# tanmayb123/OpenAI-Whisper-CoreML

Measured on AMD Instinct MI355X. Metric: audio-sec/s (RTF) + decoder tok/s, Whisper-large-v2 30s chunks, 1->8 GPU, higher is better.
Workload: dtype bf16

## Files before the change

include/whisper_mi355x_debug.h:

```cpp
#ifndef WHISPER_MI355X_DEBUG_H
#define WHISPER_MI355X_DEBUG_H

#include "whisper_mi355x.h"

#ifdef __cplusplus
extern "C" {
#endif

WM_API int wmdbg_mel_filterbank(int n_mels, float *out);
WM_API int wmdbg_mel80(float *out);

WM_API int wmdbg_gemm(wm_ctx *ctx, const float *A, const float *W, const float *bias, float *C, int M, int N,
               int K, int epi);
typedef struct wmdbg_gemm_map {
    int32_t M, N, K, epi;
    int64_t a_off, a_rpb, a_bstride, a_rstride, a_elems;
    int64_t c_off, c_rpb, c_bstride, c_rstride, c_elems;
    int32_t d_model, n_head, seq, seq_pad, batch, reserved;
    int64_t vt_elems;
} wmdbg_gemm_map;
WM_API int wmdbg_gemm_mapped(wm_ctx *ctx, const wmdbg_gemm_map *map, const float *A, const float *W, const float *bias,
                             const float *pos, float *C, float *vt);
WM_API int wmdbg_gemm_map_layout(int32_t *out4);

// ... 75 lines not shown
                               uint32_t *hit_out, uint32_t *ban_out, int32_t *cnt_out, int32_t *id_out, float *total_out,
                               int32_t *woff_out);
WM_API int wmdbg_sb_expand_tables(const int32_t *tokens, const int32_t *seq_offsets, const float *bias, const uint8_t *boost_prefixes,
                                  const int32_t *table_offsets, int n_tables, int32_t eot, int V, int32_t *counts_out,
                                  int32_t *tab_grp_out, int32_t *grp_id_out, int32_t *grp_beg_out, int32_t *ent_len_out,
                                  float *ent_bias_out, int32_t *ent_ctx_out);
WM_API int wmdbg_group_given(const int32_t *lens, const int32_t *tokens, int stride, int rows, int b0, int Cg, int N, int32_t *lens_out,
                             int32_t *tok_out, int tok_cap, int32_t *L_out);
WM_API int wmdbg_group_bias_rows(const int32_t *table_of_row, int B, const int32_t *tab_grp, int n_tables, int b0, int Cg, int N,
                                 int32_t *rng_out);
WM_API int wmdbg_seqbias_rows_state(wm_ctx *ctx, const int32_t *seq, int B, int n_ctx, int pos, int n_prompt, int V,
                                    const int32_t *tokens, const int32_t *seq_offsets, const float *bias,
                                    const uint8_t *boost_prefixes, const int32_t *table_offsets, int n_tables, int32_t eot,
                                    const int32_t *table_of_row, const uint32_t *ban_in, uint32_t *hit_out, uint32_t *ban_out,
                                    int32_t *cnt_out, int32_t *id_out, float *total_out, int32_t *woff_out);
WM_API int wmdbg_constraint_state(wm_ctx *ctx, const int32_t *seq, int B, int n_ctx, int pos, int n_prompt, int V,
                                  const int32_t *edge_beg, const int32_t *edge_tok, const int32_t *edge_next, const int32_t *def_next,
                                  const uint8_t *accept, int n_states, int32_t eot, const int32_t *starts, const uint32_t *ban_in,
                                  uint32_t *ban_out, int32_t *state_out);
WM_API int wmdbg_decode_close_cst(wm_ctx *ctx, wmdbg_step *io, const int32_t *edge_beg, const int32_t *edge_tok,
                                  const int32_t *edge_next, const int32_t *def_next, const uint8_t *accept, int n_states, int32_t eot,
                                  const int32_t *starts);
WM_API int wmdbg_step_layout(int32_t *out4);

WM_API int wmdbg_dec_attention(wm_ctx *ctx, const float *q, const float *k, const float *v, int B, int H, int T,
                        int n_keys, int nsplit, float *out);
WM_API int wmdbg_dec_self_attention_off(wm_ctx *ctx, const float *q, const float *k, const float *v, int B, int H, int T,
                                        int pos, const int32_t *off, float *out);

typedef struct wmdbg_attn {
    int32_t form;
    int32_t B, C, N, H;
    int32_t T;
    int32_t n_keys;
    int32_t nsplit;
    int32_t pos;
    int32_t n_live;
    int32_t short_lived;
    int32_t warm_rows, warm_k;
    int32_t K;
    const int32_t *off;
    const int32_t *live_rows;
    const float *q;
    const float *k, *v;
    const float *x;
    const float *ln_g, *ln_b;
    const float *Wq;
    const float *bias;
    float *out;
    float *mean_out;
    int32_t plan[16];
} wmdbg_attn;
WM_API int wmdbg_dec_attention_form(wm_ctx *ctx, wmdbg_attn *io);
WM_API int wmdbg_attn_layout(int32_t *out4);

WM_API int wmdbg_dec_self_attention_panel(wm_ctx *ctx, const float *q, const float *k, const float *v, int C, int w, int H,
                                          int T, int pos, int out_rows, float *out);
WM_API int wmdbg_dec_qkv_panel(wm_ctx *ctx, const float *x, const float *ln_g, const float *ln_b, const float *W,
                               const float *bias, int C, int w, int N, int K, int n_head, int T, int pos, float *q_out,
                               float *kcache, float *vcache);
WM_API int wmdbg_dec_embed_panel(wm_ctx *ctx, const float *emb, const float *pemb, int V, int d, int n_ctx, const int32_t *seq,
                                 int stride, int c0, int C, int w, int pos, int by_steps, float *x, float *xb, float *stats,
                                 float *mean);
WM_API int wmdbg_dec_self_attention_panel_off(wm_ctx *ctx, const float *q, const float *k, const float *v, int C, int w, int H,
                                              int T, int pos, const int32_t *off, int out_rows, float *out);
WM_API int wmdbg_dec_embed_panel_off(wm_ctx *ctx, const float *emb, const float *pemb, int V, int d, int n_ctx, const int32_t *seq,
                                     int stride, int c0, int C, int w, int pos, const int32_t *off, int by_steps, float *x, float *xb,
                                     float *stats, float *mean);
WM_API int wmdbg_prompt_panel_plan(int G, int width, int P, int sot_pos, int acap_base, int32_t *out);
WM_API int wmdbg_prompt_panel_plan_batch(int n, const int32_t *in, int32_t *out);
WM_API int wmdbg_last_prompt_prefill(wm_ctx *ctx, int32_t *out);
WM_API int wmdbg_given_panel_plan(int G, int width, const int32_t *lens, const int32_t *budgets, int max_new, int P, int n_text_ctx,
                                  uint32_t bits, int32_t *out);
WM_API int wmdbg_given_panel_plan_batch(int n, int g_max, const int32_t *in, int32_t *out);
WM_API int wmdbg_last_given_panel(wm_ctx *ctx, int32_t *out);
WM_API int wmdbg_last_given_panel_lane(wm_ctx *ctx, int lane, int32_t *out);
typedef struct {
    int32_t G, w, V, K, n_ctx, pos, n_prompt, max_new, first, last;
    const float *x;
    const float *ln_g, *ln_b;
    const float *emb;
    const float *bias;
    const int32_t *suppress;
    int32_t n_suppress, fallback_tok;
    int32_t ts_mode, ts_begin, eot;
    int32_t *hist, *rng;
    int32_t *chist, *crng;
    int32_t stop_on, stop_eot, pad_tok;
    int32_t *done;
    const int32_t *budget;
    int32_t *live_rows;
    int32_t n_live;
    const int32_t *glens, *gtok;
    int32_t stride;
    int32_t *seq;
    float *logprob;
    int32_t *wtok;
    float *wlp;
    float *logits;
    int32_t pos_out;
} wmdbg_given_panel;
WM_API int wmdbg_given_panel_round(wm_ctx *ctx, wmdbg_given_panel *io);
WM_API int wmdbg_align_capture_panel(wm_ctx *ctx, const float *dq, int d, int C, int w, int pos, const int32_t *heads,
                                     int n_heads, int slot0, int Tq, int J, int by_steps, float *cap);
WM_API int wmdbg_align_token_prob_panel(wm_ctx *ctx, const float *logits, int C, int w, int V, int ldo, const int32_t *seq,
                                        int n_ctx, int pos, int S, int eot, const int32_t *n_text, int max_text, int by_steps,
                                        float *prob);

WM_API int wmdbg_bench_dec_gemv(wm_ctx *ctx, int B, int N, int K, int ln, int resid, int n_mats, int iters,
                         int nw_override, float *avg_us);
WM_API int wmdbg_bench_dec_attention(wm_ctx *ctx, int B, int H, int T, int n_keys, int nsplit, int n_slices,
                              int iters, float *avg_us);

WM_API int wmdbg_bench_launch_floor(wm_ctx *ctx, int iters, int grid, float *eager_us, float *graph_us);

WM_API int wmdbg_bench_graph_branches(wm_ctx *ctx, int iters, int grid, int us_each, float *one_us, float *two_us);

WM_API int wmdbg_bench_gemm(wm_ctx *ctx, int M, int N, int K, int epi, int iters, int n_w, float *us);

WM_API int wmdbg_set_gemm_tile(int tile);

WM_API int wmdbg_lane_parts(int B, int lanes, int explicit_lanes, int n_text_state);
WM_API int wmdbg_cu_mask(int cu_lo, int cu_hi, uint32_t *mask8);

WM_API int wmdbg_set_precision(wm_ctx *ctx, int precision);

WM_API int wmdbg_set_tuning(const char *key, int value);
WM_API int wmdbg_group_count(int B, int lanes, int explicit_lanes);
WM_API int wmdbg_right_align(const int32_t *prompts, int stride, const int32_t *prompt_len, int b0, int Bg, int32_t *table_out,
                             int32_t *off_out);

WM_API int wmdbg_cand_groups(int B, int N, int lanes, int explicit_lanes, int32_t *b0_out, int32_t *cg_out);
WM_API int wmdbg_dec_attn_plan(const int32_t *in, int n, int32_t *out);
WM_API int wmdbg_dec_gemv_plan(const int32_t *in, int n, int32_t *out);
WM_API int wmdbg_tx_plan(const int32_t *in, int n, int32_t *out, int32_t *cut, int cut_cap);
WM_API int wmdbg_tx_plan_bounded(const int32_t *in, const int32_t *max_group_rows, int n, int32_t *out, int32_t *cut, int cut_cap);
WM_API int wmdbg_group_tables(const int32_t *in, int n, int32_t *out);
WM_API int wmdbg_group_rows_out(const int32_t *in, int n, int32_t *out);
WM_API int wmdbg_spec_groups(int B, int k, int spec_group, int32_t *b0_out, int32_t *cg_out);
WM_API int wmdbg_spec_width(int k, int bound, int last);
WM_API int wmdbg_spec_round(int G, int w, const int32_t *accepted, const int32_t *live, const int32_t *eot_at, const int32_t *left,
                            int32_t *live_out, int32_t *inc_out);
WM_API int wmdbg_spec_round_batch(int n, int G, int w, const int32_t *in, int32_t *out);
WM_API int wmdbg_pending_refusal(unsigned pending, int entry, unsigned flags, int n_cand, char *msg_out, int msg_cap);
WM_API int wmdbg_pending_take(unsigned bits, unsigned again, int32_t *out);
WM_API int wmdbg_spec_script(wm_ctx *ctx, const int32_t *tokens, int B, int max_new);
WM_API int wmdbg_spec_accept(wm_ctx *ctx, int G, int w, int n_tiles, int pos, int n_prompt, int n_ctx, int max_new, int32_t eot,
                             const int32_t *budget, const uint64_t *tilemax, const float *txt, const float *win, int32_t *seq,
                             int32_t *done, float *logprob_out, int32_t *stats_out, int32_t *round_out, int32_t *acc_out,
                             int32_t *draft_seq_out, int32_t *pos_out);
typedef struct wmdbg_spec {
    int32_t which;
    int32_t G, w, cap;
    int32_t n_prompt, n_ctx, max_new, n_vocab;
    int32_t tts_on, dts_on;
    int32_t tts_par[4], dts_par[4];
    int32_t eot, pad_tok;
    const int32_t *script;
    const int32_t *budget;
    int32_t *tseq, *dseq;
    int32_t *pos2;
    int32_t *tts_hist;
    int32_t *tts_rng;
    int32_t *dts_hist, *dts_rng;
    int32_t *chist, *crng, *dchist, *dcrng;
// ... 94 lines not shown
```

openai-whisper-coreml_amd/csrc/call_src.cpp:

```cpp
#include "call_src.h"

#include <string.h>

static size_t pcm_elem(wm_dtype t) { return t == WM_I16 ? 2 : t == WM_F32 ? 4 : 8; }

int wm_check_window(const WmAudioSrc &a, int b, const char *who) {
    WM_REQUIRE(a.mel_base[b] >= 0 && a.mel_len[b] >= 1 && a.seek[b] >= 0 && a.n_frames[b] >= 1 &&
                   a.n_frames[b] <= WM_N_FRAMES && (int64_t)a.seek[b] + a.n_frames[b] <= a.mel_len[b],
               WM_ERR_INVALID, "%srow %d: window (base %lld, T %d, seek %d, n_frames %d) invalid", who, b,
               (long long)a.mel_base[b], a.mel_len[b], a.seek[b], a.n_frames[b]);
    return WM_OK;
}

int wm_check_src_pointers(const WmAudioSrc &a) {
    if (a.windows) {
        WM_REQUIRE(a.set != nullptr, WM_ERR_INVALID, "null window set");
        return WM_OK;
    }
    WM_REQUIRE(a.mel && a.mel_base && a.mel_len && a.seek && a.n_frames, WM_ERR_INVALID, "null mel / window pointer");
    return WM_OK;
}

int wm_check_set_owner(const wm_ctx *ctx, const wm_windows *w) {
    const WmModel *m = ctx->model;
// ... 10 lines not shown
    WM_REQUIRE(a.rows || B == W, WM_ERR_INVALID, "%srows is NULL: B (%d) must be the set's %d windows", who, B, W);
    for (int b = 0; a.rows && b < B; ++b)
        WM_REQUIRE(a.rows[b] >= 0 && a.rows[b] < W, WM_ERR_INVALID, "%srow %d: window %d outside the set's [0, %d)", who, b, a.rows[b], W);
    return WM_OK;
}

int wm_stage_pcm(wm_ctx *c, const WmAudioSrc &a, int b0, int Bg, wm_mem mem, const void **d_pcm) {
    WmModel *m = c->model;
    *d_pcm = nullptr;
    if (a.mel || a.windows) return WM_OK;
    const size_t row = WM_N_SAMPLES * pcm_elem(a.pcm_dtype);
    *d_pcm = (const char *)a.pcm + (size_t)b0 * row;
    if (mem != WM_MEM_HOST) return WM_OK;
    WM_TRY(m->pcm_stage.reserve(c->stream, (size_t)Bg * row));
    WM_HIP(hipMemcpyAsync(m->pcm_stage.p, *d_pcm, (size_t)Bg * row, hipMemcpyHostToDevice, c->stream));
    *d_pcm = m->pcm_stage.p;
    return WM_OK;
}

int wm_stage_mel(wm_ctx *c, const WmAudioSrc &a, int b0, int Bg, wm_mem mem, const void *d_pcm, std::vector<WmMelWin> &win,
              const float **enc_mel, const WmMelWin **enc_win) {
    WmModel *m = c->model;
    const int C = m->dims.n_mels;
    *enc_mel = m->mel_f32;
    *enc_win = nullptr;
    if (!a.mel) return wm_frontend_run(&c->fe, &c->prof, c->stream, d_pcm, a.pcm_dtype, Bg, C, m->mel_f32, WM_F32);
    win.resize(Bg);
    for (int b = 0; b < Bg; ++b) {
        const int r = b0 + b;
        WmMelWin &w = win[b];
        w.T = a.mel_len[r]; w.seek = a.seek[r]; w.n = a.n_frames[r]; w.pad = 0;
        w.base = a.mel_base[r];
        if (mem == WM_MEM_HOST) {
            WM_HIP(hipMemcpy2DAsync(m->mel_f32 + (size_t)b * C * WM_N_FRAMES, WM_N_FRAMES * sizeof(float),
                                    a.mel + w.base + w.seek, (size_t)w.T * sizeof(float), (size_t)w.n * sizeof(float),
                                    C, hipMemcpyHostToDevice, c->stream));
            w.base = (long long)b * C * WM_N_FRAMES; w.T = WM_N_FRAMES; w.seek = 0;
        }
    }
    WM_HIP(hipMemcpyAsync(m->dmel_win, win.data(), (size_t)Bg * sizeof(WmMelWin), hipMemcpyHostToDevice, c->stream));
    if (mem != WM_MEM_HOST) *enc_mel = a.mel;
    *enc_win = m->dmel_win;
    return WM_OK;
}

int wm_stage_cross_kv(wm_ctx *c, const WmAudioSrc &a, int b0, int Bg, wm_mem mem, const void *d_pcm, std::vector<WmMelWin> &win,
                   std::vector<int32_t> &map, hipEvent_t staged) {
    WmModel *m = c->model;
    if (a.windows) {
        const wm_dims &D = m->dims;
        map.resize(Bg);
        for (int b = 0; b < Bg; ++b) map[b] = a.rows ? a.rows[b0 + b] : b0 + b;
        WM_HIP(hipMemcpyAsync(m->dxkv_rows, map.data(), (size_t)Bg * 4, hipMemcpyHostToDevice, c->stream));
        WM_TRY(wm_xkv_rows(c, m->xkv, Bg, a.set->store, m->dxkv_rows, 0, Bg, 2 * D.n_text_layer, (long)D.n_text_head * 1500 * 64,
                           false));
        if (staged) WM_HIP(hipEventRecord(staged, c->stream));
        return WM_OK;
    }
    const float *enc_mel;
    const WmMelWin *enc_win;
    WM_TRY(wm_stage_mel(c, a, b0, Bg, mem, d_pcm, win, &enc_mel, &enc_win));
    if (staged) WM_HIP(hipEventRecord(staged, c->stream));
    WM_TRY(wm_model_encode_win(c, enc_mel, enc_win, Bg, nullptr));
    return wm_model_cross_kv(c, Bg);
}
```

openai-whisper-coreml_amd/csrc/debug_hooks.cpp:

```cpp
#include <math.h>
#include <stddef.h>
#include <stdio.h>
#include <stdlib.h>
#include <string.h>

#include <algorithm>
#include <cmath>
#include <vector>

#include "../../include/whisper_mi355x_debug.h"
#include "beam.h"
#include "model.h"
#include "tx_plan.h"

namespace {
struct DevPool {
    std::vector<void *> v;
    DevPool() = default;
    DevPool(const DevPool &) = delete;
    DevPool &operator=(const DevPool &) = delete;
    ~DevPool() {
        for (void *p : v) (void)hipFree(p);
    }
    template <class T>
    int get(T **d, const void *h, size_t bytes, hipStream_t s, int fill = 0) {
        void *p = nullptr;
        WM_HIP(hipMalloc(&p, bytes + 512));
        v.push_back(p);
        *d = static_cast<T *>(p);
        WM_HIP(hipMemsetAsync(p, fill, bytes + 512, s));
        if (h) WM_HIP(hipMemcpyAsync(p, h, bytes, hipMemcpyHostToDevice, s));
        return WM_OK;
    }
};

bf16_t f2bf(float f) {
    uint32_t u;
    memcpy(&u, &f, 4);
    u += 0x7fffu + ((u >> 16) & 1u);
    return (bf16_t)(u >> 16);
}
void to_bf16(const float *in, std::vector<bf16_t> &out, size_t n) {
    out.resize(n);
    for (size_t i = 0; i < n; ++i) out[i] = f2bf(in[i]);
}
void from_bf16(const std::vector<bf16_t> &in, float *out) {
    for (size_t i = 0; i < in.size(); ++i) {
        uint32_t u = (uint32_t)in[i] << 16;
        memcpy(&out[i], &u, 4);
    }
}
void tile_bf16(const float *m, size_t rows, size_t K, std::vector<bf16_t> &out) {
    const size_t rpad = (rows + 15) / 16 * 16;
    std::vector<float> t(rpad * K, 0.f);
    for (size_t r = 0; r < rows; ++r)
        for (size_t k = 0; k < K; ++k) t[wm_tiled_offset(r, k, K)] = m[r * K + k];
    to_bf16(t.data(), out, t.size());
}
void untile_bf16(const std::vector<bf16_t> &t, size_t rows, size_t K, float *out) {
    std::vector<bf16_t> lin(rows * K);
    for (size_t r = 0; r < rows; ++r)
        for (size_t k = 0; k < K; ++k) lin[r * K + k] = t[wm_tiled_offset(r, k, K)];
    from_bf16(lin, out);
}
void fill_bf16(std::vector<bf16_t> &v, size_t n) { v.assign(n, (bf16_t)WMDBG_SENTINEL_BF16); }
void fill_f32(std::vector<float> &v, size_t n) {
// ... 103 lines not shown
        return WM_OK;
    }
    int replay_us(EventPair &ev, float *us) {
        WM_HIP(hipGraphLaunch(ge, s));
        WM_HIP(hipStreamSynchronize(s));
        WM_TRY(ev.start(s));
        WM_HIP(hipGraphLaunch(ge, s));
        return ev.stop_us(s, us);
    }
};

struct SideBranch {
    hipStream_t s2 = nullptr;
    hipEvent_t ef = nullptr, ej = nullptr;
    SideBranch() = default;
    SideBranch(const SideBranch &) = delete;
    SideBranch &operator=(const SideBranch &) = delete;
    ~SideBranch() {
        if (ef) (void)hipEventDestroy(ef);
        if (ej) (void)hipEventDestroy(ej);
        if (s2) (void)hipStreamDestroy(s2);
    }
    int init() {
        WM_HIP(hipStreamCreateWithFlags(&s2, hipStreamNonBlocking));
        WM_HIP(hipEventCreateWithFlags(&ef, hipEventDisableTiming));
        WM_HIP(hipEventCreateWithFlags(&ej, hipEventDisableTiming));
        return WM_OK;
    }
    int fork(hipStream_t s) {
        WM_HIP(hipEventRecord(ef, s));
        WM_HIP(hipStreamWaitEvent(s2, ef, 0));
        return WM_OK;
    }
    int join(hipStream_t s) {
        WM_HIP(hipEventRecord(ej, s2));
        WM_HIP(hipStreamWaitEvent(s, ej, 0));
        return WM_OK;
    }
};
}

int wm_gemm_set_tile_override(int tile);
extern "C" int wmdbg_set_gemm_tile(int tile) { return wm_gemm_set_tile_override(tile); }

extern "C" int wmdbg_set_tuning(const char *key, int value) {
    WM_REQUIRE(key, WM_ERR_INVALID, "wmdbg_set_tuning: null key");
    struct { const char *name; int *field; } table[] = {
        {"gemv_tn", &g_wm_tuning.gemv_tn}, {"gemv_nblk", &g_wm_tuning.gemv_nblk}, {"gemv_no_ppw2", &g_wm_tuning.gemv_no_ppw2}, {"gemv_ppw2_nblk", &g_wm_tuning.gemv_ppw2_nblk},
        {"prefetch_max_b", &g_wm_tuning.prefetch_max_b}, {"xattn_split_below", &g_wm_tuning.xattn_split_below},
        {"xattn_wgs", &g_wm_tuning.xattn_wgs}, {"xattn_no_flat", &g_wm_tuning.xattn_no_flat},
        {"xattn_lds_pad", &g_wm_tuning.xattn_lds_pad}, {"xattn_splits", &g_wm_tuning.xattn_splits},
        {"gemm_tile", &g_wm_tuning.gemm_tile}, {"gemm128_pipe", &g_wm_tuning.gemm128_pipe}, {"gemm_gm", &g_wm_tuning.gemm_gm}, {"no_early_stop", &g_wm_tuning.no_early_stop},
        {"xattn_no_deep", &g_wm_tuning.xattn_no_deep}, {"xattn_never_short", &g_wm_tuning.xattn_never_short},         {"logits_tn", &g_wm_tuning.logits_tn}, {"enc_attn_mfma_sum", &g_wm_tuning.enc_attn_mfma_sum},
        {"group_chunks", &g_wm_tuning.group_chunks}, {"argmax_rows_per_wg", &g_wm_tuning.argmax_rows_per_wg}, {"xattn_fuse_q", &g_wm_tuning.xattn_fuse_q},
        {"teacher_panel_cut", &g_wm_tuning.teacher_panel_cut}, {"lane_parts", &g_wm_tuning.lane_parts}, {"lane_solo_cus", &g_wm_tuning.lane_solo_cus}, {"spec_group", &g_wm_tuning.spec_group}, {"frontend_per_wave_twiddles", &g_wm_tuning.frontend_per_wave_twiddles},
    };
    if (strcmp(key, "reset") == 0) { g_wm_tuning = WmTuning(); return WM_OK; }
    for (auto &e : table)
        if (strcmp(key, e.name) == 0) { *e.field = value; return WM_OK; }
    wm_set_error("wmdbg_set_tuning: unknown key '%s'", key);
    return WM_ERR_INVALID;
}

extern "C" int wmdbg_group_count(int B, int lanes, int explicit_lanes) { return wm_group_count(B, lanes, explicit_lanes != 0, 0); }
extern "C" int wmdbg_cand_groups(int B, int N, int lanes, int explicit_lanes, int32_t *b0_out, int32_t *cg_out) {
    if (B < 1 || N < 1 || N > WM_MAX_BEST_OF || !b0_out || !cg_out) return -1;
    std::vector<int> b0, cg;
    const int G = wm_cand_groups(B, N, lanes, explicit_lanes != 0, b0, cg);
    for (int g = 0; g < G; ++g) { b0_out[g] = b0[g]; cg_out[g] = cg[g]; }
    return G;
}
extern "C" int wmdbg_dec_attn_plan(const int32_t *in, int n, int32_t *out) {
    if (!in || !out || n < 0) return -1;
    for (int i = 0; i < n; ++i) wm_attn_plan_flat(in + (size_t)i * WM_ATTN_PLAN_IN, g_wm_tuning, out + (size_t)i * WM_ATTN_PLAN_OUT);
    return n;
}
extern "C" int wmdbg_dec_gemv_plan(const int32_t *in, int n, int32_t *out) {
    if (!in || !out || n < 0) return -1;
    for (int i = 0; i < n; ++i) wm_gemv_plan_flat(in + (size_t)i * WM_GEMV_PLAN_IN, g_wm_tuning, out + (size_t)i * WM_GEMV_PLAN_OUT);
    return n;
}
extern "C" int wmdbg_tx_plan(const int32_t *in, int n, int32_t *out, int32_t *cut, int cut_cap) {
    if (!in || !out || !cut || n < 0 || cut_cap < 0) return -1;
    int used = 0;
    for (int i = 0; i < n; ++i) {
        int32_t *o = out + (size_t)i * WM_TX_PLAN_OUT;
        const int k = wm_tx_plan_flat(in + (size_t)i * WM_TX_PLAN_IN, o, cut + used, cut_cap - used);
        if (k < 0) return -1;
        o[5] = used;
        used += k;
    }
    return n;
}
extern "C" int wmdbg_tx_plan_bounded(const int32_t *in, const int32_t *max_group_rows, int n, int32_t *out, int32_t *cut, int cut_cap) {
    if (!in || !max_group_rows || !out || !cut || n < 0 || cut_cap < 0) return -1;
    int used = 0;
    for (int i = 0; i < n; ++i) {
        int32_t *o = out + (size_t)i * WM_TX_PLAN_OUT;
        const int k = wm_tx_plan_flat(in + (size_t)i * WM_TX_PLAN_IN, o, cut + used, cut_cap - used, max_group_rows[i]);
        if (k < 0) return -1;
        o[5] = used;
        used += k;
    }
    return n;
}
extern "C" int wmdbg_group_tables(const int32_t *in, int n, int32_t *out) {
    if (!in || !out || n < 0) return -1;
// ... 449 lines not shown
    WM_TRY(pool.get(&dl, live.data(), live.size() * 4, s));
    WM_TRY(pool.get(&datt, nullptr, ((size_t)B + 15) / 16 * 16 * H * 64 * 2, s));
    DecAttnArgs t = {};
    t.q = dq; t.kc = dk; t.vc = dv; t.att = datt; t.part = dp; t.C = C; t.N = N; t.H = H; t.T_stride = T; t.n_keys = n_keys;
    t.live = live_rows ? dl : nullptr; t.short_lived = short_lived;
    WM_TRY(wm_dec_attention_cand(ctx, t));
    return down_tiled_bf16(datt, (size_t)B, (size_t)H * 64, out, s);
}

extern "C" int wmdbg_dec_attention_cand(wm_ctx *ctx, const float *q, const float *k, const float *v, int C, int N, int H, int T,
                                        int n_keys, const int32_t *live_rows, int n_live, float *out) {
    return dec_attention_cand(ctx, q, k, v, C, N, H, T, n_keys, live_rows, n_live, out, false);
}
extern "C" int wmdbg_dec_attention_cand_shared(wm_ctx *ctx, const float *q, const float *k, const float *v, int C, int N, int H,
                                               int T, int n_keys, const int32_t *live_rows, int n_live, float *out) {
    return dec_attention_cand(ctx, q, k, v, C, N, H, T, n_keys, live_rows, n_live, out, true);
}

extern "C" int wmdbg_dec_self_attention_off(wm_ctx *ctx, const float *q, const float *k, const float *v, int B, int H, int T,
                                            int pos, const int32_t *off, float *out) {
    WM_TRY(wm_ctx_make_current(ctx));
    WM_REQUIRE(q && k && v && off && out, WM_ERR_INVALID, "dec_self_attention_off: null pointer");
    WM_REQUIRE(B >= 1 && B <= WM_DEC_MAXB && T >= 1 && pos >= 0 && pos < T, WM_ERR_INVALID, "dec_self_attention_off: bad geometry");
    for (int b = 0; b < B; ++b)
        WM_REQUIRE(off[b] >= 0 && off[b] < T, WM_ERR_INVALID, "dec_self_attention_off: off[%d] = %d outside [0, %d)", b, off[b], T);
    std::vector<bf16_t> k16, v16;
    to_bf16(k, k16, (size_t)B * H * T * 64);
    to_bf16(v, v16, (size_t)B * H * T * 64);
    DevPool pool;
    hipStream_t s = ctx->stream;
    const float *dq;
    const bf16_t *dk, *dv;
    const int *doff, *dpos;
    bf16_t *datt;
    WM_TRY(pool.get(&dq, q, (size_t)B * H * 64 * 4, s));
    WM_TRY(pool.get(&dk, k16.data(), k16.size() * 2, s));
    WM_TRY(pool.get(&dv, v16.data(), v16.size() * 2, s));
    WM_TRY(pool.get(&doff, off, (size_t)B * 4, s));
    WM_TRY(pool.get(&dpos, &pos, 4, s));
    WM_TRY(pool.get(&datt, nullptr, ((size_t)B + 15) / 16 * 16 * H * 64 * 2, s));
    DecAttnArgs t = {};
    t.q = dq; t.kc = dk; t.vc = dv; t.att = datt; t.B = B; t.H = H; t.T_stride = T; t.pos_ptr = dpos; t.off = doff;
    WM_TRY(wm_dec_self_attention(ctx, t));
    return down_tiled_bf16(datt, (size_t)B, (size_t)H * 64, out, s);
}

extern "C" int wmdbg_attn_layout(int32_t *out4) {
    if (!out4) return WM_ERR_INVALID;
    out4[0] = (int32_t)sizeof(wmdbg_attn); out4[1] = (int32_t)offsetof(wmdbg_attn, off);
    out4[2] = (int32_t)offsetof(wmdbg_attn, out); out4[3] = (int32_t)offsetof(wmdbg_attn, plan);
    return WM_OK;
}

extern "C" int wmdbg_dec_attention_form(wm_ctx *ctx, wmdbg_attn *io) {
    WM_TRY(wm_ctx_make_current(ctx));
    WM_REQUIRE(io && io->out && io->k && io->v, WM_ERR_INVALID, "dec_attention_form: null pointer");
    memset(io->plan, 0, sizeof(io->plan));
    const int form = io->form, H = io->H, T = io->T;
    WM_REQUIRE(form >= 0 && form <= 3, WM_ERR_INVALID, "dec_attention_form: form %d is not 0 .. 3", form);
    const bool cand = form == 1, fq = form == 2, self = form == 3;
    WM_REQUIRE(!cand || (io->C >= 1 && io->N >= 1 && io->N <= WM_MAX_BEST_OF && io->C <= WM_DEC_MAXB), WM_ERR_INVALID,
               "dec_attention_form: %d windows x %d candidates", io->C, io->N);
    const int rows = cand ? io->C * io->N : io->B, entries = cand ? io->C : io->B;
    WM_REQUIRE(rows >= 1 && rows <= WM_DEC_MAXB && H >= 1 && H <= 1024, WM_ERR_INVALID, "dec_attention_form: %d rows x %d heads", rows, H);
    const size_t dd = (size_t)H * 64, rpad = ((size_t)rows + 15) / 16 * 16;
    {
        std::vector<bf16_t> s16;
        fill_bf16(s16, rpad * dd);
        from_bf16(s16, io->out);
        const uint32_t u = WMDBG_SENTINEL_F32;
        for (int b = 0; fq && io->mean_out && b < rows; ++b) memcpy(io->mean_out + b, &u, 4);
    }
    const bool has_pos = io->pos >= 0, has_pf = io->warm_rows > 0 && io->warm_k > 0;
    int32_t pin[WM_ATTN_PLAN_IN] = {0};
    pin[0] = form; pin[1] = cand ? 0 : io->B; pin[2] = cand ? io->C : 0; pin[3] = cand ? io->N : 0; pin[4] = H; pin[5] = T;
    pin[6] = io->n_keys; pin[7] = io->nsplit; pin[8] = fq ? io->K : 0;
    pin[9] = (has_pos ? 1 : 0) | (fq || self ? 0 : 2) | (io->off ? 4 : 0) | (has_pf ? 8 : 0) | (io->short_lived ? 16 : 0) | (io->live_rows ? 32 : 0);
    pin[10] = has_pf ? io->warm_rows : 0; pin[11] = has_pf ? io->warm_k : 0; pin[12] = ctx->n_cus;
    wm_attn_plan_flat(pin, g_wm_tuning, io->plan);
    if (io->plan[0] != WM_OK) return WM_ERR_INVALID;
    WM_REQUIRE(H <= 255 && T >= 1 && T <= WM_ATT_MAXK, WM_ERR_INVALID, "dec_attention_form: H 1 .. 255, T 1 .. %d", WM_ATT_MAXK);
    WM_REQUIRE(!has_pos || form == 0 || self, WM_ERR_INVALID, "dec_attention_form: form %d takes no device position", form);
    const int nk = has_pos ? io->pos + 1 : io->n_keys;
    WM_REQUIRE(nk >= 1 && nk <= T && io->n_keys >= 0 && io->n_keys <= T, WM_ERR_INVALID, "dec_attention_form: %d keys outside 1 .. T = %d", nk, T);
    WM_REQUIRE(self || (io->n_keys >= 1 && (!has_pos || io->n_keys == nk)), WM_ERR_INVALID,
               "dec_attention_form: a cross form needs n_keys >= 1 keys, and n_keys = pos + 1 with a device position");
    WM_REQUIRE(!io->off || self, WM_ERR_INVALID, "dec_attention_form: row offsets belong to the self-attention");
    WM_REQUIRE(!io->off || has_pos, WM_ERR_INVALID, "dec_attention_form: row offsets need the device position");
    for (int b = 0; io->off && b < rows; ++b)
        WM_REQUIRE(io->off[b] >= 0 && io->off[b] < T, WM_ERR_INVALID, "dec_attention_form: off[%d] = %d outside [0, %d)", b, io->off[b], T);
    WM_REQUIRE(!io->short_lived || form <= 1, WM_ERR_INVALID, "dec_attention_form: short_lived is a cross-attention shape");
    WM_REQUIRE(io->warm_rows >= 0 && io->warm_rows <= 8192 && io->warm_k >= 0 && io->warm_k <= 8192 && io->warm_k % 32 == 0 && io->warm_rows % 16 == 0,
               WM_ERR_INVALID, "dec_attention_form: warm-up matrix of %d x %d", io->warm_rows, io->warm_k);
    std::vector<int32_t> live((size_t)WM_DEC_MAXB + 4, 0);
    if (io->live_rows) {
        WM_REQUIRE(io->n_live >= 0 && io->n_live <= rows, WM_ERR_INVALID, "dec_attention_form: n_live %d outside [0, %d]", io->n_live, rows);
        for (int i = 0; i < io->n_live; ++i) {
            WM_REQUIRE(io->live_rows[i] >= 0 && io->live_rows[i] < rows && (i == 0 || io->live_rows[i] > io->live_rows[i - 1]), WM_ERR_INVALID,
                       "dec_attention_form: the live list must be ascending rows of the group");
            live[i] = io->live_rows[i];
        }
        live[WM_DEC_MAXB] = io->n_live;
    }
    if (fq)
        WM_REQUIRE(io->x && io->ln_g && io->ln_b && io->Wq && io->mean_out && io->K == H * 64 && io->K <= 1280, WM_ERR_INVALID,
                   "dec_attention_form: the fused query needs x, ln_g, ln_b, Wq, mean_out and K = H * 64 <= 1280");
    else
        WM_REQUIRE(io->q, WM_ERR_INVALID, "dec_attention_form: null query");
    std::vector<bf16_t> k16, v16, w16, x16, fill;
    std::vector<float> st, mean;
    to_bf16(io->k, k16, (size_t)entries * dd * T);
    to_bf16(io->v, v16, (size_t)entries * dd * T);
    fill_bf16(fill, rpad * dd);
    const std::vector<uint32_t> fill32((size_t)rows, WMDBG_SENTINEL_F32);
    DevPool pool;
    hipStream_t s = ctx->stream;
    const bf16_t *dk, *dv;
    bf16_t *datt;
    WM_TRY(pool.get(&dk, k16.data(), k16.size() * 2, s));
    WM_TRY(pool.get(&dv, v16.data(), v16.size() * 2, s));
    WM_TRY(pool.get(&datt, fill.data(), fill.size() * 2, s));
    DecAttnArgs t = {};
    t.kc = dk; t.vc = dv; t.att = datt; t.H = H; t.T_stride = T; t.n_keys = io->n_keys; t.short_lived = io->short_lived != 0;
    if (cand) { t.C = io->C; t.N = io->N; } else t.B = io->B;
    if (!fq) WM_TRY(pool.get(&t.q, io->q, (size_t)rows * dd * 4, s));
    if (form <= 1) WM_TRY(pool.get(&t.part, nullptr, (size_t)rows * H * WM_MAXSPLIT * 66 * 4, s));
    if (has_pos) WM_TRY(pool.get(&t.pos_ptr, &io->pos, 4, s));
    if (io->off) WM_TRY(pool.get(&t.off, io->off, (size_t)rows * 4, s));
    if (io->live_rows) WM_TRY(pool.get(&t.live, live.data(), live.size() * 4, s));
    if (has_pf) {
        WM_TRY(pool.get(&t.pf.ptr, nullptr, (size_t)io->warm_rows * io->warm_k * 2, s));
        t.pf.rows = io->warm_rows; t.pf.k = io->warm_k;
    }
    float *dmean_out = nullptr;
    switch (form) {
        case 0: t.nsplit = io->nsplit; WM_TRY(wm_dec_attention(ctx, t)); break;
        case 1: WM_TRY(wm_dec_attention_cand(ctx, t)); break;
        case 3: WM_TRY(wm_dec_self_attention(ctx, t)); break;
        default: {
            const int K = io->K, B = io->B;
            tile_bf16(io->Wq, (size_t)K, (size_t)K, w16);
            stage_ln_rows(io->x, B, K, true, x16, st, mean);
            DecGemvArgs a;
            memset(&a, 0, sizeof(a));
            a.epi = DE_Q; a.B = B; a.N = K; a.K = K; a.stats_parts = K / 16; a.ldo = K;
            const bf16_t *dW;
            bf16_t *dWf;
            float *dc1, *dc2;
            const float *dg, *db, *dbias = nullptr;
            WM_TRY(pool.get(&a.a, x16.data(), x16.size() * 2, s));
            WM_TRY(pool.get(&dW, w16.data(), w16.size() * 2, s));
            WM_TRY(pool.get(&dWf, nullptr, w16.size() * 2, s));
            WM_TRY(pool.get(&dc1, nullptr, (size_t)K * 4, s));
            WM_TRY(pool.get(&dc2, nullptr, (size_t)K * 4, s));
            WM_TRY(pool.get(&dg, io->ln_g, (size_t)K * 4, s));
            WM_TRY(pool.get(&db, io->ln_b, (size_t)K * 4, s));
            if (io->bias) WM_TRY(pool.get(&dbias, io->bias, (size_t)K * 4, s));
            WM_TRY(pool.get(&a.stats_in, st.data(), st.size() * 4, s));
            WM_TRY(pool.get(&a.mean_in, mean.data(), (size_t)B * 4, s));
            WM_TRY(pool.get(&a.mean_out, fill32.data(), (size_t)B * 4, s));
            WM_TRY(wm_ln_fold(ctx, dW, dg, db, dbias, K, K, dWf, dc1, dc2));
            a.W = dWf; a.c1 = dc1; a.c2 = dc2;
            dmean_out = a.mean_out;
            WM_TRY(wm_dec_xattn_fq(ctx, a, t));
        }
    }
    if (dmean_out) WM_HIP(hipMemcpyAsync(io->mean_out, dmean_out, (size_t)rows * 4, hipMemcpyDeviceToHost, s));
    return down_tiled_bf16(datt, rpad, dd, io->out, s);
}


extern "C" int wmdbg_bench_dec_gemv(wm_ctx *ctx, int B, int N, int K, int ln, int resid, int n_mats, int iters,
                                    int nw_override, float *avg_us) {
    (void)nw_override;
    WM_TRY(wm_ctx_make_current(ctx));
    WM_REQUIRE(B >= 1 && B <= WM_DEC_MAXB, WM_ERR_INVALID, "wmdbg_bench_dec_gemv: B out of range");
    DevPool pool;
    hipStream_t s = ctx->stream;
    const int Npad = ((N + 15) / 16) * 16;
    const bf16_t *dW;
    const float *dc;
    bf16_t *dout16;
    float *dstat;
    DecGemvArgs a;
    memset(&a, 0, sizeof(a));
    a.B = B; a.N = N; a.K = K; a.ldo = Npad; a.epi = resid ? DE_RESID : DE_Q;
    WM_TRY(pool.get(&dW, nullptr, (size_t)n_mats * Npad * K * 2, s, 0x3c));
    WM_TRY(pool.get(&a.a, nullptr, (size_t)WM_DEC_MAXB * K * 2, s));
    WM_TRY(pool.get(&dc, nullptr, (size_t)Npad * 4, s));
    WM_TRY(pool.get(&a.out_f32, nullptr, (size_t)WM_DEC_MAXB * Npad * 4, s));
    WM_TRY(pool.get(&dout16, nullptr, (size_t)WM_DEC_MAXB * Npad * 2, s));
    WM_TRY(pool.get(&dstat, nullptr, (size_t)(WM_DEC_MAXB / 16) * 2 * (K > N ? K : N) * 4 + 4096, s));
    a.c2 = dc;
    if (resid) { a.stats_out = dstat; a.out_bf16 = dout16; }
    if (ln) { a.c1 = dc; a.stats_in = dstat; a.stats_parts = K / 16; }
    EventPair ev;
    WM_TRY(ev.init());
    GraphRun run(s);
    WM_TRY(run.begin());
    for (int i = 0; i < iters; ++i) {
        a.W = dW + (size_t)(i % n_mats) * Npad * K;
        WM_TRY(wm_dec_gemv(ctx, a));
    }
    WM_TRY(run.end());
    float us = 0.f;
    WM_TRY(run.replay_us(ev, &us));
    *avg_us = us / iters;
    return WM_OK;
}

extern "C" int wmdbg_bench_dec_attention(wm_ctx *ctx, int B, int H, int T, int n_keys, int nsplit, int n_slices,
                                         int iters, float *avg_us) {
    WM_TRY(wm_ctx_make_current(ctx));
    DevPool pool;
    hipStream_t s = ctx->stream;
    const size_t slice = (size_t)B * H * T * 64;
    const bf16_t *dk, *dv;
    const float *dq;
    float *dp;
    bf16_t *datt;
    WM_TRY(pool.get(&dk, nullptr, slice * n_slices * 2, s));
    WM_TRY(pool.get(&dv, nullptr, slice * n_slices * 2, s));
    WM_TRY(pool.get(&dq, nullptr, (size_t)B * H * 64 * 4, s));
    WM_TRY(pool.get(&dp, nullptr, (size_t)B * H * WM_MAXSPLIT * 66 * 4, s));
    WM_TRY(pool.get(&datt, nullptr, ((size_t)B + 15) / 16 * 16 * H * 64 * 2, s));
    EventPair ev;
    WM_TRY(ev.init());
    DecAttnArgs t = {};
    t.q = dq; t.att = datt; t.part = dp; t.B = B; t.H = H; t.T_stride = T; t.n_keys = n_keys; t.nsplit = nsplit;
    for (int pass = 0; pass < 2; ++pass) {
        if (pass == 1) WM_TRY(ev.start(s));
        for (int i = 0; i < iters; ++i) {
            t.kc = dk + (size_t)(i % n_slices) * slice;
            t.vc = dv + (size_t)(i % n_slices) * slice;
            WM_TRY(wm_dec_attention(ctx, t));
        }
    }
    float us = 0.f;
    WM_TRY(ev.stop_us(s, &us));
    *avg_us = us / iters;
    return WM_OK;
}

int wm_launch_trivial(wm_ctx *ctx, int *p, int grid);
extern "C" int wmdbg_bench_launch_floor(wm_ctx *ctx, int iters, int grid, float *eager_us, float *graph_us) {
    WM_TRY(wm_ctx_make_current(ctx));
    DevPool pool;
    hipStream_t s = ctx->stream;
    int *d;
    WM_TRY(pool.get(&d, nullptr, 64, s));
    EventPair ev;
    WM_TRY(ev.init());
    float us = 0.f;
    for (int i = 0; i < 20; ++i) WM_TRY(wm_launch_trivial(ctx, d, grid));
    WM_TRY(ev.start(s));
    for (int i = 0; i < iters; ++i) WM_TRY(wm_launch_trivial(ctx, d, grid));
    WM_TRY(ev.stop_us(s, &us));
    *eager_us = us / iters;
    GraphRun run(s);
    WM_TRY(run.begin());
    for (int i = 0; i < iters; ++i) WM_TRY(wm_launch_trivial(ctx, d, grid));
    WM_TRY(run.end());
    WM_TRY(run.replay_us(ev, &us));
    *graph_us = us / iters;
    return WM_OK;
}

extern "C" int wmdbg_bench_gemm(wm_ctx *ctx, int M, int N, int K, int epi, int iters, int n_w, float *us) {
    WM_TRY(wm_ctx_make_current(ctx));
    WM_REQUIRE(epi == EPI_F32 || epi == EPI_BIAS_BF16 || epi == EPI_GELU_BF16 || epi == EPI_RESID_F32, WM_ERR_INVALID,
               "wmdbg_bench_gemm: epilogue %d not exposed", epi);
    WM_REQUIRE(n_w >= 1 && n_w <= 64, WM_ERR_INVALID, "wmdbg_bench_gemm: n_w out of range");
    std::vector<bf16_t> a16((size_t)M * K), w16((size_t)N * K);
    uint32_t x = 12345u;
    auto gauss = [&]() {
        float acc = 0.f;
        for (int i = 0; i < 4; ++i) { x = x * 1664525u + 1013904223u; acc += (float)(x >> 8) * (1.0f / 16777216.0f); }
        return (acc - 2.0f) * 1.7320508f;
    };
    for (auto &v : a16) v = f2bf(gauss());
    for (auto &v : w16) v = f2bf(0.02f * gauss());
    std::vector<float> bias(N);
    for (auto &v : bias) v = 0.01f * gauss();
    DevPool pool;
    hipStream_t s = ctx->stream;
    std::vector<const bf16_t *> dW(n_w, nullptr);
    GemmArgs g;
    memset(&g, 0, sizeof(g));
    WM_TRY(pool.get(&g.A, a16.data(), a16.size() * 2, s));
    for (int i = 0; i < n_w; ++i) WM_TRY(pool.get(&dW[i], w16.data(), w16.size() * 2, s));
    WM_TRY(pool.get(&g.bias, bias.data(), (size_t)N * 4, s));
    WM_TRY(pool.get(&g.C, nullptr, (size_t)M * N * 4, s));
    g.a_rpb = (long)M + 1; g.a_rstride = K;
    g.c_rpb = (long)M + 1; g.c_rstride = N; g.M = M; g.N = N; g.K = K; g.epi = epi;
// ... 584 lines not shown
    WmTsDev ts;
    memset(&ts, 0, sizeof(ts));
    if (io->ts_on) {
        ts.hist = (int *)dev(io->hist); ts.rng = (int *)dev(io->rng);
        ts.ts_begin = io->ts_par[0]; ts.eot = io->ts_par[1]; ts.n_vocab = io->ts_par[2]; ts.max_initial = io->ts_par[3];
    }
    WmStopDev sp;
    memset(&sp, 0, sizeof(sp));
    if (io->stop_on) {
        sp.done = (int *)dev(io->done); sp.live_rows = (int *)dev(io->live_rows); sp.n_live = (int *)dev(io->n_live);
        sp.eot = io->eot; sp.pad_tok = io->pad;
    }
    WmXDev xd;
    memset(&xd, 0, sizeof(xd));
    WM_TRY(pool.get(&xd.par, &xp, sizeof(xp), s));
    xd.logprob = (float *)dev(io->logprob);
    WM_TRY(wm_beam_select_step(ctx, rows, (int *)dev(io->seq), d_pos, n_prompt, WmEmbedDev{d_emb, d_pemb, d, d_x, d_xb, d_st, d_mean}, ts, sp,
                               xd, d_off, bm));
    for (const Buf &b : bufs)
        if (b.h) WM_HIP(hipMemcpyAsync(b.h, b.d, b.bytes, hipMemcpyDeviceToHost, s));
    WM_HIP(hipMemcpyAsync(&io->pos_out, d_pos, 4, hipMemcpyDeviceToHost, s));
    WM_HIP(hipMemcpyAsync(io->x_next, d_x, nr * d * 4, hipMemcpyDeviceToHost, s));
    WM_HIP(hipMemcpyAsync(io->mean_next, d_mean, nr * 4, hipMemcpyDeviceToHost, s));
    WM_HIP(hipMemcpyAsync(stn.data(), d_st, st_words * 4, hipMemcpyDeviceToHost, s));
    WM_TRY(down_tiled_bf16(d_xb, nr, (size_t)d, io->xb_next, s));
    io->stats_tail_nonzero = 0;
    for (size_t b = 0; b < nr; ++b) {
        stats_sum(stn.data(), d, (int)b, io->stats_next + b * 2);
        for (int part = 1; part < d / 16 && b < (size_t)rows; ++part)
            for (int c = 0; c < 2; ++c) {
                uint32_t u;
                memcpy(&u, &stn[stat_at(d, b, part, c)], 4);
                if (u != 0u) ++io->stats_tail_nonzero;
            }
    }
    return WM_OK;
}

extern "C" int wmdbg_xkv_rows(wm_ctx *ctx, uint16_t *group, int group_rows, uint16_t *store, int64_t store_rows, const int32_t *rows,
                              int n_rows, int L, int H, int to_store) {
    WM_TRY(wm_ctx_make_current(ctx));
    WM_REQUIRE(group && store && rows && L >= 1 && H >= 1 && n_rows >= 1 && n_rows <= group_rows && group_rows <= WM_DEC_MAXB &&
                   store_rows >= 1, WM_ERR_INVALID, "xkv_rows: bad args");
    for (int b = 0; b < n_rows; ++b) {
        WM_REQUIRE(rows[b] >= 0 && rows[b] < store_rows, WM_ERR_INVALID, "xkv_rows: rows[%d] = %d outside [0, %lld)", b, rows[b],
                   (long long)store_rows);
        for (int o = 0; to_store && o < b; ++o)
            WM_REQUIRE(rows[o] != rows[b], WM_ERR_INVALID, "xkv_rows: store row %d named twice", rows[b]);
    }
    DevPool pool;
    hipStream_t s = ctx->stream;
    const int *drows;
    WM_TRY(pool.get(&drows, rows, (size_t)n_rows * 4, s));
    int rc = wm_xkv_rows(ctx, group, group_rows, store, drows, 0, n_rows, 2 * L, (long)H * 1500 * 64, to_store != 0);
    if (hipStreamSynchronize(s) != hipSuccess && rc == WM_OK) {
        wm_set_error("xkv_rows: %s", hipGetErrorString(hipGetLastError()));
        rc = WM_ERR_HIP;
    }
    return rc;
}

static int dec_gemv_ln_run(wm_ctx *ctx, int epi, const float *x, const float *ln_g, const float *ln_b, const float *W,
                           const float *bias, int B, int N, int K, int centre, int n_head, int T, int pos, int panel, float *out_f32,
                           float *out_bf16, float *kcache, float *vcache, float *mean_out, float *Wf, float *c1, float *c2) {
    WM_TRY(wm_ctx_make_current(ctx));
    WM_REQUIRE(panel == 0 || (epi == DE_QKV && panel >= 1 && panel <= WM_MAX_TEACHER_PANEL && pos + panel <= T), WM_ERR_INVALID,
               "wmdbg_dec_qkv_panel: width 1 .. %d, pos + width <= T", WM_MAX_TEACHER_PANEL);
    WM_REQUIRE(epi == DE_QKV || epi == DE_Q || epi == DE_GELU, WM_ERR_INVALID, "wmdbg_dec_gemv_ln: epilogue %d not exposed", epi);
    WM_REQUIRE(x && ln_g && ln_b && W && mean_out && Wf && c1 && c2, WM_ERR_INVALID, "wmdbg_dec_gemv_ln: null pointer");
    WM_REQUIRE(B >= 1 && B <= WM_DEC_MAXB && N >= 1 && K >= 64 && K % 64 == 0 && K <= 1280, WM_ERR_INVALID,
               "wmdbg_dec_gemv_ln: B 1 .. %d, N >= 1, K a multiple of 64 up to 1280", WM_DEC_MAXB);
    const int d = N / 3;
    if (epi == DE_QKV)
        WM_REQUIRE(N % 3 == 0 && n_head >= 1 && d == n_head * 64 && T >= 1 && pos >= 0 && pos < T && out_f32 && kcache && vcache,
                   WM_ERR_INVALID, "wmdbg_dec_gemv_ln: DE_QKV needs N = 3 * n_head * 64, pos in [0, T) and its three outputs");
    if (epi == DE_Q) WM_REQUIRE(out_f32, WM_ERR_INVALID, "wmdbg_dec_gemv_ln: DE_Q needs out_f32");
    if (epi == DE_GELU) WM_REQUIRE(N % 32 == 0 && out_bf16, WM_ERR_INVALID, "wmdbg_dec_gemv_ln: DE_GELU needs N %% 32 == 0 and out_bf16");
    const size_t Npad = ((size_t)N + 15) / 16 * 16, Bpad = ((size_t)B + 15) / 16 * 16;
    std::vector<bf16_t> w16, x16;
    std::vector<float> st, mean;
    tile_bf16(W, (size_t)N, (size_t)K, w16);
    stage_ln_rows(x, B, K, centre != 0, x16, st, mean);
    const size_t n_f32 = epi == DE_QKV ? (size_t)B * d : epi == DE_Q ? (size_t)B * N : 0;
    const size_t n_b16 = epi == DE_GELU ? Bpad * N : 0, n_cache = epi == DE_QKV ? (size_t)(panel ? (B + panel - 1) / panel : B) * n_head * T * 64 : 0;
    const std::vector<bf16_t> fill16(std::max(n_b16, n_cache), (bf16_t)WMDBG_SENTINEL_BF16);
    const std::vector<uint32_t> fill32((size_t)B, WMDBG_SENTINEL_F32);
    std::vector<bf16_t> wf16(w16.size()), ob16(n_b16), k16(n_cache), v16(n_cache);
    DevPool pool;
    hipStream_t s = ctx->stream;
    DecGemvArgs a;
    memset(&a, 0, sizeof(a));
    a.epi = epi; a.B = B; a.N = N; a.K = K; a.stats_parts = K / 16; a.ldo = N;
    const bf16_t *dW;
    bf16_t *dWf;
    float *dc1, *dc2;
    const float *dg, *db, *dbias = nullptr, *dmin;
    const int *dpos;
    WM_TRY(pool.get(&a.a, x16.data(), x16.size() * 2, s));
    WM_TRY(pool.get(&dW, w16.data(), w16.size() * 2, s));
    WM_TRY(pool.get(&dWf, nullptr, w16.size() * 2, s));
    WM_TRY(pool.get(&dc1, nullptr, Npad * 4, s));
    WM_TRY(pool.get(&dc2, nullptr, Npad * 4, s));
    WM_TRY(pool.get(&dg, ln_g, (size_t)K * 4, s));
    WM_TRY(pool.get(&db, ln_b, (size_t)K * 4, s));
    if (bias) WM_TRY(pool.get(&dbias, bias, (size_t)N * 4, s));
    WM_TRY(pool.get(&a.stats_in, st.data(), st.size() * 4, s));
// ... 1364 lines not shown
    WM_HIP(hipMemcpyAsync(m->att, s16.data(), M * d * 2, hipMemcpyHostToDevice, s));
    WM_HIP(hipMemcpyAsync(m->hid, s16.data(), M * 4 * d * 2, hipMemcpyHostToDevice, s));
    WM_HIP(hipMemsetAsync(m->vt, 0, vt_n * 2, s));
    int rc = wm_model_encode_layer_qkv(ctx, layer, B);
    if (rc == WM_OK) rc = wm_model_encode_layer_tail(ctx, layer, B, dmid);
    if (rc == WM_OK) rc = down_bf16(m->att, M * d, att_out, s);
    if (rc == WM_OK) rc = down_bf16(m->xn, M * d, xn2_out, s);
    if (rc == WM_OK) rc = down_bf16(m->hid, M * 4 * d, hid_out, s);
    if (rc == WM_OK) {
        WM_HIP(hipMemcpyAsync(x_mid_out, dmid, M * d * 4, hipMemcpyDeviceToHost, s));
        WM_HIP(hipMemcpyAsync(x_out, m->x, M * d * 4, hipMemcpyDeviceToHost, s));
    }
    WM_HIP(hipMemsetAsync(m->qk + M * 2 * d, 0, (size_t)64 * 2 * d * 2, s));
    WM_HIP(hipStreamSynchronize(s));
    return rc;
}

extern "C" int wmdbg_encode_post(wm_ctx *ctx, const float *x, int B, float *xn_out, float *xa_out) {
    WM_REQUIRE(x && xn_out && xa_out, WM_ERR_INVALID, "wmdbg_encode_post: null pointer");
    WM_TRY(model_ready(ctx, B, "wmdbg_encode_post"));
    WmModel *m = ctx->model;
    const int d = m->dims.n_audio_state;
    const size_t M = (size_t)B * 1500;
    std::vector<bf16_t> s16;
    std::vector<float> s32;
    fill_bf16(s16, M * d);
    fill_f32(s32, M * d);
    hipStream_t s = ctx->stream;
    WM_HIP(hipMemcpyAsync(m->x, x, M * d * 4, hipMemcpyHostToDevice, s));
    WM_HIP(hipMemcpyAsync(m->xn, s16.data(), M * d * 2, hipMemcpyHostToDevice, s));
    WM_HIP(hipMemcpyAsync(m->xa_f32, s32.data(), M * d * 4, hipMemcpyHostToDevice, s));
    int rc = wm_model_encode_post(ctx, B, nullptr);
    if (rc == WM_OK) rc = down_bf16(m->xn, M * d, xn_out, s);
    if (rc == WM_OK) WM_HIP(hipMemcpyAsync(xa_out, m->xa_f32, M * d * 4, hipMemcpyDeviceToHost, s));
    WM_HIP(hipStreamSynchronize(s));
    return rc;
}

extern "C" int wmdbg_cross_kv(wm_ctx *ctx, const float *xa, int B, float *xkv_out) {
    WM_REQUIRE(xa && xkv_out, WM_ERR_INVALID, "wmdbg_cross_kv: null pointer");
    WM_TRY(model_ready(ctx, B, "wmdbg_cross_kv"));
    WmModel *m = ctx->model;
    const wm_dims &D = m->dims;
    WM_REQUIRE(D.n_text_state == D.n_audio_state, WM_ERR_INVALID, "wmdbg_cross_kv: encoder and decoder widths differ");
    const int d = D.n_text_state, H = D.n_text_head;
    const size_t M = (size_t)B * 1500, used = (size_t)D.n_text_layer * 2 * B * H * 1500 * 64,
                 cap = (size_t)D.n_text_layer * 2 * m->cap_b * H * 1500 * 64;
    std::vector<bf16_t> s16, got(cap);
    fill_bf16(s16, cap);
    DevPool pool;
    hipStream_t s = ctx->stream;
    const float *dxa;
    WM_TRY(pool.get(&dxa, xa, M * d * 4, s));
    WM_HIP(hipMemcpyAsync(m->xkv, s16.data(), cap * 2, hipMemcpyHostToDevice, s));
    int rc = wm_model_set_xa(ctx, dxa, B);
    if (rc == WM_OK) rc = wm_model_cross_kv(ctx, B);
    WM_HIP(hipMemcpyAsync(got.data(), m->xkv, cap * 2, hipMemcpyDeviceToHost, s));
    if (cap > used) WM_HIP(hipMemsetAsync(m->xkv + used, 0, (cap - used) * 2, s));
    WM_HIP(hipStreamSynchronize(s));
    WM_TRY(rc);
    size_t disturbed = 0;
    for (size_t i = used; i < cap; ++i) disturbed += got[i] != (bf16_t)WMDBG_SENTINEL_BF16;
    WM_REQUIRE(disturbed == 0, WM_ERR_STATE, "wmdbg_cross_kv: %zu elements behind the %d chunks' cache were written", disturbed, B);
    got.resize(used);
    from_bf16(got, xkv_out);
    return WM_OK;
}
```

openai-whisper-coreml_amd/csrc/dec_kernels.hip:

```cpp
#include <stdlib.h>

#include <atomic>
#include <string.h>

#include "dec_close.h"
#include "model.h"
#include "philox.h"

namespace {

typedef __attribute__((ext_vector_type(8))) __bf16 bf16x8;
typedef __attribute__((ext_vector_type(4))) float f32x4;
typedef __attribute__((ext_vector_type(4))) unsigned u32x4;

typedef __attribute__((ext_vector_type(2))) float f32x2;
typedef __attribute__((ext_vector_type(2))) __bf16 bf16x2;

__device__ __forceinline__ unsigned pack2(float a, float b) {
    const f32x2 v = {a, b};
    return __builtin_bit_cast(unsigned, __builtin_convertvector(v, bf16x2));
}
__device__ __forceinline__ float gelu_erf(float x) {
    return 0.5f * x * (1.0f + erff(x * 0.70710678118654752440f));
}
struct DecGemvDev {
    int B, N, K;
    const bf16_t *W;
    const float *c1;
    const float *c2;
    const bf16_t *a;
    const float *stats_in;
    int stats_parts;
    long stats_stride;
    float *stats_out;
    const float *mean_in;
    float *mean_out;
    float *out_f32;
    bf16_t *out_bf16;
    bf16_t *kcache, *vcache;
    const int *pos_ptr;
    int n_ctx, n_head;
    long ldo;
    unsigned long long *tilemax;
    int n_tiles;
    int n_tg, n_tg_pad;
    int arg_first, arg_last;
    const unsigned *mask;
    int mask_words, mask_first_pos;
    WmTsDev ts;
    WmXDev x;
    const char *pf_ptr;
    long pf_tile_bytes;
    int pf_tiles;
    int pf_head_major;
    int bgroups;
    WmRepDev rep;
    int panel;
    WmSbEpi sb;
};

// ... 1003 lines not shown
        const bf16_t *vb = vc + (long)bh * T_stride * 64 + e8 * 8;
        float qe[8];
        attn_scale_query(q + (long)b * d + h * 64 + e8 * 8, qe);
        float m_run = -1e30f, l_run = 0.f;
        float oa[8] = {0, 0, 0, 0, 0, 0, 0, 0};
        auto load_block = [&](int r0, u32x4 (&kv)[U], u32x4 (&vv)[U]) {
            attn_load_block<NS, U, NT>(kb, vb, r0, stream, rg, n_keys, last, kv, vv);
        };
        auto process_block = [&](int r0, const u32x4 (&kv)[U], const u32x4 (&vv)[U]) {
            attn_block<NS, U, false>(qe, r0, stream, rg, n_keys, kv, vv, m_run, l_run, oa);
        };
        if (DEEP) {
            constexpr int NB = ATT_MAXK / (NS * 8 * U);
            u32x4 kall[NB][U], vall[NB][U];
#pragma unroll
            for (int blk = 0; blk < NB; ++blk) load_block(blk * (NS * 8 * U), kall[blk], vall[blk]);
#pragma unroll
            for (int blk = 0; blk < NB; ++blk)
                if (blk * (NS * 8 * U) < n_keys) process_block(blk * (NS * 8 * U), kall[blk], vall[blk]);
        } else {
            for (int r0 = 0; r0 < n_keys; r0 += NS * 8 * U) {
                u32x4 kv[U], vv[U];
                load_block(r0, kv, vv);
                process_block(r0, kv, vv);
            }
        }
        attn_stream_reduce(l_run, oa);
        if (nsplit > 1) {
            if (rg == 0) {
                float *po = part + ((long)bh * NS + stream) * 66;
#pragma unroll
                for (int i = 0; i < 8; ++i) po[2 + e8 * 8 + i] = oa[i];
                if (e8 == 0) {
                    po[0] = m_run;
                    po[1] = l_run;
                }
            }
            continue;
        }
        if (rg == 0) {
#pragma unroll
            for (int i = 0; i < 8; ++i) wo_[wave][e8 * 8 + i] = oa[i];
            if (e8 == 0) {
                wm_[wave] = m_run;
                wl_[wave] = l_run;
            }
        }
        __syncthreads();
        if (tid < 64)
            att[wm_tiled_offset((size_t)b, (size_t)(h * 64 + tid), (size_t)d)] = f2bf(attn_merge<NS>(wm_, wl_, &wo_[0][0], 64, tid));
    }
}

struct CandLive {
    int r_lo, r_hi;
    unsigned long long head_lo, head_hi;
};
template <int N>
__device__ __forceinline__ void cand_window(const CandLive &L, int wj, int lane, int &c, unsigned &lm) {
    const int rank_lo = (int)__builtin_amdgcn_mbcnt_hi((unsigned)(L.head_lo >> 32), __builtin_amdgcn_mbcnt_lo((unsigned)L.head_lo, 0u));
    const int rank_hi = (int)__builtin_amdgcn_mbcnt_hi((unsigned)(L.head_hi >> 32), __builtin_amdgcn_mbcnt_lo((unsigned)L.head_hi, 0u)) +
                        __popcll(L.head_lo);
    const unsigned long long sel_lo = __ballot(((L.head_lo >> lane) & 1ull) && rank_lo == wj);
    const unsigned long long sel_hi = __ballot(((L.head_hi >> lane) & 1ull) && rank_hi == wj);
    int row;
    if (sel_lo) row = __builtin_amdgcn_readlane(L.r_lo, __builtin_ctzll(sel_lo));
    else row = __builtin_amdgcn_readlane(L.r_hi, sel_hi ? __builtin_ctzll(sel_hi) : 0);
    c = row / N;
    lm = 0u;
#pragma unroll
    for (int s = 0; s < N; ++s) {
        const int r = c * N + s;
        if ((__ballot(L.r_lo == r) | __ballot(L.r_hi == r)) != 0ull) lm |= 1u << s;
    }
}

template <int N, bool NT>
__global__ __launch_bounds__(512) void dec_xcand_attn_kernel(
    const float *__restrict__ q, const bf16_t *__restrict__ kc, const bf16_t *__restrict__ vc,
    const int *__restrict__ live_rows , bf16_t *__restrict__ att,
    float *__restrict__ part, unsigned packA , unsigned packB ,
    unsigned packC , const char *pf_ptr, long pf_tile_bytes) {
    constexpr int NS = 8, U = 4;
    static_assert(N >= 1 && N <= 8, "1 .. 8 candidates per window");
    constexpr int NP = N <= 5 ? N : (N + 1) / 2;
    const int H = (int)(packA & 0xffu), flat_wpw = (int)(packA >> 16);
    const int T_stride = (int)(packB & 0xffffu), n_keys = (int)(packB >> 16);
    const int C = (int)(packC & 0xffffu), n_wg = (int)(packC >> 16);
    const int d = H * 64;
    if (attn_warm_up(n_wg, pf_ptr, pf_tile_bytes, blockDim.x)) return;
    __shared__ float wm_[N][NS], wl_[N][NS];
    __shared__ float wo_[N][NS][64];
    const int tid = threadIdx.x, lane = tid & 63, wave = tid >> 6;
    const int rg = lane >> 3, e8 = lane & 7;
    const int last = n_keys - 1;
    CandLive L;
    {
        int n_live = C * N, p_lo = lane - 1, p_hi = lane + 63;
        L.r_lo = lane;
        L.r_hi = lane + 64;
        if (live_rows) {
            n_live = live_rows[WM_DEC_MAXB];
            L.r_lo = live_rows[lane];
            L.r_hi = live_rows[lane + 64];
            p_lo = live_rows[lane > 0 ? lane - 1 : 0];
            p_hi = live_rows[lane + 63];
// ... 520 lines not shown
        p.pf_ptr = (const char *)a.pf_ptr;
        p.pf_tile_bytes = pl.pf_tile_bytes; p.pf_tiles = pl.pf_tiles; p.pf_head_major = pl.pf_head_major;
    }
    WmProfScope ps(&ctx->prof, e->label_k && a.K > a.N ? e->label_k : e->label, ctx->stream);
    return e->launch(ctx, p, pl);
}

int wm_ln_fold(wm_ctx *ctx, const bf16_t *W, const float *g, const float *beta, const float *bias, int N, int K,
               bf16_t *Wf, float *c1, float *c2) {
    const int npad = (N + 15) / 16 * 16;
    ln_fold_kernel<<<npad, 256, 0, ctx->stream>>>(W, g, beta, bias, N, K, Wf, c1, c2);
    WM_HIP(hipGetLastError());
    return WM_OK;
}

int wm_dec_embed(wm_ctx *ctx, const int *seq, const int *pos_ptr, int B, const WmEmbedDev &e, const int *off) {
    WmProfScope ps(&ctx->prof, "dec_embed", ctx->stream);
    dec_embed_kernel<<<B, 256, 0, ctx->stream>>>(seq, pos_ptr, B, e.emb, e.pemb, e.d, e.x, e.xb, e.stats_out, e.mean_buf, off);
    WM_HIP(hipGetLastError());
    return WM_OK;
}

int wm_dec_embed_panel(wm_ctx *ctx, const int *seq, int seq_stride, const int *pos_ptr, int pos_add, int C, int w, int n_ctx,
                       const WmEmbedDev &e, const int *off) {
    WM_REQUIRE(w >= 1 && w <= WM_MAX_TEACHER_PANEL && C >= 1 && C * w <= WM_DEC_MAXB && seq_stride >= C, WM_ERR_INVALID,
               "dec_embed_panel: %d windows x %d positions (stride %d)", C, w, seq_stride);
    WmProfScope ps(&ctx->prof, "dec_embed_panel", ctx->stream);
    if (off)
        dec_embed_panel_off_kernel<<<C * w, 256, 0, ctx->stream>>>(seq, seq_stride, pos_ptr, pos_add, w, e.emb, e.pemb, e.d, n_ctx, e.x,
                                                                  e.xb, e.stats_out, e.mean_buf, off);
    else
        dec_embed_panel_kernel<<<C * w, 256, 0, ctx->stream>>>(seq, seq_stride, pos_ptr, pos_add, w, e.emb, e.pemb, e.d, n_ctx, e.x, e.xb,
                                                              e.stats_out, e.mean_buf);
    WM_HIP(hipGetLastError());
    return WM_OK;
}

int wm_dec_pos_add(wm_ctx *ctx, int *pos_ptr, int add) {
    dec_pos_add_kernel<<<1, 1, 0, ctx->stream>>>(pos_ptr, add);
    WM_HIP(hipGetLastError());
    return WM_OK;
}

int wm_dec_attn_splits(int B, int H) { return wm_dec_attn_splits(B, H, g_wm_tuning); }
bool wm_dec_xattn_fq_applies(int B, int H, int K, bool short_lived) { return wm_dec_xattn_fq_applies(B, H, K, short_lived, g_wm_tuning); }

namespace {
DecAttnShape attn_shape(const DecAttnArgs &t) {
    DecAttnShape s;
    memset(&s, 0, sizeof(s));
    s.B = t.B; s.C = t.C; s.N = t.N; s.H = t.H; s.T_stride = t.T_stride; s.n_keys = t.n_keys; s.nsplit = t.nsplit;
    s.has_pos = t.pos_ptr != nullptr; s.has_part = t.part != nullptr; s.has_off = t.off != nullptr; s.short_lived = t.short_lived;
    s.has_pf = t.pf.ptr != nullptr; s.pf_rows = t.pf.rows; s.pf_k = t.pf.k;
    return s;
}
int launch_combine(wm_ctx *ctx, const DecAttnArgs &t, const DecAttnPlan &pl);
}

int wm_dec_attention(wm_ctx *ctx, const DecAttnArgs &t) {
    DecAttnPlan pl;
    WM_TRY(wm_plan_attention(attn_shape(t), ctx->n_cus, g_wm_tuning, &pl));
    {
        WmProfScope ps(&ctx->prof, "dec_attn_cross", ctx->stream);
        const dim3 grid(pl.grid_x, pl.grid_y);
        if (pl.variant == DAV_STREAM) {
            const int lds_pad = g_wm_tuning.xattn_lds_pad;
            static std::atomic<int> pad_set[64];
            if (lds_pad > pad_set[ctx->device & 63].load(std::memory_order_acquire)) {
                WM_HIP(hipFuncSetAttribute((const void *)dec_xrows_attn_kernel<8, 4, WM_XATTN_NT>,
                                           hipFuncAttributeMaxDynamicSharedMemorySize, lds_pad));
                pad_set[ctx->device & 63].store(lds_pad, std::memory_order_release);
            }
            const AttnCold cold = {t.att, t.part, (const char *)t.pf.ptr, pl.tile_bytes};
            dec_xrows_attn_kernel<8, 4, WM_XATTN_NT><<<grid, pl.block, pl.lds, ctx->stream>>>(
                t.q, t.kc, t.vc, t.pos_ptr, t.live, pl.w.a, pl.w.b, pl.w.c, cold);
        } else {
            const AttnCold cold = {t.att, t.part, nullptr, 0};
            if (pl.variant == DAV_FLAT)
                dec_xrows_attn_kernel<8, 4, WM_XATTN_NT><<<grid, pl.block, 0, ctx->stream>>>(
                    t.q, t.kc, t.vc, t.pos_ptr, t.live, pl.w.a, pl.w.b, pl.w.c, cold);
            else if (pl.variant == DAV_FLAT_DEEP_C)
                dec_rows_attn_kernel<8, 4, false, true><<<grid, pl.block, 0, ctx->stream>>>(
                    t.q, t.kc, t.vc, t.pos_ptr, t.live, pl.w.a, pl.w.b, pl.w.c, cold);
            else
                dec_rows_attn_kernel<8, 4, WM_XATTN_NT, true><<<grid, pl.block, 0, ctx->stream>>>(
                    t.q, t.kc, t.vc, t.pos_ptr, t.live, pl.w.a, pl.w.b, pl.w.c, cold);
        }
        WM_HIP(hipGetLastError());
    }
    return pl.combine_grid ? launch_combine(ctx, t, pl) : WM_OK;
}

namespace {
int launch_combine(wm_ctx *ctx, const DecAttnArgs &t, const DecAttnPlan &pl) {
    WmProfScope ps(&ctx->prof, "dec_attn_combine", ctx->stream);
    dec_attn_combine_kernel<8><<<pl.combine_grid, 64, 0, ctx->stream>>>(t.part, t.H, t.H * 64, t.att);
    WM_HIP(hipGetLastError());
    return WM_OK;
}
}

int wm_dec_attention_cand(wm_ctx *ctx, const DecAttnArgs &t) {
    DecAttnPlan pl;
    WM_TRY(wm_plan_attention_cand(attn_shape(t), ctx->n_cus, g_wm_tuning, &pl));
    {
        WmProfScope ps(&ctx->prof, "dec_attn_cross_cand", ctx->stream);
        const char *pf = pl.warm_tiles ? (const char *)t.pf.ptr : nullptr;
        switch (t.N) {
#define WM_XCAND_CASE(n)                                                                                              \
    case n:                                                                                                           \
        dec_xcand_attn_kernel<n, WM_XATTN_NT><<<pl.grid_x, pl.block, 0, ctx->stream>>>(                               \
            t.q, t.kc, t.vc, t.live, t.att, t.part, pl.w.a, pl.w.b, pl.w.c, pf, pl.warm_tiles ? pl.tile_bytes : 0);   \
        break
            WM_XCAND_CASE(1); WM_XCAND_CASE(2); WM_XCAND_CASE(3); WM_XCAND_CASE(4);
            WM_XCAND_CASE(5); WM_XCAND_CASE(6); WM_XCAND_CASE(7); WM_XCAND_CASE(8);
#undef WM_XCAND_CASE
        }
        WM_HIP(hipGetLastError());
// ... 188 lines not shown
```

openai-whisper-coreml_amd/csrc/dec_launch.cpp:

```cpp
#include "dec_launch.h"

#include <stddef.h>
#include <string.h>

#include "../../include/whisper_mi355x.h"

void wm_set_error(const char *fmt, ...);

#define PLAN_REQUIRE(cond, ...)           \
    do {                                  \
        if (!(cond)) {                    \
            wm_set_error(__VA_ARGS__);    \
            return WM_ERR_INVALID;        \
        }                                 \
    } while (0)

namespace {
inline bool fits(int v, int bits) { return v >= 0 && (bits >= 31 || v < (1 << bits)); }
}

bool wm_pack_attn_keys(int T_stride, int n_keys, unsigned *b) {
    *b = (unsigned)T_stride | ((unsigned)n_keys << 16);
    return fits(T_stride, 16) && fits(n_keys, 16);
}
// ... 63 lines not shown
    const int bh = B * H;
    const int thr = t.xattn_split_below;
    if (bh >= thr) return 1;
    int ns = 2;
    while (ns < 8 && bh * ns < 192) ns *= 2;
    return ns;
}

int wm_dec_gemv_split(int K, int *spw) {
    const int steps = K / 32;
    for (int nw = steps >= 96 ? 16 : 8; nw >= 1; --nw) {
        if (steps % nw) continue;
        const int s = steps / nw;
        if (s == 2 || s == 4 || s == 5 || s == 6 || s == 8 || s == 10 || s == 12) {
            if (spw) *spw = s;
            return nw;
        }
    }
    return 0;
}

bool wm_dec_xattn_fq_applies(int B, int H, int K, bool short_lived, const WmTuning &t) {
    if (!t.xattn_fuse_q || short_lived) return false;
    const int pairs = B * H;
    if (pairs < t.xattn_split_below || pairs > 256 || K != H * 64) return false;
    int spw = 0;
    const int nw = wm_dec_gemv_split(K, &spw);
    return nw >= 1 && nw <= 8 && (spw == 2 || spw == 4 || spw == 5 || spw == 6);
}

int wm_plan_attention(const DecAttnShape &s, int n_cus, const WmTuning &t, DecAttnPlan *p) {
    const int B = s.B, H = s.H, nsplit = s.nsplit;
    memset(p, 0, sizeof(*p));
    PLAN_REQUIRE(nsplit == 1 || nsplit == 2 || nsplit == 4 || nsplit == 8, "dec_attention: nsplit %d is not 1, 2, 4 or 8", nsplit);
    PLAN_REQUIRE(s.T_stride <= WM_ATT_MAXK && s.n_keys <= WM_ATT_MAXK, "dec_attention: more than %d keys", WM_ATT_MAXK);
    PLAN_REQUIRE(nsplit == 1 || s.has_part, "dec_attention: split launch without a partials buffer");
    PLAN_REQUIRE(H >= 1 && H <= 255 && (long)B * H < 65536, "dec_attention: %d heads x %d rows do not fit the packed arguments", H, B);
    bool ok = wm_pack_attn_keys(s.T_stride, s.n_keys, &p->w.b);
    if (nsplit > 1 && !t.xattn_no_flat) {
        int wpw, g;
        wm_dec_flat_deal(B * H, 4, &wpw, &g);
        PLAN_REQUIRE(g < 65536, "dec_attention: flat grid too large");
        ok = wm_pack_attn_rows(H, 8, wpw, B * H, g, &p->w.a, &p->w.c) && ok;
        if (t.xattn_no_deep) p->variant = DAV_FLAT;
        else if ((size_t)B * H * s.T_stride * 64 * 2 * 2 <= (size_t)3200 * 1024) p->variant = DAV_FLAT_DEEP_C;
        else p->variant = DAV_FLAT_DEEP_NT;
        p->n_wg = p->grid_x = g;
        p->grid_y = 1;
        p->block = wpw * 64;
    } else {
        const int n_wg = wm_dec_persistent_wgs(B * H, n_cus, s.short_lived, t);
        p->warm_tiles = wm_dec_warm_tiles(B, s.has_pf && nsplit == 1, s.pf_rows, s.pf_k, n_wg, t, &p->tile_bytes);
        ok = wm_pack_attn_rows(H, nsplit, 0, B * H, n_wg, &p->w.a, &p->w.c) && ok;
        p->variant = DAV_STREAM;
        p->n_wg = n_wg;
        p->grid_x = n_wg + p->warm_tiles;
        p->grid_y = nsplit;
        p->block = (8 / nsplit) * 64;
        p->lds = nsplit == 1 ? t.xattn_lds_pad : 0;
    }
    PLAN_REQUIRE(ok, "dec_attention: a packed argument does not fit its bits");
    p->combine_grid = nsplit > 1 ? B * H : 0;
    return WM_OK;
}

int wm_plan_attention_cand(const DecAttnShape &s, int n_cus, const WmTuning &t, DecAttnPlan *p) {
    const int C = s.C, N = s.N, H = s.H;
    memset(p, 0, sizeof(*p));
    PLAN_REQUIRE(N >= 1 && N <= WM_MAX_BEST_OF && C >= 1 && (long)C * N <= WM_DEC_MAXB,
                 "dec_attention_cand: %d windows x %d candidates outside 1 .. %d rows of 1 .. %d candidates", C, N, WM_DEC_MAXB,
                 WM_MAX_BEST_OF);
    PLAN_REQUIRE(s.T_stride >= 1 && s.T_stride <= WM_ATT_MAXK && s.n_keys >= 1 && s.n_keys <= s.T_stride,
                 "dec_attention_cand: 1 .. %d keys", WM_ATT_MAXK);
    PLAN_REQUIRE(H >= 1 && H <= 255, "dec_attention_cand: %d heads do not fit the packed arguments", H);
    PLAN_REQUIRE(s.has_part || C * H >= 256 || s.short_lived, "dec_attention_cand: flat launch without a partials buffer");
    const int pairs = C * H;
    const bool flat = pairs < 256 && !s.short_lived;
    bool ok = wm_pack_attn_keys(s.T_stride, s.n_keys, &p->w.b);
    if (flat) {
        int wpw, g;
        wm_dec_flat_deal(pairs, 8, &wpw, &g);
        ok = wm_pack_attn_cand(H, wpw, C, g, &p->w.a, &p->w.c) && ok;
        p->variant = DAV_CAND_FLAT;
        p->n_wg = g;
        p->block = wpw * 64;
        p->combine_grid = C * N * H;
    } else {
        const int n_wg = wm_dec_persistent_wgs(pairs, n_cus, s.short_lived, t);
        PLAN_REQUIRE(n_wg < 65536, "dec_attention_cand: grid too large");
        ok = wm_pack_attn_cand(H, 0, C, n_wg, &p->w.a, &p->w.c) && ok;
        p->variant = DAV_CAND;
        p->n_wg = n_wg;
        p->block = 512;
    }
    PLAN_REQUIRE(ok, "dec_attention_cand: a packed argument does not fit its bits");
    p->warm_tiles = wm_dec_warm_tiles(C * N, s.has_pf, s.pf_rows, s.pf_k, p->n_wg, t, &p->tile_bytes);
    p->grid_x = p->n_wg + p->warm_tiles;
    p->grid_y = 1;
    return WM_OK;
}

int wm_plan_xattn_fq(const DecAttnShape &s, int n_cus, const WmTuning &t, DecAttnPlan *p) {
    (void)n_cus;
    const int B = s.B, H = s.H;
    memset(p, 0, sizeof(*p));
    PLAN_REQUIRE(s.K == (long)H * 64, "xattn_fq: not a LayerNorm-folded d x d query projection");
    PLAN_REQUIRE(H >= 1 && H <= 255 && B >= 1 && B <= WM_DEC_MAXB && s.T_stride <= WM_ATT_MAXK && s.n_keys >= 1 && s.n_keys <= WM_ATT_MAXK,
// ... 108 lines not shown
        const bool two = knob ? knob == 2 : (p->n_tiles * blocks > n_cus && p->n_tiles * ((blocks + 1) / 2) <= n_cus);
        if (two) {
            nblk = 2;
            p->bgroups = (blocks + 1) / 2;
        }
    }
    p->tn = tn;
    p->nblk = nblk;
    p->ppw = ppw;
    p->n_tg = (p->n_tiles + tn - 1) / tn;
    p->n_tg_pad = p->bgroups > 1 ? (p->n_tg + 7) / 8 * 8 : p->n_tg;
    p->grid = p->n_tg_pad * p->bgroups;
    p->pf_tiles = wm_dec_warm_tiles(B, s.has_pf, s.pf_rows, s.pf_k, p->grid, t, &p->pf_tile_bytes);
    if (p->pf_tiles) {
        p->pf_head_major = s.pf_head_major;
        p->grid += s.pf_head_major ? 32 * (s.pf_head_major / B + 2) : p->pf_tiles;
    }
    PLAN_REQUIRE(spw == 2 || spw == 4 || spw == 5 || spw == 6 || spw == 8 || spw == 10 || spw == 12,
                 "dec_gemv: unsupported k-steps per wave %d", spw);
    const bool resid = !ln && epi == DE_RESID;
    if (ppw == 2) {
        const bool two = resid && spw >= 6 && spw <= 10;
        PLAN_REQUIRE(two && tn == 1 && nblk >= 1 && nblk <= 2 && nw % 2 == 0, "dec_gemv: no two-part kernel for this shape");
        const int w2 = nw / 2;
        PLAN_REQUIRE(nblk != 2 || w2 == 8, "dec_gemv: the two-block two-part kernel needs 8 waves");
        p->row_split = nblk == 2 || (w2 >= 4 && B > 1);
        p->block = w2 * 64;
        p->lds = (long)nw * nblk * 1024 + (long)w2 * 32 * 4;
        return WM_OK;
    }
    p->block = nw * 64;
    if (resid && B > 1 && tn == 1 && nblk * 4 <= nw) {
        PLAN_REQUIRE(nblk == 1 || (nblk == 2 && spw <= 8), "dec_gemv: unsupported row-split shape (nblk %d, spw %d)", nblk, spw);
        p->row_split = 1;
        p->lds = (long)nw * nblk * 1024 + (long)nw * 32 * 4;
        return WM_OK;
    }
    const bool logits = de_is_logits(epi);
    const bool wide = ln && (de_is_qkv(epi) || epi == DE_GELU || logits) && spw <= 6;
    const bool have = (tn == 1 && nblk == 1) || (tn == 1 && nblk == 2 && spw <= 8) || ((tn == 2 || tn == 4) && nblk == 1 && wide && logits) ||
                      ((tn == 2 || tn == 4) && nblk == 2 && wide);
    PLAN_REQUIRE(have, "dec_gemv: unsupported launch shape (tn %d, nblk %d, spw %d)", tn, nblk, spw);
    p->lds = (long)nw * tn * nblk * 1024 + (long)nw * 32 * 4;
    return WM_OK;
}

void wm_attn_plan_flat(const int32_t *in, const WmTuning &t, int32_t *out) {
    DecAttnShape s;
    memset(&s, 0, sizeof(s));
    s.B = in[1]; s.C = in[2]; s.N = in[3]; s.H = in[4]; s.T_stride = in[5]; s.n_keys = in[6]; s.nsplit = in[7]; s.K = in[8];
    const int f = in[9];
    s.has_pos = f & 1; s.has_part = f & 2; s.has_off = f & 4; s.has_pf = f & 8; s.short_lived = f & 16;
    s.pf_rows = in[10]; s.pf_k = in[11];
    const int n_cus = in[12];
    DecAttnPlan p;
    memset(&p, 0, sizeof(p));
    int rc = WM_ERR_INVALID;
    switch (in[0]) {
        case 0: rc = wm_plan_attention(s, n_cus, t, &p); break;
        case 1: rc = wm_plan_attention_cand(s, n_cus, t, &p); break;
        case 2: rc = wm_plan_xattn_fq(s, n_cus, t, &p); break;
        case 3: rc = wm_plan_self_attention(s, n_cus, t, &p); break;
        case 4: rc = wm_plan_self_attention_panel(s, n_cus, t, &p); break;
        default: wm_set_error("attention plan: unknown form %d", in[0]);
    }
    memset(out, 0, sizeof(int32_t) * WM_ATTN_PLAN_OUT);
    out[0] = rc;
    const bool sane = s.B >= 0 && s.B <= WM_DEC_MAXB && s.H >= 0 && s.H <= 255;
    if (in[0] == 0 && sane) out[14] = wm_dec_attn_splits(s.B, s.H, t);
    if (in[0] == 2 && sane) out[14] = wm_dec_xattn_fq_applies(s.B, s.H, s.K, s.short_lived, t) ? 1 : 0;
    if (rc != WM_OK) return;
    out[1] = p.variant; out[2] = p.spw; out[3] = p.grid_x; out[4] = p.grid_y; out[5] = p.block; out[6] = p.lds; out[7] = p.n_wg;
    out[8] = p.warm_tiles; out[9] = (int32_t)p.tile_bytes; out[10] = (int32_t)p.w.a; out[11] = (int32_t)p.w.b; out[12] = (int32_t)p.w.c;
    out[13] = p.combine_grid;
}

void wm_gemv_plan_flat(const int32_t *in, const WmTuning &t, int32_t *out) {
    DecGemvShape s;
    memset(&s, 0, sizeof(s));
    s.epi = in[0]; s.ln = in[1] != 0; s.B = in[2]; s.N = in[3]; s.K = in[4];
    s.has_pf = in[5] != 0; s.pf_rows = in[6]; s.pf_k = in[7]; s.pf_head_major = in[8];
    DecGemvPlan p;
    const int rc = wm_plan_gemv(s, in[9], t, &p);
    memset(out, 0, sizeof(int32_t) * WM_GEMV_PLAN_OUT);
    out[0] = rc;
    if (rc != WM_OK) return;
    out[1] = p.nw; out[2] = p.spw; out[3] = p.tn; out[4] = p.nblk; out[5] = p.ppw; out[6] = p.row_split; out[7] = p.bgroups;
    out[8] = p.n_tiles; out[9] = p.n_tg; out[10] = p.n_tg_pad; out[11] = p.grid; out[12] = p.block; out[13] = (int32_t)p.lds;
    out[14] = p.pf_tiles; out[15] = (int32_t)p.pf_tile_bytes; out[16] = p.pf_head_major;
}
```

openai-whisper-coreml_amd/csrc/dec_launch.h:

```cpp
#pragma once
#include <stdint.h>

#include "wm_tuning.h"

constexpr int WM_DEC_MAXB = 128;
constexpr int WM_ATT_MAXK = 1536;

enum DecEpi { DE_QKV = 0, DE_Q = 1, DE_RESID = 2, DE_GELU = 3, DE_LOGITS = 4, DE_LOGITS_X = 5, DE_LOGITS_XR = 6, DE_QKV_P = 7, DE_LOGITS_XB = 8 };
constexpr bool de_is_x(int epi) { return epi == DE_LOGITS_X || epi == DE_LOGITS_XR || epi == DE_LOGITS_XB; }
constexpr bool de_has_rep(int epi) { return epi == DE_LOGITS_XR || epi == DE_LOGITS_XB; }
constexpr bool de_is_logits(int epi) { return epi == DE_LOGITS || de_is_x(epi); }
constexpr bool de_is_qkv(int epi) { return epi == DE_QKV || epi == DE_QKV_P; }

struct DecAttnWords { unsigned a, b, c; };
bool wm_pack_attn_keys(int T_stride, int n_keys, unsigned *b);
void wm_unpack_attn_keys(unsigned b, int *T_stride, int *n_keys);
bool wm_pack_attn_rows(int H, int nsplit, int flat_wpw, int n_bh, int n_wg, unsigned *a, unsigned *c);
void wm_unpack_attn_rows(unsigned a, unsigned c, int *H, int *nsplit, int *flat_wpw, int *n_bh, int *n_wg);
bool wm_pack_attn_cand(int H, int flat_wpw, int C, int n_wg, unsigned *a, unsigned *c);
void wm_unpack_attn_cand(unsigned a, unsigned c, int *H, int *flat_wpw, int *C, int *n_wg);
bool wm_pack_attn_fq(int H, int B, unsigned *a);
void wm_unpack_attn_fq(unsigned a, int *H, int *B);

int wm_dec_warm_tiles(int rows, bool has_pf, int pf_rows, int pf_k, int compute_grid, const WmTuning &t, long *tile_bytes);
int wm_dec_persistent_wgs(int pairs, int n_cus, bool short_lived, const WmTuning &t);
void wm_dec_flat_deal(int pairs, int wave_cap, int *wpw, int *g);
int wm_dec_attn_splits(int B, int H, const WmTuning &t);
int wm_dec_gemv_split(int K, int *spw);
bool wm_dec_xattn_fq_applies(int B, int H, int K, bool short_lived, const WmTuning &t);

enum DecAttnVariant {
    DAV_STREAM = 0,
    DAV_FLAT = 1,
    DAV_FLAT_DEEP_C = 2,
    DAV_FLAT_DEEP_NT = 3,
    DAV_SELF = 4,
    DAV_SELF_OFF = 5,
    DAV_SELF_PANEL = 6,
    DAV_CAND = 7,
    DAV_CAND_FLAT = 8,
    DAV_FQ = 9,
    DAV_SELF_OFF_PANEL = 10,
};
struct DecAttnShape {
    int B;
    int C, N;
    int H, T_stride, n_keys;
    int nsplit;
    int K;
    bool has_pos, has_part, has_off, has_pf, short_lived;
    int pf_rows, pf_k;
};
struct DecAttnPlan {
    int variant;
    int spw;
    int grid_x, grid_y, block;
    int lds;
    int n_wg;
    int warm_tiles;
    long tile_bytes;
    DecAttnWords w;
    int combine_grid;
};
int wm_plan_attention(const DecAttnShape &s, int n_cus, const WmTuning &t, DecAttnPlan *p);
int wm_plan_attention_cand(const DecAttnShape &s, int n_cus, const WmTuning &t, DecAttnPlan *p);
int wm_plan_xattn_fq(const DecAttnShape &s, int n_cus, const WmTuning &t, DecAttnPlan *p);
int wm_plan_self_attention(const DecAttnShape &s, int n_cus, const WmTuning &t, DecAttnPlan *p);
int wm_plan_self_attention_panel(const DecAttnShape &s, int n_cus, const WmTuning &t, DecAttnPlan *p);

struct DecGemvShape {
    int epi;
    bool ln;
    int B, N, K;
    bool has_pf;
    int pf_rows, pf_k, pf_head_major;
};
struct DecGemvPlan {
    int nw, spw;
    int tn, nblk;
    int ppw;
    int row_split;
    int bgroups, n_tiles, n_tg, n_tg_pad;
    int grid, block;
    long lds;
    int pf_tiles;
    long pf_tile_bytes;
    int pf_head_major;
};
int wm_plan_gemv(const DecGemvShape &s, int n_cus, const WmTuning &t, DecGemvPlan *p);

constexpr int WM_ATTN_PLAN_IN = 16, WM_ATTN_PLAN_OUT = 16, WM_GEMV_PLAN_IN = 12, WM_GEMV_PLAN_OUT = 20;
void wm_attn_plan_flat(const int32_t *in, const WmTuning &t, int32_t *out);
void wm_gemv_plan_flat(const int32_t *in, const WmTuning &t, int32_t *out);
```

openai-whisper-coreml_amd/csrc/model.cpp:

```cpp
#include "model.h"
#include "tx_plan.h"

#include <math.h>
#include <cmath>
#include <string.h>

static inline bf16_t host_f2bf(float f) {
    uint32_t u;
    memcpy(&u, &f, 4);
    u += 0x7fffu + ((u >> 16) & 1u);
    return (bf16_t)(u >> 16);
}
static inline float host_bf2f(bf16_t h) {
    uint32_t u = (uint32_t)h << 16;
    float f;
    memcpy(&f, &u, 4);
    return f;
}

static int dalloc(WmModel *m, void **p, size_t bytes, hipStream_t s) {
    bytes = (bytes + 255) & ~(size_t)255;
    WM_HIP(hipMalloc(p, bytes + 256));
    WM_HIP(hipMemsetAsync(*p, 0, bytes + 256, s));
    m->allocs.push_back(*p);
    return WM_OK;
}
template <typename T>
static int dalloc_t(WmModel *m, T **p, size_t n, hipStream_t s) {
    return dalloc(m, (void **)p, n * sizeof(T), s);
}

static void reg(WmModel *m, const std::string &name, void *ptr, bool is_bf16, size_t n, int kind,
                int layout = WL_PLAIN, int conv_c = 0, int kpad = 0) {
    WmTensor t;
    t.name = name; t.ptr = ptr; t.is_bf16 = is_bf16; t.n_elems = n; t.kind = kind;
    t.layout = layout; t.conv_c = conv_c; t.conv_kpad = kpad;
    m->index[name] = (int)m->tensors.size();
    m->tensors.push_back(t);
}

static int alloc_decode_buffers(WmModel *m, hipStream_t s) {
    const wm_dims &D = m->dims;
    const int d = D.n_text_state;
    WM_TRY(dalloc_t(m, &m->dx, (size_t)WM_DEC_MAXB * d, s));
    WM_TRY(dalloc_t(m, &m->dxb, (size_t)WM_DEC_MAXB * d, s));
    WM_TRY(dalloc_t(m, &m->dmean, (size_t)2 * WM_DEC_MAXB, s));
    WM_TRY(dalloc_t(m, &m->dq, (size_t)WM_DEC_MAXB * d, s));
    WM_TRY(dalloc_t(m, &m->dpart, (size_t)WM_DEC_MAXB * D.n_text_head * WM_MAXSPLIT * 66, s));
    WM_TRY(dalloc_t(m, &m->datt, (size_t)WM_DEC_MAXB * d, s));
    WM_TRY(dalloc_t(m, &m->dstats, (size_t)(WM_DEC_MAXB / 16) * (d / 16) * 16 * 2, s));
    WM_TRY(dalloc_t(m, &m->dhid, (size_t)WM_DEC_MAXB * 4 * d, s));
    WM_TRY(dalloc_t(m, &m->dlogits, (size_t)WM_DEC_MAXB * m->vpad, s));
    WM_TRY(dalloc_t(m, &m->dargmax, (size_t)WM_DEC_MAXB * (m->vpad / 16), s));
// ... 585 lines not shown
    const WmModel *pm = parent->model;
    WM_REQUIRE(pm && pm->finalized, WM_ERR_STATE, "clone: the parent's weights must be finalised");
    WmModel *m = new WmModel();
    child->model = m;
    m->dims = pm->dims; m->finalized = true; m->k1pad = pm->k1pad; m->vpad = pm->vpad;
    m->conv1_w = pm->conv1_w; m->conv2_w = pm->conv2_w; m->conv1_b = pm->conv1_b; m->conv2_b = pm->conv2_b;
    m->enc_pos = pm->enc_pos; m->enc = pm->enc; m->ln_post_g = pm->ln_post_g; m->ln_post_b = pm->ln_post_b;
    m->tok_emb = pm->tok_emb; m->dec_pos = pm->dec_pos; m->dec = pm->dec; m->ln_g = pm->ln_g; m->ln_b = pm->ln_b;
    m->emb_f = pm->emb_f; m->logit_c1 = pm->logit_c1; m->logit_c2 = pm->logit_c2;
    m->tensors = pm->tensors; m->index = pm->index;
    m->shares_weights = true;
    WM_TRY(alloc_decode_buffers(m, child->stream));
    WM_HIP(hipMemcpyAsync(m->dmask, pm->dmask, (size_t)2 * (m->vpad / 32) * 4, hipMemcpyDeviceToDevice, child->stream));
    m->mask_on = pm->mask_on; m->mask_host = pm->mask_host;
    m->ts_on = pm->ts_on; m->ts_begin = pm->ts_begin; m->ts_eot = pm->ts_eot; m->ts_max_initial = pm->ts_max_initial;
    m->align_l = pm->align_l; m->align_h = pm->align_h;
    m->teacher_panel = pm->teacher_panel;
    m->prompt_panel = pm->prompt_panel;
    m->given_panel = pm->given_panel;
    m->rep_on = pm->rep_on; m->rep_p = pm->rep_p; m->rep_n = pm->rep_n; m->rep_eot = pm->rep_eot;
    m->samp_k = pm->samp_k; m->samp_p = pm->samp_p; m->samp_minp = pm->samp_minp;
    if (m->rep_on || pm->sb_on || pm->sbt_on || pm->cst_on) WM_TRY(alloc_repetition_state(m, child->stream));
    if (pm->cst_on) {
        WM_TRY(alloc_constraint_state(m, child->stream));
        WM_TRY(upload_constraint(m, pm->dcst, pm->cst_states, pm->cst_edges, hipMemcpyDeviceToDevice, child->stream));
        m->cst_on = true; m->cst_states = pm->cst_states; m->cst_edges = pm->cst_edges; m->cst_eot = pm->cst_eot;
    }
    if (pm->sb_on) {
        WM_TRY(alloc_seqbias_state(m, child->stream));
        const size_t ng = (size_t)pm->sb_groups, ne = (size_t)pm->sb_entries;
        WM_HIP(hipMemcpyAsync((void *)m->dsb.grp_id, pm->dsb.grp_id, ng * 4, hipMemcpyDeviceToDevice, child->stream));
        WM_HIP(hipMemcpyAsync((void *)m->dsb.grp_beg, pm->dsb.grp_beg, (ng + 1) * 4, hipMemcpyDeviceToDevice, child->stream));
        WM_HIP(hipMemcpyAsync((void *)m->dsb.ent_len, pm->dsb.ent_len, ne * 4, hipMemcpyDeviceToDevice, child->stream));
        WM_HIP(hipMemcpyAsync((void *)m->dsb.ent_bias, pm->dsb.ent_bias, ne * 4, hipMemcpyDeviceToDevice, child->stream));
        WM_HIP(hipMemcpyAsync((void *)m->dsb.ent_ctx, pm->dsb.ent_ctx, ne * WM_SB_CTX * 4, hipMemcpyDeviceToDevice, child->stream));
        m->sb_on = true; m->sb_groups = pm->sb_groups; m->sb_entries = pm->sb_entries;
    }
    if (pm->sbt_on) {
        WM_TRY(alloc_seqbias_state(m, child->stream));
        WM_TRY(alloc_seqbias_pool(m, child->stream));
        WM_TRY(upload_seqbias_pool(m, pm->dsbt, pm->sbt_groups, pm->sbt_entries, hipMemcpyDeviceToDevice, child->stream));
        m->sbt_on = true; m->sbt_groups = pm->sbt_groups; m->sbt_entries = pm->sbt_entries; m->sbt_tab_grp = pm->sbt_tab_grp;
    }
    WM_HIP(hipStreamSynchronize(child->stream));
    return WM_OK;
}

void wm_model_destroy(wm_ctx *ctx) {
    WmModel *m = ctx->model;
    if (!m) return;
    wm_model_drop_graphs(m);
    if (m->h_nlive) (void)hipHostFree(m->h_nlive);
    if (m->h_spec) (void)hipHostFree(m->h_spec);
    m->spec_ws.release();
    for (void *p : m->allocs) (void)hipFree(p);
    for (WmDevBuf *b : {&m->pcm_stage, &m->io_stage, &m->align_ws, &m->acap_ws, &m->beam_ws, &m->beam_trace, &m->alt_ws, &m->given_ws})
        b->release();
    delete m;
    ctx->model = nullptr;
}

int wm_model_set_tensor(wm_ctx *ctx, const char *name, const float *data, size_t n) {
    WmModel *m = ctx->model;
    WM_REQUIRE(m, WM_ERR_STATE, "context has no model");
    WM_REQUIRE(!m->shares_weights, WM_ERR_STATE, "a cloned context shares its parent's weights: set them on the parent");
    WM_REQUIRE(name && data, WM_ERR_INVALID, "null name / data");
    auto it = m->index.find(name);
    WM_REQUIRE(it != m->index.end(), WM_ERR_INVALID, "unknown tensor '%s'", name);
    WmTensor &t = m->tensors[it->second];
    WM_REQUIRE(n == t.n_elems, WM_ERR_INVALID, "tensor '%s': %zu elements given, %zu expected", name, n, t.n_elems);
    if (!t.is_bf16) {
        WM_HIP(hipMemcpy(t.ptr, data, n * sizeof(float), hipMemcpyHostToDevice));
    } else if (t.layout == WL_PLAIN) {
        std::vector<bf16_t> tmp(n);
        for (size_t i = 0; i < n; ++i) tmp[i] = host_f2bf(data[i]);
        WM_HIP(hipMemcpy(t.ptr, tmp.data(), n * sizeof(bf16_t), hipMemcpyHostToDevice));
    } else if (t.layout == WL_TILED) {
        const size_t K = (size_t)t.conv_kpad, N = n / K;
        const size_t Np = (N + 15) / 16 * 16;
        std::vector<bf16_t> tmp(Np * K, 0);
        for (size_t r = 0; r < N; ++r)
            for (size_t k = 0; k < K; ++k) tmp[wm_tiled_offset(r, k, K)] = host_f2bf(data[r * K + k]);
        WM_HIP(hipMemcpy(t.ptr, tmp.data(), tmp.size() * sizeof(bf16_t), hipMemcpyHostToDevice));
    } else {
        const size_t per = (size_t)t.conv_c * 3, O = n / per;
        std::vector<bf16_t> tmp(O * t.conv_kpad, 0);
        for (size_t o = 0; o < O; ++o)
            for (int c = 0; c < t.conv_c; ++c)
                for (int tap = 0; tap < 3; ++tap)
                    tmp[o * t.conv_kpad + (size_t)tap * t.conv_c + c] = host_f2bf(data[o * per + (size_t)c * 3 + tap]);
        WM_HIP(hipMemcpy(t.ptr, tmp.data(), tmp.size() * sizeof(bf16_t), hipMemcpyHostToDevice));
    }
    t.set = true;
    m->finalized = false;
    return WM_OK;
}

int wm_model_get_tensor(wm_ctx *ctx, const char *name, float *data, size_t n) {
    WmModel *m = ctx->model;
    WM_REQUIRE(m, WM_ERR_STATE, "context has no model");
    WM_REQUIRE(name && data, WM_ERR_INVALID, "null name / data");
    auto it = m->index.find(name);
    WM_REQUIRE(it != m->index.end(), WM_ERR_INVALID, "unknown tensor '%s'", name);
    const WmTensor &t = m->tensors[it->second];
    WM_REQUIRE(n == t.n_elems, WM_ERR_INVALID, "tensor '%s': %zu elements asked, %zu stored", name, n, t.n_elems);
    WM_HIP(hipStreamSynchronize(ctx->stream));
// ... 33 lines not shown
            const int L = m->dims.n_audio_ctx, half = d / 2;
            std::vector<float> pe((size_t)L * d);
            const double inc = log(10000.0) / (half - 1);
            for (int p = 0; p < L; ++p)
                for (int j = 0; j < half; ++j) {
                    const double a = (double)p * exp(-inc * j);
                    pe[(size_t)p * d + j] = (float)sin(a);
                    pe[(size_t)p * d + half + j] = (float)cos(a);
                }
            WM_HIP(hipMemcpy(t.ptr, pe.data(), pe.size() * sizeof(float), hipMemcpyHostToDevice));
        } else {
            const bool scaled = t.kind == 0 && t.name.find("positional") == std::string::npos;
            WM_TRY(wm_fill_synthetic(ctx, t, (uint32_t)(seed & 0xffffffffu), (int)i, scaled ? matrix_gain : 1.0f));
        }
        t.set = true;
    }
    WM_HIP(hipStreamSynchronize(ctx->stream));
    m->finalized = false;
    return WM_OK;
}

int wm_model_finalize(wm_ctx *ctx) {
    WmModel *m = ctx->model;
    WM_REQUIRE(m, WM_ERR_STATE, "context has no model");
    for (const WmTensor &t : m->tensors)
        WM_REQUIRE(t.set, WM_ERR_STATE, "tensor '%s' was never set", t.name.c_str());
    const int d = m->dims.n_text_state;
    for (DecLayerW &L : m->dec) {
        WM_TRY(wm_ln_fold(ctx, L.wqkv, L.ln1_g, L.ln1_b, L.bqkv, 3 * d, d, L.wqkv_f, L.qkv_c1, L.qkv_c2));
        WM_TRY(wm_ln_fold(ctx, L.wxq, L.lnx_g, L.lnx_b, L.bxq, d, d, L.wxq_f, L.xq_c1, L.xq_c2));
        WM_TRY(wm_ln_fold(ctx, L.w1, L.ln2_g, L.ln2_b, L.b1, 4 * d, d, L.w1_f, L.fc1_c1, L.fc1_c2));
    }
    WM_TRY(wm_ln_fold(ctx, m->tok_emb, m->ln_g, m->ln_b, nullptr, m->dims.n_vocab, d, m->emb_f, m->logit_c1, m->logit_c2));
    WM_HIP(hipStreamSynchronize(ctx->stream));
    m->finalized = true;
    return WM_OK;
}

int WmDevBuf::reserve(hipStream_t stream, size_t need) {
    if (bytes >= need) return WM_OK;
    WM_HIP(hipStreamSynchronize(stream));
    if (p) WM_HIP(hipFree(p));
    p = nullptr; bytes = 0;
    WM_HIP(hipMalloc(&p, need));
    bytes = need;
    return WM_OK;
}

int wm_model_reserve(wm_ctx *ctx, int B) {
    WmModel *m = ctx->model;
    WM_REQUIRE(m, WM_ERR_STATE, "context has no model");
    if (B <= m->cap_b) return WM_OK;
    WM_HIP(hipStreamSynchronize(ctx->stream));
    void *olds[] = {m->mel_t, m->h1p, m->x, m->xn, m->qk, m->vt, m->att, m->hid, m->xa_f32, m->mel_f32, m->xkv, m->skv};
    for (void *p : olds)
        if (p) {
            (void)hipFree(p);
            for (auto &a : m->allocs)
                if (a == p) a = nullptr;
        }
    const wm_dims &D = m->dims;
    const int d = D.n_audio_state, H = D.n_audio_head;
    const size_t M = (size_t)B * 1500;
    hipStream_t s = ctx->stream;
    WM_TRY(dalloc_t(m, &m->mel_t, (size_t)B * 3002 * D.n_mels, s));
    WM_TRY(dalloc_t(m, &m->h1p, (size_t)B * 3001 * d, s));
    WM_TRY(dalloc_t(m, &m->x, M * d, s));
    WM_TRY(dalloc_t(m, &m->xn, M * d, s));
    WM_TRY(dalloc_t(m, &m->qk, (M + 64) * 2 * d, s));
    WM_TRY(dalloc_t(m, &m->vt, (size_t)B * H * 64 * 1536, s));
    WM_TRY(dalloc_t(m, &m->att, M * d, s));
    WM_TRY(dalloc_t(m, &m->hid, M * 4 * d, s));
    WM_TRY(dalloc_t(m, &m->xa_f32, M * d, s));
    WM_TRY(dalloc_t(m, &m->mel_f32, (size_t)B * D.n_mels * WM_N_FRAMES, s));
    WM_TRY(dalloc_t(m, &m->xkv, (size_t)D.n_text_layer * 2 * B * H * 1500 * 64, s));
    const int Bd = std::max(B < WM_DEC_MAXB ? B : WM_DEC_MAXB, m->cap_rows);
    WM_TRY(dalloc_t(m, &m->skv, (size_t)D.n_text_layer * 2 * Bd * H * D.n_text_ctx * 64, s));
    m->cap_b = B;
    m->cap_rows = Bd;
    WM_HIP(hipStreamSynchronize(s));
    return WM_OK;
}

int wm_model_reserve_rows(wm_ctx *ctx, int rows) {
    WmModel *m = ctx->model;
    WM_REQUIRE(m && rows >= 1 && rows <= WM_DEC_MAXB, WM_ERR_INVALID, "decode rows must be 1..%d", WM_DEC_MAXB);
    if (rows <= m->cap_rows) return WM_OK;
    WM_HIP(hipStreamSynchronize(ctx->stream));
    wm_model_drop_graphs(m);
    if (m->skv) {
        (void)hipFree(m->skv);
        for (auto &a : m->allocs)
            if (a == m->skv) a = nullptr;
        m->skv = nullptr;
    }
    const wm_dims &D = m->dims;
    m->cap_rows = 0;
    WM_TRY(dalloc_t(m, &m->skv, (size_t)D.n_text_layer * 2 * rows * D.n_audio_head * D.n_text_ctx * 64, ctx->stream));
    m->cap_rows = rows;
    WM_HIP(hipStreamSynchronize(ctx->stream));
    return WM_OK;
}

static GemmArgs plain_gemm(const bf16_t *A, int lda, const bf16_t *W, const float *bias, void *C, int ldc,
                           int M, int N, int K, int epi) {
    GemmArgs g;
// ... 40 lines not shown
}

int wm_model_encode_layer_qkv(wm_ctx *ctx, int layer, int B) {
    WmModel *m = ctx->model;
    const wm_dims &D = m->dims;
    const int d = D.n_audio_state, H = D.n_audio_head, S = 1500, M = B * S;
    const EncLayerW &L = m->enc[layer];
    WM_TRY(wm_layernorm(ctx, m->x, L.ln1_g, L.ln1_b, M, d, m->xn, nullptr));
    GemmArgs g = plain_gemm(m->xn, d, L.wqkv, L.bqkv, m->qk, 2 * d, M, 3 * d, d, EPI_QKV_ENC);
    g.vt = m->vt; g.d_model = d; g.n_head = H; g.seq = S; g.seq_pad = 1536; g.batch = B;
    return wm_gemm(ctx, g);
}

int wm_model_encode_layer_tail(wm_ctx *ctx, int layer, int B, float *d_x_mid) {
    WmModel *m = ctx->model;
    const wm_dims &D = m->dims;
    const int d = D.n_audio_state, H = D.n_audio_head, S = 1500, M = B * S;
    const EncLayerW &L = m->enc[layer];
    WM_TRY(wm_enc_attention(ctx, m->qk, m->vt, m->att, B, H, S, 1536, d));
    WM_TRY(wm_gemm(ctx, plain_gemm(m->att, d, L.wo, L.bo, m->x, d, M, d, d, EPI_RESID_F32)));
    if (d_x_mid) WM_HIP(hipMemcpyAsync(d_x_mid, m->x, (size_t)M * d * 4, hipMemcpyDeviceToDevice, ctx->stream));
    WM_TRY(wm_layernorm(ctx, m->x, L.ln2_g, L.ln2_b, M, d, m->xn, nullptr));
    WM_TRY(wm_gemm(ctx, plain_gemm(m->xn, d, L.w1, L.b1, m->hid, 4 * d, M, 4 * d, d, EPI_GELU_BF16)));
    return wm_gemm(ctx, plain_gemm(m->hid, 4 * d, L.w2, L.b2, m->x, d, M, d, 4 * d, EPI_RESID_F32));
}

int wm_model_encode_post(wm_ctx *ctx, int B, float *d_xa_out) {
    WmModel *m = ctx->model;
    const int d = m->dims.n_audio_state, M = B * 1500;
    return wm_layernorm(ctx, m->x, m->ln_post_g, m->ln_post_b, M, d, m->xn, d_xa_out ? d_xa_out : m->xa_f32);
}

int wm_model_encode_win(wm_ctx *ctx, const float *d_mel, const WmMelWin *d_win, int B, float *d_xa_out) {
    WM_TRY(wm_model_encode_stem(ctx, d_mel, d_win, B));
    const int n_layer = ctx->model->dims.n_audio_layer;
    for (int i = 0; i < n_layer; ++i) {
        WM_TRY(wm_model_encode_layer_qkv(ctx, i, B));
        WM_TRY(wm_model_encode_layer_tail(ctx, i, B, nullptr));
    }
    return wm_model_encode_post(ctx, B, d_xa_out);
}

int wm_model_set_xa(wm_ctx *ctx, const float *d_xa, int B) {
    WmModel *m = ctx->model;
    WM_REQUIRE(m && m->finalized, WM_ERR_STATE, "model weights not finalised (wm_finalize)");
    WM_TRY(wm_model_reserve(ctx, B));
    return wm_f32_to_bf16(ctx, d_xa, m->xn, (size_t)B * 1500 * m->dims.n_audio_state);
}

int wm_model_cross_kv(wm_ctx *ctx, int B) {
    WmModel *m = ctx->model;
    const wm_dims &D = m->dims;
    const int d = D.n_text_state, H = D.n_text_head, S = 1500, M = B * S;
    for (int l = 0; l < D.n_text_layer; ++l) {
        const DecLayerW &L = m->dec[l];
        GemmArgs g = plain_gemm(m->xn, d, L.wxkv, L.bxkv, m->xkv + (size_t)l * 2 * B * H * S * 64, 0, M, 2 * d, d,
                                EPI_XKV);
        g.d_model = d; g.n_head = H; g.seq = S; g.batch = B;
        WM_TRY(wm_gemm(ctx, g));
    }
    return WM_OK;
}

int wm_model_decode_begin(wm_ctx *ctx, int B) {
    WmModel *m = ctx->model;
    WM_REQUIRE(m && m->finalized, WM_ERR_STATE, "model weights not finalised (wm_finalize)");
    WM_REQUIRE(B >= 1 && B <= WM_DEC_MAXB, WM_ERR_INVALID, "decode batch must be 1..%d", WM_DEC_MAXB);
    WM_HIP(hipMemsetAsync(m->darrive, 0, sizeof(int), ctx->stream));
    return WM_OK;
}

int wm_model_set_pos(wm_ctx *ctx, int pos) {
    WmModel *m = ctx->model;
    if (pos == 0) {
        WM_HIP(hipMemsetAsync(m->dpos, 0, sizeof(int), ctx->stream));
        return WM_OK;
    }
    WM_HIP(hipMemcpyAsync(m->dpos, &pos, sizeof(int), hipMemcpyHostToDevice, ctx->stream));
    WM_HIP(hipStreamSynchronize(ctx->stream));
    return WM_OK;
}

static int decode_step_impl(wm_ctx *ctx, int B, bool want_logits, int arg_first, int arg_last, const WmAlignCap *cap,
                            const WmDecodeMode &mode, int n_prompt, int grp, int c0, bool cache_only = false) {
    WmModel *m = ctx->model;
    const wm_dims &D = m->dims;
    const int d = D.n_text_state, H = D.n_text_head, T = D.n_text_ctx, S = 1500;
    const int PW = mode.panel > 1 ? mode.panel : 1;
    const int NC = mode.n_cand > 1 ? mode.n_cand : 1;
    WM_REQUIRE(PW == 1 || (NC == 1 && !mode.stop && (!mode.off || cache_only) && !(mode.x && mode.rep) && B % PW == 0), WM_ERR_STATE,
               "decode step: a panel is a plain teacher-forced step of windows x width rows");
    const int Bx = B / (NC * PW);
    const int Gx = grp > 0 ? grp : Bx;
    const int Gs = grp > 0 ? grp : (PW > 1 ? Bx : B);
    const int ns = wm_dec_attn_splits(B, H);
    const int xns = g_wm_tuning.xattn_splits > 0 ? g_wm_tuning.xattn_splits : ns;
    const bool xshort = mode.xattn_shared && !g_wm_tuning.xattn_never_short;
    int cur = 0;
    auto mean_buf = [&](int i) { return m->dmean + (size_t)i * WM_DEC_MAXB; };
    for (int l = 0; l < D.n_text_layer; ++l) {
        const DecLayerW &L = m->dec[l];
        bf16_t *kc = m->skv + ((size_t)(l * 2 + 0) * Gs + c0) * H * T * 64;
        bf16_t *vc = m->skv + ((size_t)(l * 2 + 1) * Gs + c0) * H * T * 64;
        const bf16_t *xk = m->xkv + ((size_t)(l * 2 + 0) * Gx + c0) * H * S * 64;
        const bf16_t *xv = m->xkv + ((size_t)(l * 2 + 1) * Gx + c0) * H * S * 64;
        DecAttnArgs t = {};
        t.q = m->dq; t.att = m->datt; t.H = H; t.live = mode.stop ? m->dlive : nullptr;
        t.B = B; t.C = Bx; t.N = NC * PW;
        DecGemvArgs a;
        memset(&a, 0, sizeof(a));
        a.epi = DE_QKV; a.B = B; a.N = 3 * d; a.K = d; a.W = L.wqkv_f; a.c1 = L.qkv_c1; a.c2 = L.qkv_c2;
        a.a = m->dxb; a.out_f32 = m->dq; a.kcache = kc; a.vcache = vc;
        a.stats_in = m->dstats;
        a.mean_in = mean_buf(cur); a.mean_out = mean_buf(cur ^ 1); cur ^= 1;
        a.pos_ptr = m->dpos; a.n_ctx = T; a.n_head = H;
        if (PW > 1) { a.epi = DE_QKV_P; a.panel = PW; }
        WM_TRY(wm_dec_gemv(ctx, a));
        t.kc = kc; t.vc = vc; t.T_stride = T; t.n_keys = 0; t.pos_ptr = m->dpos; t.off = mode.off ? m->doff + c0 : nullptr;
        t.pf = {L.wo, d, d};
        WM_TRY(PW > 1 ? wm_dec_self_attention_panel(ctx, t) : wm_dec_self_attention(ctx, t));
        memset(&a, 0, sizeof(a));
        a.epi = DE_RESID; a.B = B; a.N = d; a.K = d; a.W = L.wo; a.c2 = L.bo;
        a.a = m->datt; a.out_f32 = m->dx; a.out_bf16 = m->dxb; a.ldo = d; a.stats_out = m->dstats;
        a.mean_in = mean_buf(cur);
        a.pf_ptr = L.wxq_f; a.pf_rows = d; a.pf_k = d;
        const bool cap_l = cap && cap->layer[l].n > 0;
        const bool fuse_q = NC == 1 && PW == 1 && !cap_l && xns == 1 && wm_dec_xattn_fq_applies(B, H, d, xshort);
        a.pf_head_major = fuse_q ? (H * B + 7) / 8 : 0;
        WM_TRY(wm_dec_gemv(ctx, a));
        memset(&a, 0, sizeof(a));
        a.epi = DE_Q; a.B = B; a.N = d; a.K = d; a.W = L.wxq_f; a.c1 = L.xq_c1; a.c2 = L.xq_c2;
        a.a = m->dxb; a.out_f32 = m->dq; a.ldo = d;
        a.stats_in = m->dstats;
        a.mean_in = mean_buf(cur); a.mean_out = mean_buf(cur ^ 1); cur ^= 1;
        t.kc = xk; t.vc = xv; t.T_stride = S; t.n_keys = S; t.pos_ptr = nullptr; t.off = nullptr;
        t.part = m->dpart; t.nsplit = xns; t.short_lived = xshort; t.pf = {L.wxo, d, d};
        if (fuse_q) {
            WM_TRY(wm_dec_xattn_fq(ctx, a, t));
        } else {
            WM_TRY(wm_dec_gemv(ctx, a));
            if (cap_l) WM_TRY(wm_align_capture_q(ctx, m->dq, d, B, cap->layer[l], cap->q, cap->Tq, cap->J, m->dpos, PW, cap->base));
            WM_TRY(NC > 1 || PW > 1 ? wm_dec_attention_cand(ctx, t) : wm_dec_attention(ctx, t));
        }
        memset(&a, 0, sizeof(a));
        a.epi = DE_RESID; a.B = B; a.N = d; a.K = d; a.W = L.wxo; a.c2 = L.bxo;
        a.a = m->datt; a.out_f32 = m->dx; a.out_bf16 = m->dxb; a.ldo = d; a.stats_out = m->dstats;
        a.mean_in = mean_buf(cur);
        a.pf_ptr = L.w1_f; a.pf_rows = 4 * d; a.pf_k = d;
        WM_TRY(wm_dec_gemv(ctx, a));
        memset(&a, 0, sizeof(a));
        a.epi = DE_GELU; a.B = B; a.N = 4 * d; a.K = d; a.W = L.w1_f; a.c1 = L.fc1_c1; a.c2 = L.fc1_c2;
        a.a = m->dxb; a.out_bf16 = m->dhid; a.ldo = 4 * d;
        a.stats_in = m->dstats;
        a.mean_in = mean_buf(cur); a.mean_out = mean_buf(cur ^ 1); cur ^= 1;
        a.pf_ptr = L.w2; a.pf_rows = d; a.pf_k = 4 * d;
        WM_TRY(wm_dec_gemv(ctx, a));
        memset(&a, 0, sizeof(a));
        a.epi = DE_RESID; a.B = B; a.N = d; a.K = 4 * d; a.W = L.w2; a.c2 = L.b2;
        a.a = m->dhid; a.out_f32 = m->dx; a.out_bf16 = m->dxb; a.ldo = d; a.stats_out = m->dstats;
        a.mean_in = mean_buf(cur);
        if (l + 1 < D.n_text_layer) { a.pf_ptr = m->dec[l + 1].wqkv_f; a.pf_rows = 3 * d; a.pf_k = d; }
        WM_TRY(wm_dec_gemv(ctx, a));
    }
    if (cache_only) return WM_OK;
    {
        DecGemvArgs a;
        memset(&a, 0, sizeof(a));
        a.epi = DE_LOGITS; a.B = B; a.N = D.n_vocab; a.K = d; a.W = m->emb_f; a.c1 = m->logit_c1; a.c2 = m->logit_c2;
        a.a = m->dxb; a.stats_in = m->dstats;
        a.mean_in = mean_buf(cur); a.mean_out = mean_buf(cur ^ 1);
        a.out_f32 = want_logits ? m->dlogits : nullptr; a.ldo = m->vpad;
        a.argmax = m->dargmax; a.arg_first = arg_first; a.arg_last = arg_last;
        if (mode.mask) {
            a.mask = m->dmask; a.mask_words = m->vpad / 32; a.mask_first_pos = n_prompt - 1; a.pos_ptr = m->dpos;
        }
        if (mode.ts) a.ts = wm_model_ts_dev(m);
        if (mode.x) {
            a.epi = DE_LOGITS_X; a.x = wm_model_x_dev(m, mode); a.pos_ptr = m->dpos;
        }
        if (mode.rep) {
            WM_REQUIRE(mode.x, WM_ERR_STATE, "decode step: the repetition rules need the extended decode");
            a.epi = DE_LOGITS_XR; a.rep = wm_model_rep_dev(m, mode);
            WM_TRY(wm_repeat_state(ctx, m->dseq, m->dpos, B, n_prompt, D.n_text_ctx, D.n_vocab, a.rep));
        }
        if (mode.sb) {
            WM_REQUIRE(mode.rep, WM_ERR_STATE, "decode step: the sequence bias needs the repetition-rule state");
            const WmSbDev sb = wm_model_sb_dev(m, mode);
            a.epi = DE_LOGITS_XB; a.sb = sb.e;
            if (mode.sbt)
// ... 176 lines not shown
```

openai-whisper-coreml_amd/csrc/model.h:

```cpp
#pragma once
#include "wm_internal.h"
#include "dec_launch.h"
#include "tx_pending.h"

struct EncLayerW {
    float *ln1_g, *ln1_b;
    bf16_t *wqkv;
    float *bqkv;
    bf16_t *wo;
    float *bo;
    float *ln2_g, *ln2_b;
    bf16_t *w1;
    float *b1;
    bf16_t *w2;
    float *b2;
};
struct DecLayerW {
    float *ln1_g, *ln1_b;
    bf16_t *wqkv;
    float *bqkv;
    bf16_t *wo;
    float *bo;
    float *lnx_g, *lnx_b;
    bf16_t *wxq;
// ... 197 lines not shown
    int N, n_ctx;
    const int *budget;
    float *sum;
    int *src;
    int *list_n;
    int *list_tok;
    float *list_lp;
    int *wdone;
    int *wsteps;
    int *fin_n;
    int *fin_len;
    float *fin_sum;
    int *fin_tok;
    float *fin_lp;
    float *trace;
    int *anc;
    int *fin_src;
};

struct WmAlignLayer {
    int n = 0, slot0 = 0;
    int head[32] = {};
};
struct WmAlignCap {
    const WmAlignLayer *layer;
    float *q;
    int Tq, J;
    int base = -1;
};
struct WmAlignDev {
    const float *q;
    const bf16_t *xkv;
    const int *hl, *hh;
    const int *n_text;
    const int *n_frames;
    float *rowst;
    float *colst;
    float *x;
    int B, H, Tq, J, S, n_ld;
    float sc;
    int half;
    int tail = 1, n_min = 1;
};

struct WmDecodeMode {
    bool mask = false;
    bool ts = false;
    bool x = false;
    bool off = false;
    bool stop = false;
    bool budget = false;
    int stop_eot = -1;
    bool xattn_shared = false;
    int n_cand = 1;
    int beam = 0;
    bool rep = false;
    bool sb = false;
    bool sbt = false;
    bool cst = false;
    bool trunc = false;
    bool alt = false;
    bool given = false;
    bool srows = false;
    int panel = 1;
    bool acap = false;
    int acap_base = 0, acap_Tq = 0, acap_J = 0;
    float *acap_q = nullptr;
    bool operator==(const WmDecodeMode &o) const {
        return acap == o.acap && acap_base == o.acap_base && acap_Tq == o.acap_Tq && acap_J == o.acap_J && acap_q == o.acap_q && panel == o.panel && trunc == o.trunc && alt == o.alt && given == o.given && srows == o.srows && rep == o.rep && sb == o.sb && sbt == o.sbt && cst == o.cst && n_cand == o.n_cand && beam == o.beam && mask == o.mask && ts == o.ts && x == o.x && off == o.off && stop == o.stop && budget == o.budget &&
               stop_eot == o.stop_eot && xattn_shared == o.xattn_shared;
    }
};

struct WmDevBuf {
    void *p = nullptr;
    size_t bytes = 0;
    int reserve(hipStream_t stream, size_t need);
    void release() {
        if (p) (void)hipFree(p);
        p = nullptr; bytes = 0;
    }
};

struct WmGraph {
    hipGraph_t g = nullptr;
    hipGraphExec_t e = nullptr;
    void destroy() {
        if (e) (void)hipGraphExecDestroy(e);
        if (g) (void)hipGraphDestroy(g);
        e = nullptr; g = nullptr;
    }
};

struct WmModel {
    wm_dims dims;
    bool finalized = false;
    bool shares_weights = false;
    int k1pad = 0;
    int vpad = 0;
    bf16_t *conv1_w = nullptr, *conv2_w = nullptr;
    float *conv1_b = nullptr, *conv2_b = nullptr, *enc_pos = nullptr;
    std::vector<EncLayerW> enc;
    float *ln_post_g = nullptr, *ln_post_b = nullptr;
    bf16_t *tok_emb = nullptr;
    float *dec_pos = nullptr;
    std::vector<DecLayerW> dec;
    float *ln_g = nullptr, *ln_b = nullptr;
    bf16_t *emb_f = nullptr;
    float *logit_c1 = nullptr, *logit_c2 = nullptr;
    std::vector<void *> allocs;
    std::vector<WmTensor> tensors;
    std::map<std::string, int> index;
    int cap_b = 0;
    int cap_rows = 0;
    bf16_t *mel_t = nullptr;
    bf16_t *h1p = nullptr;
    float *x = nullptr;
    bf16_t *xn = nullptr;
    bf16_t *qk = nullptr;
    bf16_t *vt = nullptr;
    bf16_t *att = nullptr;
    bf16_t *hid = nullptr;
    float *xa_f32 = nullptr;
    float *mel_f32 = nullptr;
    bf16_t *xkv = nullptr;
    bf16_t *skv = nullptr;
    float *dx = nullptr;
    bf16_t *dxb = nullptr;
    float *dmean = nullptr;
    float *dq = nullptr;
    float *dpart = nullptr;
    float *dstats = nullptr;
    bf16_t *datt = nullptr;
    bf16_t *dhid = nullptr;
    float *dlogits = nullptr;
    unsigned long long *dargmax = nullptr;
    int *dresult = nullptr;
    int *dseq = nullptr;
    int *dpos = nullptr;
    int *doff = nullptr;
    int *darrive = nullptr;
    int *ddone = nullptr, *dbudget = nullptr, *dlive = nullptr, *dnlive = nullptr;
    int *h_nlive = nullptr;
    WmPending pending;
    struct GraphSet {
        int B = 0, n_prompt = 0, cap_b = 0;
        WmDecodeMode mode;
        int burst[2] = {0, 0};
        WmGraph g1[2], gk[2];
        int bburst[2] = {0, 0};
        WmGraph b1[2], bk[2];
        void destroy() {
            for (int i = 0; i < 2; ++i) { g1[i].destroy(); gk[i].destroy(); b1[i].destroy(); bk[i].destroy(); }
        }
        unsigned long stamp = 0;
    };
    struct LidGraph {
        int B = 0, cap_b = 0, first = 0, last = 0, logits = 0;
        WmGraph graph;
        void destroy() { graph.destroy(); B = 0; }
    } lid_graph;
    std::vector<int32_t> lid_host;
    static constexpr int kMaxGraphSets = 4;
    std::vector<GraphSet> graph_sets;
    unsigned long graph_clock = 0;
    unsigned *dmask = nullptr;
    bool mask_on = false;
    std::vector<unsigned> mask_host;
    bool ts_on = false;
    int ts_begin = 0, ts_eot = 0, ts_max_initial = -1;
    int *dts_rng = nullptr, *dts_hist = nullptr;
    unsigned long long *dts_key = nullptr;
    float *dts_lse = nullptr;
    float *dx_txt = nullptr, *dx_win = nullptr, *dx_all = nullptr, *dx_nsv = nullptr;
    float *dx_logprob = nullptr;
    float *dx_nospeech = nullptr;
    WmXPar *dx_par = nullptr;
    bool rep_on = false;
    float rep_p = 1.f;
    int rep_n = 0, rep_eot = 0;
    unsigned *drep_seen = nullptr, *drep_ban = nullptr;
    WmRepPar *drep_par = nullptr;
    int samp_k = 0;
    float samp_p = 1.f, samp_minp = 0.f;
    bool samp_on() const { return samp_k > 0 || samp_p < 1.f || samp_minp > 0.f; }
    WmSampPar *dsamp_par = nullptr;
    WmAltPar *dalt_par = nullptr;
    WmDevBuf alt_ws;
    WmGivenPar *dgiven_par = nullptr;
    WmDevBuf given_ws;
    int *dgiven_side = nullptr;
    bool sb_on = false;
    int sb_groups = 0, sb_entries = 0;
    WmSbDev dsb = {};
    bool sbt_on = false;
    int sbt_groups = 0, sbt_entries = 0;
    std::vector<int32_t> sbt_tab_grp;
    WmSbDev dsbt = {};
    int *dsb_rng = nullptr;
    bool cst_on = false;
    int cst_states = 0, cst_edges = 0, cst_eot = 0;
    WmCstDev dcst = {};
    unsigned *dx_ids = nullptr;
    WmMelWin *dmel_win = nullptr;
    int *dxkv_rows = nullptr;
    std::vector<int32_t> align_l, align_h;
    WmDevBuf align_ws;
    WmDevBuf acap_ws;
    int teacher_panel = 1;
    int prompt_panel = 1;
    int last_prefill[3] = {0, 0, 0};
    int given_panel = 1;
    int last_given_panel[4] = {0, 0, 0, 0};
    WmDevBuf beam_ws;
    WmDevBuf beam_trace;
    bool beam_trace_on = false;
    WmDevBuf spec_ws;
    int *h_spec = nullptr;
    WmDevBuf pcm_stage;
    WmDevBuf io_stage;
};

struct wm_windows {
    int device = 0;
    wm_dims dims = {};
    const void *weights = nullptr;
    int W = 0;
    std::vector<int32_t> n_frames;
    bf16_t *store = nullptr;
    size_t bytes = 0;
};

int wm_model_create(wm_ctx *ctx, const wm_dims *dims);
void wm_model_destroy(wm_ctx *ctx);
int wm_model_clone(wm_ctx *child, const wm_ctx *parent);
int wm_model_reserve(wm_ctx *ctx, int B);
int wm_model_reserve_rows(wm_ctx *ctx, int rows);
int wm_model_set_tensor(wm_ctx *ctx, const char *name, const float *data, size_t n);
int wm_model_get_tensor(wm_ctx *ctx, const char *name, float *data, size_t n);
int wm_model_init_synthetic(wm_ctx *ctx, uint64_t seed, float matrix_gain);
int wm_model_finalize(wm_ctx *ctx);
int wm_model_encode_dev(wm_ctx *ctx, const float *d_mel, int B, float *d_xa_out );
int wm_model_encode_win(wm_ctx *ctx, const float *d_mel, const WmMelWin *d_win, int B, float *d_xa_out );
int wm_model_encode_stem(wm_ctx *ctx, const float *d_mel, const WmMelWin *d_win, int B);
int wm_model_encode_layer_qkv(wm_ctx *ctx, int layer, int B);
int wm_model_encode_layer_tail(wm_ctx *ctx, int layer, int B, float *d_x_mid );
int wm_model_encode_post(wm_ctx *ctx, int B, float *d_xa_out );
int wm_model_cross_kv(wm_ctx *ctx, int B);
int wm_model_set_xa(wm_ctx *ctx, const float *d_xa, int B);
int wm_model_decode_begin(wm_ctx *ctx, int B);
int wm_model_decode_step(wm_ctx *ctx, int B, bool want_logits, int arg_first, int arg_last, const WmAlignCap *cap = nullptr,
                         const WmDecodeMode &mode = WmDecodeMode(), int n_prompt = 0);
WmXDev wm_model_x_dev(const WmModel *m, const WmDecodeMode &mode);
WmTsDev wm_model_ts_dev(const WmModel *m);
WmRepDev wm_model_rep_dev(const WmModel *m, const WmDecodeMode &mode);
int wm_model_set_repetition_rules(wm_ctx *ctx, float penalty, int ngram, int32_t eot);
int wm_model_set_sampling_rules(wm_ctx *ctx, int top_k, float top_p, float min_p);
int wm_model_sample_truncate(wm_ctx *ctx, int B, int n_prompt, const WmDecodeMode &mode);
int wm_model_alt_begin(wm_ctx *ctx, int rows, int max_new, int n, WmAltPar *host_par);
int wm_model_alternatives(wm_ctx *ctx, int B, int n_prompt, const WmDecodeMode &mode);
int wm_model_given_begin(wm_ctx *ctx, int rows, int stride, const int32_t *lens, const int32_t *tok, WmGivenPar *host_par);
int wm_model_given_tokens(wm_ctx *ctx, int B, int n_prompt, const WmDecodeMode &mode);
WmSbDev wm_model_sb_dev(const WmModel *m, const WmDecodeMode &mode);
int wm_model_set_sequence_bias(wm_ctx *ctx, const WmSbTable &t);
int wm_model_set_sequence_bias_tables(wm_ctx *ctx, const WmSbPool &p);
int wm_model_set_constraint(wm_ctx *ctx, const WmCstTable &t);
int wm_model_set_timestamp_rules(wm_ctx *ctx, int enable, int32_t ts_begin, int32_t eot, int32_t max_initial);
int wm_model_set_suppress(wm_ctx *ctx, const int32_t *ids, int n, const int32_t *first_ids, int n_first);
struct WmSpecDev {
    int *tseq, *dseq;
    int *tpos, *dpos;
    WmTsDev tts, dts;
    int *chist, *crng;
    int *dchist, *dcrng;
    int *wtok;
    float *wlp;
    int *acc;
    int *stats;
    int *round;
    const int *script;
    int max_new, n_vocab;
};
int wm_model_spec_panel_step(wm_ctx *ctx, int G, int w, const WmDecodeMode &mode, int n_prompt);
int wm_model_spec_dev(wm_ctx *ctx, wm_ctx *draft, int max_new, WmSpecDev *out, int **script_area);
int wm_spec_adopt(wm_ctx *draft, const WmSpecDev &sp, int G, int n_prompt);
int wm_spec_stage(wm_ctx *ctx, const WmSpecDev &sp, int G, int w, int n_prompt, int n_ctx);
int wm_spec_accept(wm_ctx *ctx, const unsigned long long *tilemax, int n_tiles, const WmSpecDev &sp, const WmXDev &xd,
                   const WmStopDev &stop, int G, int w, int n_prompt, int n_ctx, int fallback_tok);
int wm_spec_commit(wm_ctx *ctx, const WmSpecDev &sp, const WmXDev &xd, const WmStopDev &stop, int G, int w, int n_prompt, int n_ctx);
int wm_model_prompt_prefill(wm_ctx *ctx, int G, int P0, const WmDecodeMode &mode);
struct WmGivenPanelDev;
int wm_model_given_panel_phase(wm_ctx *ctx, int G, int w, int Lp, int n_prompt, int max_new, const WmDecodeMode &mode);
int wm_model_given_panel_dev(wm_ctx *ctx, int max_new, WmGivenPanelDev *out);
int wm_model_embed_first(wm_ctx *ctx, int B, const WmDecodeMode &mode = WmDecodeMode());
int wm_model_close_step(wm_ctx *ctx, int B, int n_prompt, bool write_seq, int *result, int arg_first,
                        const WmDecodeMode &mode = WmDecodeMode());
WmStopDev wm_model_stop_dev(const WmModel *m, const WmDecodeMode &mode);
WmEmbedDev wm_model_embed_dev(const WmModel *m);
int wm_model_beam_dev(wm_ctx *ctx, const WmDecodeMode &mode, WmBeamDev *out);
int wm_model_beam_begin(wm_ctx *ctx, const WmDecodeMode &mode, int rows, int windows, const WmBeamPar *par, const int32_t *budgets);
int wm_model_beam_close(wm_ctx *ctx, int B, int n_prompt, const WmDecodeMode &mode);
// ... 56 lines not shown
    int stats_parts;
    float *stats_out;
    const float *mean_in;
    float *mean_out;
    float *out_f32;
    bf16_t *out_bf16;
    bf16_t *kcache, *vcache;
    const int *pos_ptr;
    int n_ctx, n_head;
    long ldo;
    unsigned long long *argmax;
    int arg_first, arg_last;
    const unsigned *mask;
    int mask_words, mask_first_pos;
    WmTsDev ts;
    WmXDev x;
    const bf16_t *pf_ptr;
    int pf_rows, pf_k;
    int pf_head_major;
    WmRepDev rep;
    WmSbEpi sb;
    int panel;
};
int wm_dec_gemv(wm_ctx *ctx, const DecGemvArgs &a);
bool wm_dec_xattn_fq_applies(int B, int H, int K, bool short_lived);
struct DecAttnArgs;
int wm_dec_xattn_fq(wm_ctx *ctx, const DecGemvArgs &qa, const DecAttnArgs &t);
int wm_ln_fold(wm_ctx *ctx, const bf16_t *W, const float *g, const float *beta, const float *bias , int N,
               int K, bf16_t *Wf, float *c1, float *c2);
int wm_dec_embed(wm_ctx *ctx, const int *seq, const int *pos_ptr, int B, const WmEmbedDev &e, const int *off);
int wm_dec_embed_panel(wm_ctx *ctx, const int *seq, int seq_stride, const int *pos_ptr, int pos_add, int C, int w, int n_ctx,
                       const WmEmbedDev &e, const int *off = nullptr);
int wm_dec_pos_add(wm_ctx *ctx, int *pos_ptr, int add);
struct DecWarm {
    const bf16_t *ptr;
    int rows, k;
};
struct DecAttnArgs {
    const float *q;
    const bf16_t *kc, *vc;
    bf16_t *att;
    float *part;
    int B;
    int C, N;
    int H;
    int T_stride;
    int n_keys;
    const int *pos_ptr;
    int nsplit;
    const int *live;
    const int *off;
    DecWarm pf;
    bool short_lived;
};
int wm_dec_attn_splits(int B, int H);
int wm_dec_attention(wm_ctx *ctx, const DecAttnArgs &t);
int wm_dec_attention_cand(wm_ctx *ctx, const DecAttnArgs &t);
int wm_dec_self_attention(wm_ctx *ctx, const DecAttnArgs &t);
int wm_dec_self_attention_panel(wm_ctx *ctx, const DecAttnArgs &t);
int wm_argmax_embed(wm_ctx *ctx, const unsigned long long *tilemax, int n_tiles, int B, int *seq, int *pos_ptr,
                    int n_prompt, int *result, int arg_first, int n_ctx, const WmEmbedDev &e, const WmTsDev &ts, int *arrive,
                    int fallback_tok, const WmStopDev &stop, const WmXDev &xd, const int *off);
int wm_sample_noise(wm_ctx *ctx, uint64_t seed, int chunk, int gi, int n0, int count, float *out);
int wm_stop_init(wm_ctx *ctx, const WmStopDev &stop, int B);
int wm_ts_init(wm_ctx *ctx, const WmTsDev &ts, int B);
int wm_range_softmax(wm_ctx *ctx, const float *logits, long ldo, int B, int first, int n, float *probs);
int wm_fill_synthetic(wm_ctx *ctx, const WmTensor &t, uint32_t seed, int tensor_id, float gain);

struct WmStoredRows {
    const float *logits;
    long ldo;
    int n_vocab;
    unsigned long long *tilemax;
    int rows;
    WmTsDev ts;
    WmXDev xd;
    const unsigned *mask;
    int mask_words, n_prompt;
    const int *pos_ptr;
    WmStopDev stop;
    const unsigned *ban;
    int ban_words;
};
inline int wm_stored_rows_check(const WmStoredRows &r, const char *who, bool needs_win) {
    WM_REQUIRE(r.rows >= 1 && r.rows <= WM_DEC_MAXB && r.logits && r.tilemax && r.xd.par && r.xd.txt && (!needs_win || r.xd.win) && r.pos_ptr,
               WM_ERR_INVALID, "%s: bad group", who);
    WM_REQUIRE(r.n_vocab >= 1 && r.ldo >= r.n_vocab, WM_ERR_INVALID, "%s: %d ids in rows of %ld", who, r.n_vocab, r.ldo);
    WM_REQUIRE(!r.mask || (long)r.mask_words * 32 >= r.n_vocab, WM_ERR_INVALID, "%s: %d mask words do not cover %d ids", who, r.mask_words,
               r.n_vocab);
    WM_REQUIRE(!r.ban || (long)r.ban_words * 32 >= r.n_vocab, WM_ERR_INVALID, "%s: %d ban words do not cover %d ids", who, r.ban_words,
               r.n_vocab);
    WM_REQUIRE(!r.ts.rng || (r.ts.key_ts && r.ts.lse && r.ts.ts_begin >= 0), WM_ERR_INVALID, "%s: incomplete timestamp-rule state", who);
    return WM_OK;
}
inline int wm_panel_shape_check(int G, int w, const char *what) {
    WM_REQUIRE(G >= 1 && w >= 1 && w <= WM_MAX_TEACHER_PANEL && G * w <= WM_DEC_MAXB, WM_ERR_INVALID, "%s: %d windows x %d rows", what, G, w);
    return WM_OK;
}

int wm_beam_topk(wm_ctx *ctx, const WmStoredRows &rows, const WmBeamDev &bm);
int wm_beam_select_step(wm_ctx *ctx, int rows, int *seq, int *pos_ptr, int n_prompt, const WmEmbedDev &e, const WmTsDev &ts,
                        const WmStopDev &stop, const WmXDev &xd, const int *off, const WmBeamDev &bm);
int wm_beam_reorder(wm_ctx *ctx, bf16_t *skv, int L2, int rows, int H, int T, const int *pos_ptr, int n_prompt, int *seq,
                    float *logprob, const WmBeamDev &bm);

int wm_sample_truncate(wm_ctx *ctx, const WmStoredRows &rows, const WmSampPar *par, int *dbg);

int wm_alternatives(wm_ctx *ctx, const WmStoredRows &rows, const WmAltPar *par);

int wm_given_tokens(wm_ctx *ctx, const WmStoredRows &rows, const WmGivenPar *par);

struct WmGivenPanelDev {
    int *seq;
    int *pos;
    WmTsDev ts;
    int *chist, *crng;
    int *wtok;
    float *wlp;
    const WmGivenPar *par;
    int max_new, n_vocab;
};
int wm_given_panel_stage(wm_ctx *ctx, const WmGivenPanelDev &gp, const WmStopDev &stop, int G, int w, int n_prompt, int n_ctx, bool first);
int wm_given_panel_close(wm_ctx *ctx, const WmStoredRows &rows, const WmGivenPanelDev &gp, int G, int w, int fallback_tok, bool last);
int wm_given_panel_commit(wm_ctx *ctx, const WmGivenPanelDev &gp, const WmXDev &xd, const WmStopDev &stop, int G, int w, int n_prompt,
                          bool last);

int wm_repeat_state(wm_ctx *ctx, const int *seq, const int *pos_ptr, int B, int n_prompt, int n_ctx, int V, const WmRepDev &rep);

int wm_seqbias_state(wm_ctx *ctx, const int *seq, const int *pos_ptr, int B, int n_prompt, int n_ctx, int V, const WmSbDev &sb,
                     unsigned *ban, int ban_words);
int wm_constraint_state(wm_ctx *ctx, const int *seq, const int *pos_ptr, int B, int n_prompt, int n_ctx, int V, const WmCstDev &cst,
                        unsigned *ban, int ban_words, int *state_out);
int wm_seqbias_rows_state(wm_ctx *ctx, const int *seq, const int *pos_ptr, int B, int n_prompt, int n_ctx, int V, const WmSbDev &pool,
                          const int *rng, unsigned *ban, int ban_words);

int wm_xkv_rows(wm_ctx *ctx, bf16_t *group, long group_rows, bf16_t *store, const int *d_rows, int row0, int n_rows, int L2,
                long slab, bool to_store);

int wm_align_capture_q(wm_ctx *ctx, const float *dq, int d, int B, const WmAlignLayer &L, float *cap, int Tq, int J,
                       const int *pos_ptr, int panel = 1, int base = -1);
int wm_align_token_prob(wm_ctx *ctx, const float *logits, long ldo, const int *seq, const int *pos_ptr, int B, int S, int eot,
                        const int *n_text, float *prob, int max_text, int panel = 1, int seq_stride = 0);
constexpr size_t WM_ALIGN_CAPTURE_BUDGET = (size_t)2 << 30;
inline size_t wm_align_chunk_bytes(size_t T, size_t J, size_t n_ld) { return T * J * (64 * 4 + 8) + J * 1500 * 8 + n_ld * 1500 * 4; }
inline int wm_align_group_rows(size_t T, size_t J, size_t n_ld) {
    const size_t g = WM_ALIGN_CAPTURE_BUDGET / wm_align_chunk_bytes(T, J, n_ld);
    return (int)(g < 1 ? 1 : (g > (size_t)WM_DEC_MAXB ? (size_t)WM_DEC_MAXB : g));
}
inline size_t wm_align_window_bytes(size_t T, size_t J, size_t n_ld, size_t N) {
    return wm_align_chunk_bytes(T, J, n_ld) + (N > 1 ? (N * T * J * 64 + T) * 4 : 0);
}
inline int wm_align_group_windows(size_t T, size_t J, size_t n_ld, size_t N) {
    const size_t g = WM_ALIGN_CAPTURE_BUDGET / wm_align_window_bytes(T, J, n_ld, N), c_max = (size_t)WM_DEC_MAXB / N;
    return (int)(g < 1 ? 1 : (g > c_max ? c_max : g));
}
int wm_align_gather(wm_ctx *ctx, const float *cap, float *q_sel, const int *slot, const int *n_rows, int C, int N, int Tq, int J);
void wm_align_heads(const WmModel *m, std::vector<int32_t> *hl, std::vector<int32_t> *hh);
int wm_align_matrix(wm_ctx *ctx, const WmAlignDev &a, int max_n, int max_m);
size_t wm_dtw_trace_words(int max_rows);
int wm_dtw(wm_ctx *ctx, const float *x, long x_bstride, int ld, const int *N, const int *M, int B, int max_rows, int max_m,
           unsigned *trace, int *start, int n_out);
```

openai-whisper-coreml_amd/csrc/transcribe.cpp:

```cpp
#include <math.h>
#include <stdio.h>
#include <stdlib.h>
#include <string.h>
#include <unistd.h>

#include <algorithm>
#include <cmath>
#include <vector>

#include "beam.h"
#include "call_src.h"
#include "model.h"
#include "tx_plan.h"


namespace {
int lane_limit() {
    static const int n = [] {
        const char *e = getenv("WM_LANES");
        const int v = e ? atoi(e) : 3;
        return v < 1 ? 1 : (v > 8 ? 8 : v);
    }();
    return n;
}
// ... 195 lines not shown
            WM_HIP(hipMemcpyAsync((void *)wm_x_rows(m->dx_ids), j.samp.data(), j.samp.size() * sizeof(WmXRow), hipMemcpyHostToDevice, c->stream));
        }
        WM_HIP(hipMemcpyAsync(m->dx_par, &j.xpar, sizeof(WmXPar), hipMemcpyHostToDevice, c->stream));
    }

    if (j.mode.rep) {
        WM_REQUIRE(xc.on, WM_ERR_STATE, "the repetition rules need the extended decode");
        j.rpar.p = m->rep_p; j.rpar.inv_p = (float)(1.0 / (double)m->rep_p); j.rpar.n = m->rep_n; j.rpar.eot = m->rep_eot;
        if (!m->rep_on) { j.rpar.p = 1.f; j.rpar.inv_p = 1.f; j.rpar.n = 0; j.rpar.eot = 0; }
        WM_HIP(hipMemcpyAsync(m->drep_par, &j.rpar, sizeof(WmRepPar), hipMemcpyHostToDevice, c->stream));
    }
    if (j.mode.trunc) {
        j.spar.top_k = m->samp_k; j.spar.top_p = m->samp_p; j.spar.min_p = m->samp_minp;
        WM_HIP(hipMemcpyAsync(m->dsamp_par, &j.spar, sizeof(WmSampPar), hipMemcpyHostToDevice, c->stream));
    }
    if (j.mode.alt) {
        WM_REQUIRE(xc.on, WM_ERR_STATE, "alternatives need the extended decode");
        WM_TRY(wm_model_alt_begin(c, Bg, call.max_new, pend.alt.n, &j.apar));
    }
    if (j.mode.given) {
        WM_REQUIRE(xc.on, WM_ERR_STATE, "given tokens need the extended decode");
        WM_TRY(wm_model_given_begin(c, Bg, given_L, j.tab.glen.data(), j.tab.gtok.data(), &j.gpar));
    }
    if (j.mode.sbt) {
        WM_REQUIRE(!pend.bias_rows.empty(), WM_ERR_STATE, "sequence-bias tables are in force and the call has no row map (wm_set_bias_rows)");
        wm_group_bias_rows(pend.bias_rows.data(), m->sbt_tab_grp.data(), (int)m->sbt_tab_grp.size() - 1, j.b0, Cg, N, &j.tab.sbr);
        WM_HIP(hipMemcpyAsync(m->dsb_rng, j.tab.sbr.data(), j.tab.sbr.size() * 4, hipMemcpyHostToDevice, c->stream));
    } else if (j.mode.sb) {
        j.sbpar.n_groups = m->sb_groups; j.sbpar.n_entries = m->sb_entries;
        WM_HIP(hipMemcpyAsync((void *)m->dsb.par, &j.sbpar, sizeof(WmSbPar), hipMemcpyHostToDevice, c->stream));
    }
    if (j.mode.cst) {
        j.cpar.n_states = m->cst_states; j.cpar.n_edges = m->cst_edges; j.cpar.eot = m->cst_eot;
        j.cstart.resize(Bg);
        for (int r = 0; r < Bg; ++r) j.cstart[r] = pend.cst_rows.empty() ? 0 : pend.cst_rows[j.b0 + r / N];
        WM_HIP(hipMemcpyAsync((void *)m->dcst.par, &j.cpar, sizeof(WmCstPar), hipMemcpyHostToDevice, c->stream));
        WM_HIP(hipMemcpyAsync((void *)m->dcst.start, j.cstart.data(), (size_t)Bg * 4, hipMemcpyHostToDevice, c->stream));
    }
    WM_TRY(wm_model_reserve(c, Cg));
    if (N > 1) WM_TRY(wm_model_reserve_rows(c, Bg));
    if (call.beam) {
        j.bbud.resize(Cg);
        for (int w = 0; w < Cg; ++w) j.bbud[w] = stop_budget(stop, j.b0 + w, j.bpar.max_new);
        m->beam_trace_on = call.dbg.beam_trace != nullptr;
        if (call.dbg.beam_trace) {
            const size_t bytes = (size_t)j.bpar.max_new * Bg * WM_BEAM_TRACE * 4;
            WM_TRY(m->beam_trace.reserve(c->stream, bytes));
            WM_HIP(hipMemsetAsync(m->beam_trace.p, 0, bytes, c->stream));
        }
        WM_TRY(wm_model_beam_begin(c, j.mode, Bg, Cg, &j.bpar, j.bbud.data()));
    }
    WM_HIP(hipEventRecord(j.ev[0], c->stream));
    WM_TRY(wm_stage_cross_kv(c, call.src, j.b0, Cg, call.mem, d_pcm, j.win, j.xrows, j.ev[1]));

    WM_HIP(hipEventRecord(j.ev[2], c->stream));
    WM_TRY(wm_model_embed_first(c, Bg, j.mode));
    if (j.mode.ts) WM_TRY(wm_ts_init(c, wm_model_ts_dev(m), Bg));
    return WM_OK;
}

int lane_prompt_panels(LaneJob &j, const TxCall &call, const wm_ctx *caller) {
    WmModel *m = j.c->model;
    if (m->prompt_panel <= 1 || call.n_cand != 1 || call.beam || caller->dbg_hooks) return WM_OK;
    WmPromptPanelPlan pl;
    wm_prompt_panel_plan(j.Bg, m->prompt_panel, j.P, j.mode.x ? j.xpar.sot_pos : -1, j.mode.acap ? j.mode.acap_base : -1,
                         g_wm_tuning.teacher_panel_cut, &pl);
    if (pl.w < 1) return WM_OK;
    WM_TRY(wm_model_prompt_prefill(j.c, j.Bg, pl.P0, j.mode));
    j.t = pl.P0;
    return WM_OK;
}

void lane_given_plan(LaneJob &j, const TxCall &call, const wm_ctx *caller) {
    const WmModel *m = j.c->model;
    const WmDecodeMode &md = j.mode;
    unsigned bits = 0;
    if (md.given) bits |= WM_GPB_GIVEN;
    if (call.n_cand != 1 || call.beam) bits |= WM_GPB_CAND;
    if (md.off) bits |= WM_GPB_OFF;
    if (md.x) bits |= WM_GPB_X;
    if (md.srows) bits |= WM_GPB_SROWS;
    if (md.trunc) bits |= WM_GPB_TRUNC;
    if (md.x && j.xpar.sample) bits |= WM_GPB_SAMPLE;
    if (md.alt) bits |= WM_GPB_ALT;
    if (md.sbt) bits |= WM_GPB_SBT;
    if (md.sb) bits |= WM_GPB_SB;
    if (md.cst) bits |= WM_GPB_CST;
    if (md.rep) bits |= WM_GPB_REP;
    if (md.acap) bits |= WM_GPB_ACAP;
    if (call.f32_path || caller->dbg_hooks) bits |= WM_GPB_F32;
    wm_given_panel_plan(j.Bg, m->given_panel, md.given ? j.tab.glen.data() : nullptr, md.budget ? j.tab.bud.data() : nullptr, call.max_new,
                        j.P, m->dims.n_text_ctx, bits, &j.gplan);
}

int lane_given_panels(LaneJob &j, int max_new, const WmDecodeMode &mode) {
    const WmGivenPanelPlan pl = j.gplan;
    j.gplan = WmGivenPanelPlan();
    WM_TRY(wm_model_given_panel_phase(j.c, j.Bg, pl.w, pl.Lp, j.P, max_new, mode));
    j.t = j.P + pl.Lp - 1;
    return WM_OK;
}

int lane_position(LaneJob &j, const WmDecodeMode &mode, int n_prompt, bool gen) {
    WmAlignCap cap = {j.alayers.data(), mode.acap_q, mode.acap_Tq, mode.acap_J, mode.acap_base};
    WM_TRY(wm_model_decode_step(j.c, j.Bg, gen || mode.trunc || mode.alt || mode.given, 0, j.c->model->dims.n_vocab - 1, mode.acap ? &cap : nullptr, mode, n_prompt));
    if (gen) return wm_model_beam_close(j.c, j.Bg, n_prompt, mode);
// ... 71 lines not shown
    WmBeamDev bm;
    (void)wm_model_beam_dev(j.c, j.mode, &bm);
    const char *dev0 = (const char *)j.c->model->beam_ws.p;
    auto host = [&](const void *dev) { return j.bstate.data() + ((const char *)dev - dev0); };
    const float *sum = (const float *)host(bm.sum), *fin_sum = (const float *)host(bm.fin_sum);
    const int *fin_n = (const int *)host(bm.fin_n), *fin_len = (const int *)host(bm.fin_len), *wsteps = (const int *)host(bm.wsteps);
    for (int w = 0; w < j.Cg; ++w) {
        const int W = j.b0 + w;
        int n_hyp = 0;
        auto put = [&](const int32_t *tok, size_t tok_stride, const float *lp, size_t lp_stride, int len, float s) {
            const size_t o = (size_t)W * S + n_hyp++;
            for (int i = 0; i < max_new; ++i) {
                tokens_out[o * max_new + i] = i < len ? tok[(size_t)i * tok_stride] : eot;
                if (logprobs_out) logprobs_out[o * max_new + i] = i < len ? lp[(size_t)i * lp_stride] : 0.f;
            }
            lens_out[o] = len;
            call.sums[o] = s;
        };
        for (int f = 0; f < fin_n[w]; ++f) {
            const size_t base = ((size_t)w * WM_MAX_BEAM_HYPS + f) * n_ctx;
            put(j.bfin_tok.data() + base, 1, j.bfin_lp.data() + base, 1, fin_len[w * WM_MAX_BEAM_HYPS + f], fin_sum[w * WM_MAX_BEAM_HYPS + f]);
        }
        if (n_hyp < N) {
            int order[WM_MAX_BEAM];
            const int n_live = wm_beam_fill_order(N, sum + (size_t)w * N, order);
            for (int k = 0; k < n_live && n_hyp < N; ++k) {
                const int b = w * N + order[k];
                put(j.gen.data() + b, j.Bg, j.lp.data() + b, j.Bg, wsteps[w], sum[b]);
            }
        }
        call.n_hyp[W] = n_hyp;
        for (int h = n_hyp; h < S; ++h) {
            const size_t o = (size_t)W * S + h;
            for (int i = 0; i < max_new; ++i) {
                tokens_out[o * max_new + i] = eot;
                if (logprobs_out) logprobs_out[o * max_new + i] = 0.f;
            }
            lens_out[o] = 0;
            call.sums[o] = -INFINITY;
        }
        if (no_speech_out) no_speech_out[W] = j.ns[(size_t)w * N];
        if (call.dbg.beam_trace)
            for (int gi = 0; gi < max_new; ++gi)
                memcpy(call.dbg.beam_trace + (((size_t)W * max_new + gi) * N) * WM_BEAM_TRACE,
                       j.btrace.data() + ((size_t)gi * j.Bg + (size_t)w * N) * WM_BEAM_TRACE, (size_t)N * WM_BEAM_TRACE * 4);
    }
}

int lane_burst(LaneJob &j, int n_prompt, int n_steps, bool use_graph, bool shared) {
    wm_ctx *c = j.c;
    WmModel *m = c->model;
    const int K = burst_len();
    const bool gen = j.mode.beam && j.t >= n_prompt - 1;
    const int sh = shared ? 1 : 0;
    WmDecodeMode mode = j.mode;
    mode.xattn_shared = shared;
    const bool phase = j.gplan.reason == WM_GP_SERVED;
    if (phase && j.t == n_prompt) {
        WM_TRY(lane_given_panels(j, n_steps - n_prompt + 1, mode));
    } else {
        const int left = (j.mode.beam && !gen ? n_prompt - 1 : (phase ? n_prompt : n_steps)) - j.t;
        const int k = left < K ? left : K;
        WmModel::GraphSet *g = use_graph ? &m->graph_sets[j.gset] : nullptr;
        WmGraph *g1 = g ? (gen ? g->b1 : g->g1) : nullptr, *gk = g ? (gen ? g->bk : g->gk) : nullptr;
        int *burst = g ? (gen ? g->bburst : g->burst) : nullptr;
        if (use_graph && k == K && K > 1) {
            if (!gk[sh].e || burst[sh] != K) {
                WM_TRY(capture_positions(j, mode, n_prompt, K, gen, &gk[sh]));
                burst[sh] = K;
            }
            WM_HIP(hipGraphLaunch(gk[sh].e, c->stream));
        } else {
            if (use_graph && !g1[sh].e) WM_TRY(capture_positions(j, mode, n_prompt, 1, gen, &g1[sh]));
            for (int i = 0; i < k; ++i) {
                if (use_graph) {
                    WM_HIP(hipGraphLaunch(g1[sh].e, c->stream));
                } else {
                    WM_TRY(lane_position(j, mode, n_prompt, gen));
                }
            }
        }
        j.t += k;
    }
    if (j.mode.stop) {
        const int slot = j.bursts % WM_NLIVE_RING;
        WM_HIP(hipMemcpyAsync(m->h_nlive + slot, m->dnlive, sizeof(int), hipMemcpyDeviceToHost, c->stream));
        WM_HIP(hipEventRecord(j.burst_ev[slot], c->stream));
    }
    ++j.bursts;
    return WM_OK;
}
int entry_checks(const TxCall &call) {
    const TxPrompts &p = call.prompts;
    switch (call.entry) {
    case TxCall::PLAIN:
        break;
    case TxCall::MEL:
    case TxCall::RAGGED:
        WM_REQUIRE(call.src.mel && call.src.mel_base && call.src.mel_len && call.src.seek && call.src.n_frames, WM_ERR_INVALID,
                   "null mel / window pointer");
        if (call.entry == TxCall::MEL) break;
        WM_REQUIRE(p.len, WM_ERR_INVALID, "null prompt_len");
        WM_REQUIRE(p.stride >= 1, WM_ERR_INVALID, "prompt_stride %d < 1", p.stride);
        break;
    case TxCall::BEST_OF:
    case TxCall::BEAM:
        WM_TRY(wm_check_src_pointers(call.src));
        if (call.beam) WM_REQUIRE(call.n_hyp && call.sums, WM_ERR_INVALID, "null n_hyp_out / sum_logprobs_out");
        WM_REQUIRE(p.stride >= 1, WM_ERR_INVALID, "prompt_stride %d < 1", p.stride);
        if (call.beam) {
            WM_REQUIRE(call.n_cand >= 1 && call.n_cand <= WM_MAX_BEAM, WM_ERR_INVALID, "beam_size %d outside [1, %d]", call.n_cand,
// ... 919 lines not shown
```

openai-whisper-coreml_amd/csrc/wm_tuning.h:

```cpp
#pragma once
struct WmTuning {
    int gemv_tn = 0;
    int gemv_nblk = 0;
    int gemv_ppw2_nblk = 0;
    int gemv_no_ppw2 = 0;
    int prefetch_max_b = 16;
    int xattn_split_below = 96;
    int xattn_wgs = 256;
    int xattn_no_flat = 0;
    int xattn_lds_pad = 84 * 1024;
    int xattn_splits = 0;
    int gemm_tile = 0;
    int gemm_gm = 4;
    int gemm128_pipe = 0;
    int no_early_stop = 0;
    int logits_tn = 0;
    int enc_attn_mfma_sum = 0;
    int xattn_never_short = 0;
    int xattn_no_deep = 0;
    int xattn_fuse_q = 1;
    int argmax_rows_per_wg = 0;
    int group_chunks = 0;
    int frontend_per_wave_twiddles = 0;
    int lane_parts = 0;
    int teacher_panel_cut = 0;
    int spec_group = 0;
    int lane_solo_cus = 0;
};
```

Before: 2183.

## Pack cross-attention KV cache into 12-bit rows with per-row exponent base

Adds a lossless packing of bf16 cross-attention K/V rows into 96-byte rows (12-bit codes relative to a per-row exponent base, with an escape for rows whose exponent range is too wide), plus a packed decoder cross-attention kernel that unpacks on the fly. The aim is to cut HBM traffic for the bandwidth-bound cross-attention during decode. It adds a pack pass per window set, graph variants keyed on the packed mode, state tracking for invalidation when xkv is rewritten, and debug and bench hooks. Packing is gated by a new tuning knob, xkv_pack, whose default is 0.

```diff
diff --git a/include/whisper_mi355x_debug.h b/include/whisper_mi355x_debug.h
--- a/include/whisper_mi355x_debug.h
+++ b/include/whisper_mi355x_debug.h
@@ -151,6 +151,11 @@
     int32_t plan[16];
 } wmdbg_attn;
 WM_API int wmdbg_dec_attention_form(wm_ctx *ctx, wmdbg_attn *io);
+WM_API int wmdbg_dec_attention_form_packed(wm_ctx *ctx, wmdbg_attn *io, int planes, int32_t *escaped);
+WM_API int wmdbg_xkv_pack_rows(const uint16_t *rows, int n, uint8_t *packed, uint8_t *bases);
+WM_API int wmdbg_xkv_unpack_rows(const uint8_t *packed, const uint8_t *bases, int n, uint16_t *rows);
+WM_API int wmdbg_xkv_base_slot(int i);
+WM_API int wmdbg_xkv_state(wm_ctx *ctx, int32_t *out6);
 WM_API int wmdbg_attn_layout(int32_t *out4);
 
 WM_API int wmdbg_dec_self_attention_panel(wm_ctx *ctx, const float *q, const float *k, const float *v, int C, int w, int H,
@@ -210,6 +215,8 @@
                          int nw_override, float *avg_us);
 WM_API int wmdbg_bench_dec_attention(wm_ctx *ctx, int B, int H, int T, int n_keys, int nsplit, int n_slices,
                               int iters, float *avg_us);
+WM_API int wmdbg_bench_dec_attention_packed(wm_ctx *ctx, int B, int H, int T, int n_keys, int n_slices, int iters, int planes,
+                                            int short_lived, float *avg_us, float *pack_us);
 
 WM_API int wmdbg_bench_launch_floor(wm_ctx *ctx, int iters, int grid, float *eager_us, float *graph_us);
 
diff --git a/openai-whisper-coreml_amd/csrc/call_src.cpp b/openai-whisper-coreml_amd/csrc/call_src.cpp
--- a/openai-whisper-coreml_amd/csrc/call_src.cpp
+++ b/openai-whisper-coreml_amd/csrc/call_src.cpp
@@ -86,6 +86,7 @@
         map.resize(Bg);
         for (int b = 0; b < Bg; ++b) map[b] = a.rows ? a.rows[b0 + b] : b0 + b;
         WM_HIP(hipMemcpyAsync(m->dxkv_rows, map.data(), (size_t)Bg * 4, hipMemcpyHostToDevice, c->stream));
+        wm_model_xkv_written(m);
         WM_TRY(wm_xkv_rows(c, m->xkv, Bg, a.set->store, m->dxkv_rows, 0, Bg, 2 * D.n_text_layer, (long)D.n_text_head * 1500 * 64,
                            false));
         if (staged) WM_HIP(hipEventRecord(staged, c->stream));
diff --git a/openai-whisper-coreml_amd/csrc/debug_hooks.cpp b/openai-whisper-coreml_amd/csrc/debug_hooks.cpp
--- a/openai-whisper-coreml_amd/csrc/debug_hooks.cpp
+++ b/openai-whisper-coreml_amd/csrc/debug_hooks.cpp
@@ -12,6 +12,7 @@
 #include "beam.h"
 #include "model.h"
 #include "tx_plan.h"
+#include "xkv_pack.h"
 
 namespace {
 struct DevPool {
@@ -221,7 +222,7 @@
         {"xattn_lds_pad", &g_wm_tuning.xattn_lds_pad}, {"xattn_splits", &g_wm_tuning.xattn_splits},
         {"gemm_tile", &g_wm_tuning.gemm_tile}, {"gemm128_pipe", &g_wm_tuning.gemm128_pipe}, {"gemm_gm", &g_wm_tuning.gemm_gm}, {"no_early_stop", &g_wm_tuning.no_early_stop},
         {"xattn_no_deep", &g_wm_tuning.xattn_no_deep}, {"xattn_never_short", &g_wm_tuning.xattn_never_short},         {"logits_tn", &g_wm_tuning.logits_tn}, {"enc_attn_mfma_sum", &g_wm_tuning.enc_attn_mfma_sum},
-        {"group_chunks", &g_wm_tuning.group_chunks}, {"argmax_rows_per_wg", &g_wm_tuning.argmax_rows_per_wg}, {"xattn_fuse_q", &g_wm_tuning.xattn_fuse_q},
+        {"group_chunks", &g_wm_tuning.group_chunks}, {"argmax_rows_per_wg", &g_wm_tuning.argmax_rows_per_wg}, {"xattn_fuse_q", &g_wm_tuning.xattn_fuse_q}, {"xkv_pack", &g_wm_tuning.xkv_pack},
         {"teacher_panel_cut", &g_wm_tuning.teacher_panel_cut}, {"lane_parts", &g_wm_tuning.lane_parts}, {"lane_solo_cus", &g_wm_tuning.lane_solo_cus}, {"spec_group", &g_wm_tuning.spec_group}, {"frontend_per_wave_twiddles", &g_wm_tuning.frontend_per_wave_twiddles},
     };
     if (strcmp(key, "reset") == 0) { g_wm_tuning = WmTuning(); return WM_OK; }
@@ -777,9 +778,12 @@
     return WM_OK;
 }
 
-extern "C" int wmdbg_dec_attention_form(wm_ctx *ctx, wmdbg_attn *io) {
+static int dec_attention_form(wm_ctx *ctx, wmdbg_attn *io, int planes, int32_t *escaped) {
     WM_TRY(wm_ctx_make_current(ctx));
     WM_REQUIRE(io && io->out && io->k && io->v, WM_ERR_INVALID, "dec_attention_form: null pointer");
+    WM_REQUIRE(planes >= 0 && planes <= 3 && (planes == 0 || (io->form == 0 && escaped)), WM_ERR_INVALID,
+               "dec_attention_form: packed planes %d (form %d)", planes, io->form);
+    if (escaped) escaped[0] = escaped[1] = -1;
     memset(io->plan, 0, sizeof(io->plan));
     const int form = io->form, H = io->H, T = io->T;
     WM_REQUIRE(form >= 0 && form <= 3, WM_ERR_INVALID, "dec_attention_form: form %d is not 0 .. 3", form);
@@ -801,7 +805,7 @@
     pin[0] = form; pin[1] = cand ? 0 : io->B; pin[2] = cand ? io->C : 0; pin[3] = cand ? io->N : 0; pin[4] = H; pin[5] = T;
     pin[6] = io->n_keys; pin[7] = io->nsplit; pin[8] = fq ? io->K : 0;
     pin[9] = (has_pos ? 1 : 0) | (fq || self ? 0 : 2) | (io->off ? 4 : 0) | (has_pf ? 8 : 0) | (io->short_lived ? 16 : 0) | (io->live_rows ? 32 : 0);
-    pin[10] = has_pf ? io->warm_rows : 0; pin[11] = has_pf ? io->warm_k : 0; pin[12] = ctx->n_cus;
+    pin[10] = has_pf ? io->warm_rows : 0; pin[11] = has_pf ? io->warm_k : 0; pin[12] = ctx->n_cus; pin[13] = planes;
     wm_attn_plan_flat(pin, g_wm_tuning, io->plan);
     if (io->plan[0] != WM_OK) return WM_ERR_INVALID;
     WM_REQUIRE(H <= 255 && T >= 1 && T <= WM_ATT_MAXK, WM_ERR_INVALID, "dec_attention_form: H 1 .. 255, T 1 .. %d", WM_ATT_MAXK);
@@ -856,6 +860,19 @@
     if (has_pf) {
         WM_TRY(pool.get(&t.pf.ptr, nullptr, (size_t)io->warm_rows * io->warm_k * 2, s));
         t.pf.rows = io->warm_rows; t.pf.k = io->warm_k;
+    }
+    int *desc = nullptr;
+    if (planes) {
+        const long pairs = (long)entries * H;
+        unsigned char *pk[2] = {nullptr, nullptr}, *bs[2] = {nullptr, nullptr};
+        WM_TRY(pool.get(&desc, nullptr, 2 * sizeof(int), s));
+        for (int pl = 0; pl < 2; ++pl) {
+            if (!((planes >> pl) & 1)) continue;
+            WM_TRY(pool.get(&pk[pl], nullptr, (size_t)pairs * T * XKV_ROW_BYTES, s, 0xff));
+            WM_TRY(pool.get(&bs[pl], nullptr, (size_t)pairs * XKV_SLOTS, s, 0xff));
+            WM_TRY(wm_xkv_pack(ctx, pl ? dv : dk, pairs, T, pairs, pk[pl], bs[pl], desc + pl));
+        }
+        t.packed = planes; t.kpk = pk[0]; t.kbs = bs[0]; t.vpk = pk[1]; t.vbs = bs[1];
     }
     float *dmean_out = nullptr;
     switch (form) {
@@ -891,8 +908,43 @@
         }
     }
     if (dmean_out) WM_HIP(hipMemcpyAsync(io->mean_out, dmean_out, (size_t)rows * 4, hipMemcpyDeviceToHost, s));
+    if (desc) {
+        int32_t n[2] = {0, 0};
+        WM_HIP(hipMemcpyAsync(n, desc, sizeof(n), hipMemcpyDeviceToHost, s));
+        WM_HIP(hipStreamSynchronize(s));
+        for (int pl = 0; pl < 2; ++pl)
+            if ((planes >> pl) & 1) escaped[pl] = n[pl];
+    }
     return down_tiled_bf16(datt, rpad, dd, io->out, s);
 }
+
+extern "C" int wmdbg_dec_attention_form(wm_ctx *ctx, wmdbg_attn *io) { return dec_attention_form(ctx, io, 0, nullptr); }
+extern "C" int wmdbg_dec_attention_form_packed(wm_ctx *ctx, wmdbg_attn *io, int planes, int32_t *escaped) {
+    WM_REQUIRE(planes >= 1 && planes <= 3, WM_ERR_INVALID, "dec_attention_form_packed: planes %d is not 1 (K), 2 (V) or 3 (both)", planes);
+    return dec_attention_form(ctx, io, planes, escaped);
+}
+
+extern "C" int wmdbg_xkv_pack_rows(const uint16_t *rows, int n, uint8_t *packed, uint8_t *bases) {
+    if (!rows || !packed || !bases || n < 0) return WM_ERR_INVALID;
+    for (int i = 0; i < n; ++i) bases[i] = (uint8_t)xkv_pack_row(rows + (size_t)i * XKV_ROW_VALUES, packed + (size_t)i * XKV_ROW_BYTES);
+    return WM_OK;
+}
+extern "C" int wmdbg_xkv_unpack_rows(const uint8_t *packed, const uint8_t *bases, int n, uint16_t *rows) {
+    if (!rows || !packed || !bases || n < 0) return WM_ERR_INVALID;
+    for (int i = 0; i < n; ++i) {
+        if (!bases[i]) return WM_ERR_INVALID;
+        xkv_unpack_row(packed + (size_t)i * XKV_ROW_BYTES, bases[i], rows + (size_t)i * XKV_ROW_VALUES);
+    }
+    return WM_OK;
+}
+extern "C" int wmdbg_xkv_state(wm_ctx *ctx, int32_t *out6) {
+    WM_REQUIRE(ctx && ctx->model && out6, WM_ERR_INVALID, "xkv_state: null pointer / no model");
+    const WmModel *m = ctx->model;
+    out6[0] = m->xpk_valid; out6[1] = m->xpk_planes; out6[2] = m->h_xpk_esc ? m->h_xpk_esc[0] : -1; out6[3] = m->h_xpk_esc ? m->h_xpk_esc[1] : -1;
+    out6[4] = m->xpk_b; out6[5] = (int32_t)m->xpk_bursts;
+    return WM_OK;
+}
+extern "C" int wmdbg_xkv_base_slot(int i) { return i >= 0 && i < XKV_SLOTS ? xkv_base_slot(i) : -1; }
 
 
 extern "C" int wmdbg_bench_dec_gemv(wm_ctx *ctx, int B, int N, int K, int ln, int resid, int n_mats, int iters,
@@ -934,9 +986,11 @@
     return WM_OK;
 }
 
-extern "C" int wmdbg_bench_dec_attention(wm_ctx *ctx, int B, int H, int T, int n_keys, int nsplit, int n_slices,
-                                         int iters, float *avg_us) {
-    WM_TRY(wm_ctx_make_current(ctx));
+static int bench_dec_attention(wm_ctx *ctx, int B, int H, int T, int n_keys, int nsplit, int n_slices, int iters, int planes,
+                               bool short_lived, float *avg_us, float *pack_us) {
+    WM_TRY(wm_ctx_make_current(ctx));
+    WM_REQUIRE(B >= 1 && B <= WM_DEC_MAXB && H >= 1 && T >= 1 && T <= WM_ATT_MAXK && n_slices >= 1 && iters >= 1 && avg_us, WM_ERR_INVALID,
+               "bench_dec_attention: bad arguments");
     DevPool pool;
     hipStream_t s = ctx->stream;
     const size_t slice = (size_t)B * H * T * 64;
@@ -944,20 +998,46 @@
     const float *dq;
     float *dp;
     bf16_t *datt;
-    WM_TRY(pool.get(&dk, nullptr, slice * n_slices * 2, s));
-    WM_TRY(pool.get(&dv, nullptr, slice * n_slices * 2, s));
+    WM_TRY(pool.get(&dk, nullptr, slice * n_slices * 2, s, planes ? 0x3c : 0));
+    WM_TRY(pool.get(&dv, nullptr, slice * n_slices * 2, s, planes ? 0x3c : 0));
+    unsigned char *pk[2] = {nullptr, nullptr}, *bs[2] = {nullptr, nullptr};
+    int *desc = nullptr;
+    const long pairs = (long)B * H;
+    const size_t pslice = (size_t)pairs * T * XKV_ROW_BYTES, bslice = (size_t)pairs * XKV_SLOTS;
+    if (planes) {
+        WM_TRY(pool.get(&desc, nullptr, 2 * sizeof(int), s));
+        EventPair pev;
+        WM_TRY(pev.init());
+        for (int pl = 0; pl < 2; ++pl) {
+            if (!((planes >> pl) & 1)) continue;
+            WM_TRY(pool.get(&pk[pl], nullptr, pslice * n_slices, s));
+            WM_TRY(pool.get(&bs[pl], nullptr, bslice * n_slices, s));
+            for (int i = 0; i < n_slices; ++i) {
+                const bool timed = i == n_slices - 1 && pack_us;
+                if (timed) WM_TRY(pev.start(s));
+                WM_TRY(wm_xkv_pack(ctx, (pl ? dv : dk) + (size_t)i * slice, pairs, T, pairs, pk[pl] + (size_t)i * pslice,
+                                   bs[pl] + (size_t)i * bslice, desc + pl));
+                if (timed) WM_TRY(pev.stop_us(s, pack_us));
+            }
+        }
+    }
     WM_TRY(pool.get(&dq, nullptr, (size_t)B * H * 64 * 4, s));
     WM_TRY(pool.get(&dp, nullptr, (size_t)B * H * WM_MAXSPLIT * 66 * 4, s));
     WM_TRY(pool.get(&datt, nullptr, ((size_t)B + 15) / 16 * 16 * H * 64 * 2, s));
     EventPair ev;
     WM_TRY(ev.init());
     DecAttnArgs t = {};
-    t.q = dq; t.att = datt; t.part = dp; t.B = B; t.H = H; t.T_stride = T; t.n_keys = n_keys; t.nsplit = nsplit;
+    t.q = dq; t.att = datt; t.part = dp; t.B = B; t.H = H; t.T_stride = T; t.n_keys = n_keys; t.nsplit = nsplit; t.short_lived = short_lived;
     for (int pass = 0; pass < 2; ++pass) {
         if (pass == 1) WM_TRY(ev.start(s));
         for (int i = 0; i < iters; ++i) {
             t.kc = dk + (size_t)(i % n_slices) * slice;
             t.vc = dv + (size_t)(i % n_slices) * slice;
+            if (planes) {
+                t.packed = planes;
+                t.kpk = pk[0] ? pk[0] + (size_t)(i % n_slices) * pslice : nullptr; t.kbs = bs[0] ? bs[0] + (size_t)(i % n_slices) * bslice : nullptr;
+                t.vpk = pk[1] ? pk[1] + (size_t)(i % n_slices) * pslice : nullptr; t.vbs = bs[1] ? bs[1] + (size_t)(i % n_slices) * bslice : nullptr;
+            }
             WM_TRY(wm_dec_attention(ctx, t));
         }
     }
@@ -965,6 +1045,16 @@
     WM_TRY(ev.stop_us(s, &us));
     *avg_us = us / iters;
     return WM_OK;
+}
+
+extern "C" int wmdbg_bench_dec_attention(wm_ctx *ctx, int B, int H, int T, int n_keys, int nsplit, int n_slices,
+                                         int iters, float *avg_us) {
+    return bench_dec_attention(ctx, B, H, T, n_keys, nsplit, n_slices, iters, 0, false, avg_us, nullptr);
+}
+extern "C" int wmdbg_bench_dec_attention_packed(wm_ctx *ctx, int B, int H, int T, int n_keys, int n_slices, int iters, int planes,
+                                                int short_lived, float *avg_us, float *pack_us) {
+    WM_REQUIRE(planes >= 0 && planes <= 3, WM_ERR_INVALID, "bench_dec_attention_packed: planes %d", planes);
+    return bench_dec_attention(ctx, B, H, T, n_keys, 1, n_slices, iters, planes, short_lived != 0, avg_us, pack_us);
 }
 
 int wm_launch_trivial(wm_ctx *ctx, int *p, int grid);
@@ -1655,6 +1745,7 @@
     hipStream_t s = ctx->stream;
     const int *drows;
     WM_TRY(pool.get(&drows, rows, (size_t)n_rows * 4, s));
+    if (!to_store && ctx->model) wm_model_xkv_written(ctx->model);
     int rc = wm_xkv_rows(ctx, group, group_rows, store, drows, 0, n_rows, 2 * L, (long)H * 1500 * 64, to_store != 0);
     if (hipStreamSynchronize(s) != hipSuccess && rc == WM_OK) {
         wm_set_error("xkv_rows: %s", hipGetErrorString(hipGetLastError()));
@@ -3125,6 +3216,7 @@
     hipStream_t s = ctx->stream;
     const float *dxa;
     WM_TRY(pool.get(&dxa, xa, M * d * 4, s));
+    wm_model_xkv_written(m);
     WM_HIP(hipMemcpyAsync(m->xkv, s16.data(), cap * 2, hipMemcpyHostToDevice, s));
     int rc = wm_model_set_xa(ctx, dxa, B);
     if (rc == WM_OK) rc = wm_model_cross_kv(ctx, B);
diff --git a/openai-whisper-coreml_amd/csrc/dec_kernels.hip b/openai-whisper-coreml_amd/csrc/dec_kernels.hip
--- a/openai-whisper-coreml_amd/csrc/dec_kernels.hip
+++ b/openai-whisper-coreml_amd/csrc/dec_kernels.hip
@@ -6,6 +6,7 @@
 #include "dec_close.h"
 #include "model.h"
 #include "philox.h"
+#include "xkv_pack.h"
 
 namespace {
 
@@ -1115,6 +1116,135 @@
     }
 }
 
+struct AttnColdPk {
+    const unsigned char *kpk, *vpk;
+    const unsigned char *kbs, *vbs;
+    bf16_t *att;
+    const char *pf_ptr;
+    long pf_tile_bytes;
+};
+typedef __attribute__((ext_vector_type(3))) unsigned u32x3;
+typedef u32x3 u32x3_a4 __attribute__((aligned(4)));
+
+template <bool NT>
+__device__ __forceinline__ void attn_load_row_pk(const bf16_t *pb, const unsigned char *pp, int i, unsigned base, u32x4 &x) {
+    if (base) {
+        const u32x3_a4 *p = (const u32x3_a4 *)(pp + (long)i * XKV_ROW_BYTES);
+        const u32x3 t = NT ? __builtin_nontemporal_load(p) : *p;
+        x = u32x4{t.x, t.y, t.z, 0u};
+    } else {
+        x = NT ? __builtin_nontemporal_load((const u32x4 *)(pb + (long)i * 64)) : *(const u32x4 *)(pb + (long)i * 64);
+    }
+}
+__device__ __forceinline__ void attn_unpack_row_pk(unsigned base, u32x4 &x) {
+    uint32_t v[4];
+    xkv_unpack_lane(x[0], x[1], x[2], (int)base, v);
+    x = u32x4{v[0], v[1], v[2], v[3]};
+}
+
+template <int NS, int U, bool NT, bool KP, bool VP>
+__global__ __launch_bounds__(NS * 64) void dec_xrows_attn_pk_kernel(
+    const float *__restrict__ q, const bf16_t *__restrict__ kc, const bf16_t *__restrict__ vc,
+    const int *__restrict__ live_rows , unsigned packA ,
+    unsigned packB , unsigned packC , AttnColdPk cold) {
+    static_assert(U == 4 && NS == 8, "a block's base bytes are one dword: 4 loads, 64 lane groups");
+    const int H = (int)(packA & 0xffu);
+    const int T_stride = (int)(packB & 0xffffu), n_keys = (int)(packB >> 16);
+    int n_bh = (int)(packC & 0xffffu);
+    const int n_wg = (int)(packC >> 16);
+    const int d = H * 64;
+    if ((int)blockIdx.x >= n_wg) {
+        l2_warm_tile(cold.pf_ptr, cold.pf_tile_bytes, (int)blockIdx.x - n_wg, blockDim.x);
+        return;
+    }
+    if (live_rows) n_bh = live_rows[WM_DEC_MAXB] * H;
+    __shared__ float wm_[NS], wl_[NS];
+    __shared__ float wo_[NS][64];
+    const int tid = threadIdx.x, lane = tid & 63, wave = tid >> 6;
+    const int rg = lane >> 3, e8 = lane & 7;
+    const int last = n_keys - 1;
+    const int stream = wave;
+    for (int pi = blockIdx.x; pi < n_bh; pi += n_wg) {
+        if (pi != (int)blockIdx.x) __syncthreads();
+        const int h = pi % H;
+        const int b = live_rows ? live_rows[pi / H] : pi / H;
+        const int bh = b * H + h;
+        const bf16_t *kb = kc + (long)bh * T_stride * 64 + e8 * 8;
+        const bf16_t *vb = vc + (long)bh * T_stride * 64 + e8 * 8;
+        const unsigned char *kp = cold.kpk + (long)bh * T_stride * XKV_ROW_BYTES + e8 * XKV_LANE_BYTES;
+        const unsigned char *vp = cold.vpk + (long)bh * T_stride * XKV_ROW_BYTES + e8 * XKV_LANE_BYTES;
+        const unsigned *kbw = (const unsigned *)(cold.kbs + (long)bh * XKV_SLOTS) + stream * 8 + rg;
+        const unsigned *vbw = (const unsigned *)(cold.vbs + (long)bh * XKV_SLOTS) + stream * 8 + rg;
+        float qe[8];
+        attn_scale_query(q + (long)b * d + h * 64 + e8 * 8, qe);
+        float m_run = -1e30f, l_run = 0.f;
+        float oa[8] = {0, 0, 0, 0, 0, 0, 0, 0};
+        unsigned kb_next = KP ? kbw[0] : 0u, vb_next = VP ? vbw[0] : 0u;
+        for (int r0 = 0; r0 < n_keys; r0 += NS * 8 * U) {
+            const unsigned kb4 = kb_next, vb4 = vb_next;
+            unsigned kbase[U], vbase[U];
+            int row[U];
+            u32x4 kv[U], vv[U];
+            bool esc = false;
+#pragma unroll
+            for (int u = 0; u < U; ++u) {
+                const int i = r0 + u * (NS * 8) + stream * 8 + rg;
+                const bool in = i < n_keys;
+                row[u] = in ? i : last;
+                kbase[u] = KP ? (in ? (kb4 >> (8 * u)) & 0xffu : 1u) : 0u;
+                vbase[u] = VP ? (in ? (vb4 >> (8 * u)) & 0xffu : 1u) : 0u;
+                esc = esc || (KP && kbase[u] == 0u) || (VP && vbase[u] == 0u);
+            }
+            const bool next = r0 + NS * 8 * U < n_keys;
+            const int nb = (r0 >> 8) + 1;
+            if (__builtin_amdgcn_ballot_w64(esc) == 0) {
+#pragma unroll
+                for (int u = 0; u < U; ++u) {
+                    attn_load_row_pk<NT>(kb, kp, row[u], KP ? 1u : 0u, kv[u]);
+                    attn_load_row_pk<NT>(vb, vp, row[u], VP ? 1u : 0u, vv[u]);
+                }
+                if (next) {
+                    if (KP) kb_next = kbw[nb * 64];
+                    if (VP) vb_next = vbw[nb * 64];
+                }
+#pragma unroll
+                for (int u = 0; u < U; ++u) {
+                    if (KP) attn_unpack_row_pk(kbase[u], kv[u]);
+                    if (VP) attn_unpack_row_pk(vbase[u], vv[u]);
+                }
+            } else {
+#pragma unroll
+                for (int u = 0; u < U; ++u) {
+                    attn_load_row_pk<NT>(kb, kp, row[u], kbase[u], kv[u]);
+                    attn_load_row_pk<NT>(vb, vp, row[u], vbase[u], vv[u]);
+                }
+                if (next) {
+                    if (KP) kb_next = kbw[nb * 64];
+                    if (VP) vb_next = vbw[nb * 64];
+                }
+#pragma unroll
+                for (int u = 0; u < U; ++u) {
+                    if (kbase[u]) attn_unpack_row_pk(kbase[u], kv[u]);
+                    if (vbase[u]) attn_unpack_row_pk(vbase[u], vv[u]);
+                }
+            }
+            attn_block<NS, U, false>(qe, r0, stream, rg, n_keys, kv, vv, m_run, l_run, oa);
+        }
+        attn_stream_reduce(l_run, oa);
+        if (rg == 0) {
+#pragma unroll
+            for (int i = 0; i < 8; ++i) wo_[wave][e8 * 8 + i] = oa[i];
+            if (e8 == 0) {
+                wm_[wave] = m_run;
+                wl_[wave] = l_run;
+            }
+        }
+        __syncthreads();
+        if (tid < 64)
+            cold.att[wm_tiled_offset((size_t)b, (size_t)(h * 64 + tid), (size_t)d)] = f2bf(attn_merge<NS>(wm_, wl_, &wo_[0][0], 64, tid));
+    }
+}
+
 struct CandLive {
     int r_lo, r_hi;
     unsigned long long head_lo, head_hi;
@@ -1741,6 +1871,7 @@
     s.B = t.B; s.C = t.C; s.N = t.N; s.H = t.H; s.T_stride = t.T_stride; s.n_keys = t.n_keys; s.nsplit = t.nsplit;
     s.has_pos = t.pos_ptr != nullptr; s.has_part = t.part != nullptr; s.has_off = t.off != nullptr; s.short_lived = t.short_lived;
     s.has_pf = t.pf.ptr != nullptr; s.pf_rows = t.pf.rows; s.pf_k = t.pf.k;
+    s.packed = t.packed;
     return s;
 }
 int launch_combine(wm_ctx *ctx, const DecAttnArgs &t, const DecAttnPlan &pl);
@@ -1752,7 +1883,31 @@
     {
         WmProfScope ps(&ctx->prof, "dec_attn_cross", ctx->stream);
         const dim3 grid(pl.grid_x, pl.grid_y);
-        if (pl.variant == DAV_STREAM) {
+        if (pl.variant == DAV_STREAM_PK) {
+            WM_REQUIRE(t.kc && t.vc && (!(t.packed & 1) || (t.kpk && t.kbs)) && (!(t.packed & 2) || (t.vpk && t.vbs)), WM_ERR_INVALID,
+                       "dec_attention: packed planes missing");
+            const AttnColdPk cold = {t.kpk, t.vpk, t.kbs, t.vbs, t.att, (const char *)t.pf.ptr, pl.tile_bytes};
+            const int lds_pad = g_wm_tuning.xattn_lds_pad;
+            static std::atomic<int> pk_pad_set[64];
+#define WM_XPK_LAUNCH(KP, VP)                                                                                                   \
+    do {                                                                                                                        \
+        if (lds_pad > pk_pad_set[ctx->device & 63].load(std::memory_order_acquire)) {                                           \
+            WM_HIP(hipFuncSetAttribute((const void *)dec_xrows_attn_pk_kernel<8, 4, WM_XATTN_NT, true, false>,                   \
+                                       hipFuncAttributeMaxDynamicSharedMemorySize, lds_pad));                                   \
+            WM_HIP(hipFuncSetAttribute((const void *)dec_xrows_attn_pk_kernel<8, 4, WM_XATTN_NT, false, true>,                   \
+                                       hipFuncAttributeMaxDynamicSharedMemorySize, lds_pad));                                   \
+            WM_HIP(hipFuncSetAttribute((const void *)dec_xrows_attn_pk_kernel<8, 4, WM_XATTN_NT, true, true>,                    \
+                                       hipFuncAttributeMaxDynamicSharedMemorySize, lds_pad));                                   \
+            pk_pad_set[ctx->device & 63].store(lds_pad, std::memory_order_release);                                             \
+        }                                                                                                                       \
+        dec_xrows_attn_pk_kernel<8, 4, WM_XATTN_NT, KP, VP><<<grid, pl.block, pl.lds, ctx->stream>>>(                            \
+            t.q, t.kc, t.vc, t.live, pl.w.a, pl.w.b, pl.w.c, cold);                                                             \
+    } while (0)
+            if ((t.packed & 3) == 1) WM_XPK_LAUNCH(true, false);
+            else if ((t.packed & 3) == 2) WM_XPK_LAUNCH(false, true);
+            else WM_XPK_LAUNCH(true, true);
+#undef WM_XPK_LAUNCH
+        } else if (pl.variant == DAV_STREAM) {
             const int lds_pad = g_wm_tuning.xattn_lds_pad;
             static std::atomic<int> pad_set[64];
             if (lds_pad > pad_set[ctx->device & 63].load(std::memory_order_acquire)) {
diff --git a/openai-whisper-coreml_amd/csrc/dec_launch.cpp b/openai-whisper-coreml_amd/csrc/dec_launch.cpp
--- a/openai-whisper-coreml_amd/csrc/dec_launch.cpp
+++ b/openai-whisper-coreml_amd/csrc/dec_launch.cpp
@@ -139,7 +139,7 @@
         const int n_wg = wm_dec_persistent_wgs(B * H, n_cus, s.short_lived, t);
         p->warm_tiles = wm_dec_warm_tiles(B, s.has_pf && nsplit == 1, s.pf_rows, s.pf_k, n_wg, t, &p->tile_bytes);
         ok = wm_pack_attn_rows(H, nsplit, 0, B * H, n_wg, &p->w.a, &p->w.c) && ok;
-        p->variant = DAV_STREAM;
+        p->variant = (s.packed & 3) && nsplit == 1 ? DAV_STREAM_PK : DAV_STREAM;
         p->n_wg = n_wg;
         p->grid_x = n_wg + p->warm_tiles;
         p->grid_y = nsplit;
@@ -354,6 +354,7 @@
     const int f = in[9];
     s.has_pos = f & 1; s.has_part = f & 2; s.has_off = f & 4; s.has_pf = f & 8; s.short_lived = f & 16;
     s.pf_rows = in[10]; s.pf_k = in[11];
+    s.packed = in[13];
     const int n_cus = in[12];
     DecAttnPlan p;
     memset(&p, 0, sizeof(p));
diff --git a/openai-whisper-coreml_amd/csrc/dec_launch.h b/openai-whisper-coreml_amd/csrc/dec_launch.h
--- a/openai-whisper-coreml_amd/csrc/dec_launch.h
+++ b/openai-whisper-coreml_amd/csrc/dec_launch.h
@@ -41,6 +41,7 @@
     DAV_CAND_FLAT = 8,
     DAV_FQ = 9,
     DAV_SELF_OFF_PANEL = 10,
+    DAV_STREAM_PK = 11,
 };
 struct DecAttnShape {
     int B;
@@ -50,6 +51,7 @@
     int K;
     bool has_pos, has_part, has_off, has_pf, short_lived;
     int pf_rows, pf_k;
+    int packed;
 };
 struct DecAttnPlan {
     int variant;
diff --git a/openai-whisper-coreml_amd/csrc/model.cpp b/openai-whisper-coreml_amd/csrc/model.cpp
--- a/openai-whisper-coreml_amd/csrc/model.cpp
+++ b/openai-whisper-coreml_amd/csrc/model.cpp
@@ -1,4 +1,5 @@
 #include "model.h"
+#include "xkv_pack.h"
 #include "tx_plan.h"
 
 #include <math.h>
@@ -690,6 +691,10 @@
     wm_model_drop_graphs(m);
     if (m->h_nlive) (void)hipHostFree(m->h_nlive);
     if (m->h_spec) (void)hipHostFree(m->h_spec);
+    if (m->h_xpk_esc) (void)hipHostFree(m->h_xpk_esc);
+    if (m->xpk_ev) (void)hipEventDestroy(m->xpk_ev);
+    m->xpk.release();
+    m->xbs.release();
     m->spec_ws.release();
     for (void *p : m->allocs) (void)hipFree(p);
     for (WmDevBuf *b : {&m->pcm_stage, &m->io_stage, &m->align_ws, &m->acap_ws, &m->beam_ws, &m->beam_trace, &m->alt_ws, &m->given_ws})
@@ -829,6 +834,7 @@
     WM_REQUIRE(m, WM_ERR_STATE, "context has no model");
     if (B <= m->cap_b) return WM_OK;
     WM_HIP(hipStreamSynchronize(ctx->stream));
+    wm_model_xkv_written(m);
     void *olds[] = {m->mel_t, m->h1p, m->x, m->xn, m->qk, m->vt, m->att, m->hid, m->xa_f32, m->mel_f32, m->xkv, m->skv};
     for (void *p : olds)
         if (p) {
@@ -975,6 +981,7 @@
     WmModel *m = ctx->model;
     const wm_dims &D = m->dims;
     const int d = D.n_text_state, H = D.n_text_head, S = 1500, M = B * S;
+    wm_model_xkv_written(m);
     for (int l = 0; l < D.n_text_layer; ++l) {
         const DecLayerW &L = m->dec[l];
         GemmArgs g = plain_gemm(m->xn, d, L.wxkv, L.bxkv, m->xkv + (size_t)l * 2 * B * H * S * 64, 0, M, 2 * d, d,
@@ -983,6 +990,65 @@
         WM_TRY(wm_gemm(ctx, g));
     }
     return WM_OK;
+}
+
+void wm_model_xkv_written(WmModel *m) {
+    m->xpk_valid = false;
+    m->xpk_planes = 0;
+}
+
+int wm_model_xkv_pack(wm_ctx *ctx, int B) {
+    WmModel *m = ctx->model;
+    const wm_dims &D = m->dims;
+    const int H = D.n_text_head, S = 1500, planes = g_wm_tuning.xkv_pack & 3;
+    wm_model_xkv_written(m);
+    const int xns = g_wm_tuning.xattn_splits > 0 ? g_wm_tuning.xattn_splits : wm_dec_attn_splits(B, H);
+    if (!planes || xns != 1 || B > WM_DEC_MAXB) return WM_OK;
+    const size_t pairs = (size_t)D.n_text_layer * 2 * B * H;
+    const size_t need_pk = pairs * S * XKV_ROW_BYTES, need_bs = pairs * XKV_SLOTS;
+    if (m->xpk.bytes < need_pk || m->xbs.bytes < need_bs) {
+        size_t free_b = 0, total_b = 0;
+        WM_HIP(hipMemGetInfo(&free_b, &total_b));
+        if (free_b + m->xpk.bytes + m->xbs.bytes < 2 * (need_pk + need_bs)) return WM_OK;
+        wm_model_drop_graphs(m);
+        m->xpk_b = 0;
+        WM_TRY(m->xpk.reserve(ctx->stream, need_pk));
+        WM_TRY(m->xbs.reserve(ctx->stream, need_bs));
+    }
+    if (!m->dxpk_esc) WM_TRY(dalloc_t(m, &m->dxpk_esc, 2, ctx->stream));
+    if (!m->h_xpk_esc) WM_HIP(hipHostMalloc((void **)&m->h_xpk_esc, 2 * sizeof(int), hipHostMallocDefault));
+    if (!m->xpk_ev) WM_HIP(hipEventCreateWithFlags(&m->xpk_ev, hipEventDisableTiming));
+    WM_HIP(hipMemsetAsync(m->dxpk_esc, 0, 2 * sizeof(int), ctx->stream));
+    if (planes == 3) {
+        WM_TRY(wm_xkv_pack(ctx, m->xkv, (long)pairs, S, (long)B * H, (unsigned char *)m->xpk.p, (unsigned char *)m->xbs.p, m->dxpk_esc));
+    } else {
+        const int pl = planes == 2 ? 1 : 0;
+        for (int l = 0; l < D.n_text_layer; ++l) {
+            const size_t p0 = (size_t)(l * 2 + pl) * B * H;
+            WM_TRY(wm_xkv_pack(ctx, m->xkv + p0 * S * 64, (long)B * H, S, (long)B * H, (unsigned char *)m->xpk.p + p0 * S * XKV_ROW_BYTES,
+                               (unsigned char *)m->xbs.p + p0 * XKV_SLOTS, m->dxpk_esc + pl));
+        }
+    }
+    WM_HIP(hipMemcpyAsync(m->h_xpk_esc, m->dxpk_esc, 2 * sizeof(int), hipMemcpyDeviceToHost, ctx->stream));
+    WM_HIP(hipEventRecord(m->xpk_ev, ctx->stream));
+    m->xpk_b = B;
+    m->xpk_valid = true;
+    m->xpk_planes = -1;
+    return WM_OK;
+}
+
+int wm_model_xkv_planes(wm_ctx *ctx, int B) {
+    WmModel *m = ctx->model;
+    if (!m->xpk_valid || m->xpk_b != B) return 0;
+    if (m->xpk_planes < 0) {
+        if (g_wm_tuning.xkv_pack & 4) (void)hipEventSynchronize(m->xpk_ev);
+        const hipError_t q = hipEventQuery(m->xpk_ev);
+        if (q != hipSuccess) { (void)hipGetLastError(); return 0; }
+        const long rows = (long)m->dims.n_text_layer * B * m->dims.n_text_head * 1500;
+        const int want = g_wm_tuning.xkv_pack & 3;
+        m->xpk_planes = (m->h_xpk_esc[0] * 8L < rows ? want & 1 : 0) | (m->h_xpk_esc[1] * 8L < rows ? want & 2 : 0);
+    }
+    return m->xpk_planes;
 }
 
 int wm_model_decode_begin(wm_ctx *ctx, int B) {
@@ -1019,6 +1085,8 @@
     const int ns = wm_dec_attn_splits(B, H);
     const int xns = g_wm_tuning.xattn_splits > 0 ? g_wm_tuning.xattn_splits : ns;
     const bool xshort = mode.xattn_shared && !g_wm_tuning.xattn_never_short;
+    const int xpk = NC == 1 && PW == 1 ? mode.xpk & 3 : 0;
+    WM_REQUIRE(!xpk || (m->xpk_valid && m->xpk_b == B && grp == 0), WM_ERR_STATE, "decode step: no valid 12-bit copy of the cross-attention cache");
     int cur = 0;
     auto mean_buf = [&](int i) { return m->dmean + (size_t)i * WM_DEC_MAXB; };
     for (int l = 0; l < D.n_text_layer; ++l) {
@@ -1058,6 +1126,13 @@
         a.mean_in = mean_buf(cur); a.mean_out = mean_buf(cur ^ 1); cur ^= 1;
         t.kc = xk; t.vc = xv; t.T_stride = S; t.n_keys = S; t.pos_ptr = nullptr; t.off = nullptr;
         t.part = m->dpart; t.nsplit = xns; t.short_lived = xshort; t.pf = {L.wxo, d, d};
+        if (xpk) {
+            const size_t pk0 = ((size_t)(l * 2 + 0) * Gx + c0) * H, pv0 = ((size_t)(l * 2 + 1) * Gx + c0) * H;
+            const unsigned char *pk = (const unsigned char *)m->xpk.p, *bs = (const unsigned char *)m->xbs.p;
+            t.packed = xpk;
+            t.kpk = pk + pk0 * S * XKV_ROW_BYTES; t.kbs = bs + pk0 * XKV_SLOTS;
+            t.vpk = pk + pv0 * S * XKV_ROW_BYTES; t.vbs = bs + pv0 * XKV_SLOTS;
+        }
         if (fuse_q) {
             WM_TRY(wm_dec_xattn_fq(ctx, a, t));
         } else {
diff --git a/openai-whisper-coreml_amd/csrc/model.h b/openai-whisper-coreml_amd/csrc/model.h
--- a/openai-whisper-coreml_amd/csrc/model.h
+++ b/openai-whisper-coreml_amd/csrc/model.h
@@ -273,6 +273,7 @@
     bool budget = false;
     int stop_eot = -1;
     bool xattn_shared = false;
+    int xpk = 0;
     int n_cand = 1;
     int beam = 0;
     bool rep = false;
@@ -289,7 +290,7 @@
     float *acap_q = nullptr;
     bool operator==(const WmDecodeMode &o) const {
         return acap == o.acap && acap_base == o.acap_base && acap_Tq == o.acap_Tq && acap_J == o.acap_J && acap_q == o.acap_q && panel == o.panel && trunc == o.trunc && alt == o.alt && given == o.given && srows == o.srows && rep == o.rep && sb == o.sb && sbt == o.sbt && cst == o.cst && n_cand == o.n_cand && beam == o.beam && mask == o.mask && ts == o.ts && x == o.x && off == o.off && stop == o.stop && budget == o.budget &&
-               stop_eot == o.stop_eot && xattn_shared == o.xattn_shared;
+               stop_eot == o.stop_eot && xattn_shared == o.xattn_shared && xpk == o.xpk;
     }
 };
 
@@ -346,6 +347,14 @@
     float *mel_f32 = nullptr;
     bf16_t *xkv = nullptr;
     bf16_t *skv = nullptr;
+    WmDevBuf xpk, xbs;
+    int xpk_b = 0;
+    bool xpk_valid = false;
+    int xpk_planes = 0;
+    int *dxpk_esc = nullptr;
+    int *h_xpk_esc = nullptr;
+    hipEvent_t xpk_ev = nullptr;
+    long xpk_bursts = 0;
     float *dx = nullptr;
     bf16_t *dxb = nullptr;
     float *dmean = nullptr;
@@ -367,12 +376,13 @@
     struct GraphSet {
         int B = 0, n_prompt = 0, cap_b = 0;
         WmDecodeMode mode;
-        int burst[2] = {0, 0};
-        WmGraph g1[2], gk[2];
-        int bburst[2] = {0, 0};
-        WmGraph b1[2], bk[2];
+        static constexpr int kShapes = 8;
+        int burst[kShapes] = {0, 0, 0, 0, 0, 0, 0, 0};
+        WmGraph g1[kShapes], gk[kShapes];
+        int bburst[kShapes] = {0, 0, 0, 0, 0, 0, 0, 0};
+        WmGraph b1[kShapes], bk[kShapes];
         void destroy() {
-            for (int i = 0; i < 2; ++i) { g1[i].destroy(); gk[i].destroy(); b1[i].destroy(); bk[i].destroy(); }
+            for (int i = 0; i < kShapes; ++i) { g1[i].destroy(); gk[i].destroy(); b1[i].destroy(); bk[i].destroy(); }
         }
         unsigned long stamp = 0;
     };
@@ -468,6 +478,9 @@
 int wm_model_encode_layer_tail(wm_ctx *ctx, int layer, int B, float *d_x_mid );
 int wm_model_encode_post(wm_ctx *ctx, int B, float *d_xa_out );
 int wm_model_cross_kv(wm_ctx *ctx, int B);
+int wm_model_xkv_pack(wm_ctx *ctx, int B);
+void wm_model_xkv_written(WmModel *m);
+int wm_model_xkv_planes(wm_ctx *ctx, int B);
 int wm_model_set_xa(wm_ctx *ctx, const float *d_xa, int B);
 int wm_model_decode_begin(wm_ctx *ctx, int B);
 int wm_model_decode_step(wm_ctx *ctx, int B, bool want_logits, int arg_first, int arg_last, const WmAlignCap *cap = nullptr,
@@ -630,6 +643,9 @@
     const int *off;
     DecWarm pf;
     bool short_lived;
+    int packed;
+    const unsigned char *kpk, *vpk;
+    const unsigned char *kbs, *vbs;
 };
 int wm_dec_attn_splits(int B, int H);
 int wm_dec_attention(wm_ctx *ctx, const DecAttnArgs &t);
@@ -714,6 +730,9 @@
 
 int wm_xkv_rows(wm_ctx *ctx, bf16_t *group, long group_rows, bf16_t *store, const int *d_rows, int row0, int n_rows, int L2,
                 long slab, bool to_store);
+
+int wm_xkv_pack(wm_ctx *ctx, const bf16_t *src, long pairs, int T, long pairs_per_plane, unsigned char *packed, unsigned char *bases,
+                int *escaped);
 
 int wm_align_capture_q(wm_ctx *ctx, const float *dq, int d, int B, const WmAlignLayer &L, float *cap, int Tq, int J,
                        const int *pos_ptr, int panel = 1, int base = -1);
diff --git a/openai-whisper-coreml_amd/csrc/transcribe.cpp b/openai-whisper-coreml_amd/csrc/transcribe.cpp
--- a/openai-whisper-coreml_amd/csrc/transcribe.cpp
+++ b/openai-whisper-coreml_amd/csrc/transcribe.cpp
@@ -271,6 +271,7 @@
     }
     WM_HIP(hipEventRecord(j.ev[0], c->stream));
     WM_TRY(wm_stage_cross_kv(c, call.src, j.b0, Cg, call.mem, d_pcm, j.win, j.xrows, j.ev[1]));
+    if (N == 1 && !call.beam && !call.src.windows && !j.mode.acap && !call.f32_path) WM_TRY(wm_model_xkv_pack(c, Cg));
 
     WM_HIP(hipEventRecord(j.ev[2], c->stream));
     WM_TRY(wm_model_embed_first(c, Bg, j.mode));
@@ -448,11 +449,14 @@
     WmModel *m = c->model;
     const int K = burst_len();
     const bool gen = j.mode.beam && j.t >= n_prompt - 1;
-    const int sh = shared ? 1 : 0;
     WmDecodeMode mode = j.mode;
     mode.xattn_shared = shared;
+    mode.xpk = j.mode.n_cand == 1 && !j.mode.beam && j.mode.panel <= 1 && !j.mode.acap ? wm_model_xkv_planes(c, j.Bg) : 0;
+    const int sh = (shared ? 1 : 0) + 2 * mode.xpk;
+    if (mode.xpk) ++m->xpk_bursts;
     const bool phase = j.gplan.reason == WM_GP_SERVED;
     if (phase && j.t == n_prompt) {
+        mode.xpk = 0;
         WM_TRY(lane_given_panels(j, n_steps - n_prompt + 1, mode));
     } else {
         const int left = (j.mode.beam && !gen ? n_prompt - 1 : (phase ? n_prompt : n_steps)) - j.t;
diff --git a/openai-whisper-coreml_amd/csrc/wm_tuning.h b/openai-whisper-coreml_amd/csrc/wm_tuning.h
--- a/openai-whisper-coreml_amd/csrc/wm_tuning.h
+++ b/openai-whisper-coreml_amd/csrc/wm_tuning.h
@@ -25,5 +25,6 @@
     int lane_parts = 0;
     int teacher_panel_cut = 0;
     int spec_group = 0;
+    int xkv_pack = 0;
     int lane_solo_cus = 0;
 };
diff --git a/openai-whisper-coreml_amd/csrc/xkv_pack.h b/openai-whisper-coreml_amd/csrc/xkv_pack.h
--- /dev/null
+++ b/openai-whisper-coreml_amd/csrc/xkv_pack.h
@@ -0,0 +1,98 @@
+#pragma once
+#include <stdint.h>
+
+#if defined(__HIPCC__)
+#define XKV_HD __host__ __device__ inline
+#else
+#define XKV_HD inline
+#endif
+
+constexpr int XKV_ROW_VALUES = 64;
+constexpr int XKV_ROW_BYTES = 96;
+constexpr int XKV_LANE_BYTES = 12;
+constexpr int XKV_SLOTS = 1536;
+
+XKV_HD int xkv_base_slot(int i) { return (i & ~255) | ((i & 63) << 2) | ((i >> 6) & 3); }
+
+XKV_HD int xkv_exp(uint16_t v) { return (v >> 7) & 0xff; }
+
+XKV_HD int xkv_base_of(int e_max, int e_min) {
+    const int base = e_max - 14 > 1 ? e_max - 14 : 1;
+    return (e_min >= 1 && e_max <= 254 && e_min >= base) ? base : 0;
+}
+XKV_HD int xkv_row_base(const uint16_t *row) {
+    int e_max = 0, e_min = 255;
+    for (int i = 0; i < XKV_ROW_VALUES; ++i) {
+        const int e = xkv_exp(row[i]);
+        e_max = e > e_max ? e : e_max;
+        e_min = e < e_min ? e : e_min;
+    }
+    return xkv_base_of(e_max, e_min);
+}
+
+XKV_HD uint32_t xkv_code(uint16_t v, int base) { return ((uint32_t)(v >> 15) << 11) | ((uint32_t)(v & 0x7fffu) - ((uint32_t)base << 7)); }
+XKV_HD uint16_t xkv_value(uint32_t code, int base) { return (uint16_t)(((code & 0x7ffu) + ((uint32_t)base << 7)) | ((code & 0x800u) << 4)); }
+
+XKV_HD void xkv_pack_lane(const uint32_t (&v)[4], int base, uint32_t (&out)[3]) {
+    uint32_t c[8];
+    for (int j = 0; j < 4; ++j) {
+        c[2 * j] = xkv_code((uint16_t)(v[j] & 0xffffu), base);
+        c[2 * j + 1] = xkv_code((uint16_t)(v[j] >> 16), base);
+    }
+    out[0] = c[0] | c[1] << 12 | c[2] << 24;
+    out[1] = c[2] >> 8 | c[3] << 4 | c[4] << 16 | c[5] << 28;
+    out[2] = c[5] >> 4 | c[6] << 8 | c[7] << 20;
+}
+
+XKV_HD uint32_t xkv_perm(uint32_t hi, uint32_t lo, uint32_t sel) {
+#if defined(__HIP_DEVICE_COMPILE__)
+    return __builtin_amdgcn_perm(hi, lo, sel);
+#else
+    const uint64_t all = (uint64_t)hi << 32 | lo;
+    uint32_t r = 0;
+    for (int k = 0; k < 4; ++k) r |= (uint32_t)((all >> (8 * ((sel >> (8 * k)) & 7))) & 0xff) << (8 * k);
+    return r;
+#endif
+}
+
+XKV_HD uint32_t xkv_unpack_pair(uint32_t x, uint32_t base2) {
+#if defined(__HIP_DEVICE_COMPILE__)
+    typedef __attribute__((ext_vector_type(2))) unsigned short xkv_u16x2;
+    xkv_u16x2 h = __builtin_bit_cast(xkv_u16x2, x);
+    h = h >> xkv_u16x2{0, 4};
+    const uint32_t y = __builtin_bit_cast(uint32_t, h);
+#else
+    const uint32_t y = (x & 0xffffu) | ((x >> 4) & 0x0fff0000u);
+#endif
+    return ((y & 0x07ff07ffu) + base2) | ((y & 0x08000800u) << 4);
+}
+
+XKV_HD void xkv_unpack_lane(uint32_t w0, uint32_t w1, uint32_t w2, int base, uint32_t (&v)[4]) {
+    const uint32_t base2 = ((uint32_t)base << 7) * 0x00010001u;
+    v[0] = xkv_unpack_pair(xkv_perm(w0, w0, 0x02010100u), base2);
+    v[1] = xkv_unpack_pair(xkv_perm(w1, w0, 0x05040403u), base2);
+    v[2] = xkv_unpack_pair(xkv_perm(w2, w1, 0x04030302u), base2);
+    v[3] = xkv_unpack_pair(xkv_perm(w2, w2, 0x03020201u), base2);
+}
+
+XKV_HD int xkv_pack_row(const uint16_t *row, uint8_t *packed) {
+    const int base = xkv_row_base(row);
+    for (int e8 = 0; e8 < 8; ++e8) {
+        uint32_t v[4], o[3] = {0, 0, 0};
+        for (int j = 0; j < 4; ++j) v[j] = (uint32_t)row[e8 * 8 + 2 * j] | (uint32_t)row[e8 * 8 + 2 * j + 1] << 16;
+        if (base) xkv_pack_lane(v, base, o);
+        for (int k = 0; k < XKV_LANE_BYTES; ++k) packed[e8 * XKV_LANE_BYTES + k] = (uint8_t)(o[k / 4] >> (8 * (k % 4)));
+    }
+    return base;
+}
+XKV_HD void xkv_unpack_row(const uint8_t *packed, int base, uint16_t *row) {
+    for (int e8 = 0; e8 < 8; ++e8) {
+        uint32_t w[3] = {0, 0, 0}, v[4];
+        for (int k = 0; k < XKV_LANE_BYTES; ++k) w[k / 4] |= (uint32_t)packed[e8 * XKV_LANE_BYTES + k] << (8 * (k % 4));
+        xkv_unpack_lane(w[0], w[1], w[2], base, v);
+        for (int j = 0; j < 4; ++j) {
+            row[e8 * 8 + 2 * j] = (uint16_t)(v[j] & 0xffffu);
+            row[e8 * 8 + 2 * j + 1] = (uint16_t)(v[j] >> 16);
+        }
+    }
+}
diff --git a/openai-whisper-coreml_amd/csrc/xkv_pack.hip b/openai-whisper-coreml_amd/csrc/xkv_pack.hip
--- /dev/null
+++ b/openai-whisper-coreml_amd/csrc/xkv_pack.hip
@@ -0,0 +1,66 @@
+#include "model.h"
+#include "xkv_pack.h"
+
+namespace {
+constexpr int kThreads = 256, kVec = 4;
+constexpr int kRows = (kThreads / 8) * kVec;
+typedef __attribute__((ext_vector_type(3))) unsigned u32x3;
+typedef u32x3 u32x3_a4 __attribute__((aligned(4)));
+
+__global__ __launch_bounds__(kThreads) void xkv_pack_kernel(const uint4 *__restrict__ src, unsigned char *__restrict__ packed,
+                                                            unsigned char *__restrict__ bases, int *__restrict__ escaped, int T,
+                                                            long long pairs_per_plane) {
+    const long long pair = blockIdx.x;
+    const int e8 = threadIdx.x & 7, g = threadIdx.x >> 3;
+    const int r0 = (int)blockIdx.y * kRows + g;
+    uint4 v[kVec];
+#pragma unroll
+    for (int k = 0; k < kVec; ++k) {
+        const int r = r0 + k * (kThreads / 8);
+        if (r < T) v[k] = src[(pair * T + r) * 8 + e8];
+    }
+    int n_esc = 0;
+#pragma unroll
+    for (int k = 0; k < kVec; ++k) {
+        const int r = r0 + k * (kThreads / 8);
+        if (r >= T) continue;
+        const uint32_t w[4] = {v[k].x, v[k].y, v[k].z, v[k].w};
+        int e_max = 0, e_min = 255;
+#pragma unroll
+        for (int j = 0; j < 4; ++j) {
+            const int lo = xkv_exp((uint16_t)(w[j] & 0xffffu)), hi = xkv_exp((uint16_t)(w[j] >> 16));
+            e_max = max(e_max, max(lo, hi));
+            e_min = min(e_min, min(lo, hi));
+        }
+#pragma unroll
+        for (int m = 1; m < 8; m <<= 1) {
+            e_max = max(e_max, __shfl_xor(e_max, m));
+            e_min = min(e_min, __shfl_xor(e_min, m));
+        }
+        const int base = xkv_base_of(e_max, e_min);
+        uint32_t o[3] = {0, 0, 0};
+        if (base) xkv_pack_lane(w, base, o);
+        *(u32x3_a4 *)(packed + ((pair * T + r) * 8 + e8) * XKV_LANE_BYTES) = u32x3{o[0], o[1], o[2]};
+        if (e8 == 0) {
+            bases[pair * XKV_SLOTS + xkv_base_slot(r)] = (unsigned char)base;
+            n_esc += base == 0;
+        }
+    }
+#pragma unroll
+    for (int m = 1; m < 64; m <<= 1) n_esc += __shfl_xor(n_esc, m);
+    if ((threadIdx.x & 63) == 0 && n_esc) atomicAdd(escaped + (pair / pairs_per_plane) % 2, n_esc);
+}
+}
+
+int wm_xkv_pack(wm_ctx *ctx, const bf16_t *src, long pairs, int T, long pairs_per_plane, unsigned char *packed, unsigned char *bases,
+                int *escaped) {
+    WM_REQUIRE(src && packed && bases && escaped && pairs >= 1 && pairs < (1L << 31) && T >= 1 && T <= XKV_SLOTS && pairs_per_plane >= 1,
+               WM_ERR_INVALID, "xkv_pack: bad shape (%ld pairs of %d rows, %ld per plane)", pairs, T, pairs_per_plane);
+    WM_REQUIRE((uintptr_t)src % 16 == 0 && (uintptr_t)packed % 4 == 0 && (uintptr_t)escaped % 4 == 0, WM_ERR_INVALID,
+               "xkv_pack: misaligned buffer");
+    WmProfScope ps(&ctx->prof, "xkv_pack", ctx->stream);
+    const dim3 grid((unsigned)pairs, (unsigned)((T + kRows - 1) / kRows));
+    xkv_pack_kernel<<<grid, kThreads, 0, ctx->stream>>>((const uint4 *)src, packed, bases, escaped, T, (long long)pairs_per_plane);
+    WM_HIP(hipGetLastError());
+    return WM_OK;
+}
```

Result: slower. 2156 (-1.2%).
